# Elensil/Facet_Graph_Convolution

Hardware: AMD Instinct MI355X
Metric: facets/sec (fwd+bwd) on 100k-facet mesh (higher is better)
Workload: dtype f32; 1 GPU; c2: torus 250x200 quads = 100000 facets per GPU (N0=122224 padded nodes), full graph U-Net + MLP: rotate + forward + angular loss + backward + Adam, fp32, hipGraph replay; parallelism=single GPU

## Files before the change

facet_graph_convolution_amd/_lib.py:

```python
import ctypes as C
import os

import torch

_HERE = os.path.dirname(os.path.abspath(__file__))
LIB_PATH = os.environ.get("FGC_LIB", os.path.join(_HERE, "csrc", "libfgc.so"))

ABI_VERSION = 112
FGC_M = 9
AG_LD = 24
DL_LD = 12

c_f32p = C.c_void_p
c_i32p = C.c_void_p


class ConvDesc(C.Structure):
    _fields_ = [
        ("n", C.c_int32), ("nnz", C.c_int32),
        ("rowptr", C.c_void_p), ("col", C.c_void_p),
        ("x0", C.c_void_p), ("x1", C.c_void_p),
        ("c0", C.c_int32), ("c1", C.c_int32), ("shift", C.c_int32), ("cout", C.c_int32),
        ("W0", C.c_void_p), ("b", C.c_void_p), ("u", C.c_void_p), ("c", C.c_void_p), ("v", C.c_void_p),
        ("bias_mask", C.c_int32), ("act", C.c_int32), ("alpha", C.c_float), ("src_rows", C.c_int32), ("max_deg", C.c_int32),
        ("tile_list", C.c_void_p), ("n_tiles", C.c_int32), ("proj_row0", C.c_int32), ("proj_rows", C.c_int32),
        ("flags", C.c_int32),
        ("pair_rowptr", C.c_void_p), ("pair_col", C.c_void_p), ("pair_mul", C.c_void_p),
        ("n_pairs", C.c_int32), ("max_pair_deg", C.c_int32), ("max_pair_in_deg", C.c_int32),
        ("hc", C.c_void_p),
        ("options", C.c_void_p), ("n_options", C.c_int32), ("reserved1", C.c_int32),
        ("packed_layout", C.c_uint64),
    ]


class OptionOverride(C.Structure):
    _fields_ = [("index", C.c_int32), ("reserved", C.c_int32), ("value", C.c_int64)]


def option_overrides(**values):
    names = option_names()
    arr = (OptionOverride * len(values))()
    for k, (name, value) in enumerate(values.items()):
        arr[k].index, arr[k].reserved, arr[k].value = names.index(name[4:] if name.startswith("FGC_") else name), 0, int(value)
    return arr


class RowJob(C.Structure):
    _fields_ = [("src", C.c_void_p), ("idx", C.c_void_p), ("dst", C.c_void_p), ("rows", C.c_int32), ("width", C.c_int32)]


class ConvBwdIO(C.Structure):
    _fields_ = [
        ("trowptr", C.c_void_p), ("tcol", C.c_void_p), ("tedge", C.c_void_p), ("max_in_deg", C.c_int32), ("stages", C.c_int32),
        ("ag", C.c_void_p), ("y", C.c_void_p), ("dy", C.c_void_p),
        ("ds", C.c_void_p), ("dl", C.c_void_p), ("dag", C.c_void_p), ("r", C.c_void_p),
        ("dx0", C.c_void_p), ("dx1", C.c_void_p),
        ("accumulate0", C.c_int32), ("accumulate1", C.c_int32),
        ("dW0", C.c_void_p), ("db", C.c_void_p), ("du", C.c_void_p), ("dc", C.c_void_p), ("dv", C.c_void_p),
        ("data_tile_list", C.c_void_p), ("n_data_tiles", C.c_int32), ("flags", C.c_int32),
        ("z_saved", C.c_void_p), ("pool_y", C.c_void_p), ("pool_dy", C.c_void_p),
        ("tpair_rowptr", C.c_void_p), ("tpair_col", C.c_void_p), ("tpair_edge", C.c_void_p), ("dt", C.c_void_p),
        ("r_ld", C.c_int32), ("reserved0", C.c_int32),
    ]


class PackExtra(C.Structure):
    _fields_ = [
        ("rot_x", C.c_void_p), ("rot_y", C.c_void_p), ("rot_R", C.c_void_p), ("rot_rows", C.c_int64), ("rot_vecs", C.c_int32),
        ("rot_ag", C.c_void_p), ("rot_u", C.c_void_p), ("rot_c", C.c_void_p), ("rot_v", C.c_void_p),
        ("mlp_bf16", C.c_int32), ("mlp_W1", C.c_void_p), ("mlp_W2", C.c_void_p),
        ("mlp_n", C.c_int32), ("mlp_cin", C.c_int32), ("mlp_hidden", C.c_int32), ("mlp_cout", C.c_int32),
        ("mlp_fwd_ws", C.c_void_p), ("mlp_bwd_ws", C.c_void_p),
    ]


CONV_PACKED = 1
MLP_PACKED = 1
CONV_DEFER_REDUCE = 2
CONV_DEFER_DW = 16
CONV_SAVE_Z = 4
CONV_BF16 = 8
CONV_R_PAD = 32
SYNTH_ON = 0x80000000


def mlp_layout(layout_id):
    return int(layout_id) << 8


_SIGS = {
    "fgc_last_error": (C.c_char_p, []),
    "fgc_version": (C.c_int, []),
    "fgc_set_option": (C.c_int, [C.c_char_p, C.c_int64]),
    "fgc_get_option": (C.c_int, [C.c_char_p, C.POINTER(C.c_int64)]),
    "fgc_option_count": (C.c_int32, []),
    "fgc_option_name": (C.c_char_p, [C.c_int32]),
    "fgc_struct_size": (C.c_size_t, [C.c_int32]),
    "fgc_crc32c": (C.c_uint32, [C.c_uint32, C.c_void_p, C.c_size_t]),
    "fgc_profile_enable": (C.c_int, [C.c_int]),
    "fgc_profile_tag": (C.c_int, [C.c_char_p]),
    "fgc_profile_collect": (C.c_int, [C.c_char_p, C.c_int32]),
    "fgc_csr_from_klist": (C.c_int, [C.c_void_p, C.c_int32, C.c_int32, C.c_void_p, C.c_void_p, C.c_void_p]),
    "fgc_klist_from_csr": (C.c_int, [C.c_void_p, C.c_void_p, C.c_int32, C.c_int32, C.c_void_p]),
    "fgc_csr_transpose": (C.c_int, [C.c_void_p, C.c_void_p, C.c_int32, C.c_void_p, C.c_void_p, C.c_void_p]),
    "fgc_pair_graph": (C.c_int, [C.c_void_p, C.c_void_p, C.c_int32, C.c_void_p, C.c_void_p, C.c_void_p, C.c_void_p]),
    "fgc_face_features": (C.c_int, [C.c_void_p, C.c_int32, C.c_void_p, C.c_int32, C.c_void_p, C.c_void_p]),
    "fgc_faces_large_adj": (C.c_int, [C.c_void_p, C.c_int32, C.c_int32, C.c_int32, C.c_void_p, C.c_void_p]),
    "fgc_graph_patch": (C.c_int, [C.c_void_p, C.c_int32, C.c_int32, C.c_int32, C.c_int32, C.c_void_p, C.c_int32, C.c_void_p,
                                  C.c_void_p, C.c_void_p, C.c_void_p]),
    "fgc_mesh_patch": (C.c_int, [C.c_void_p, C.c_int32, C.c_void_p, C.c_int32, C.c_void_p, C.c_int32, C.c_int32,
                                 C.c_int32, C.c_void_p, C.c_int32, C.c_void_p, C.c_void_p, C.c_void_p, C.c_void_p,
                                 C.POINTER(C.c_int32), C.POINTER(C.c_int32)]),
    "fgc_vertices_faces": (C.c_int, [C.c_void_p, C.c_int32, C.c_int32, C.c_int32, C.c_void_p]),
    "fgc_face_centers": (C.c_int, [C.c_void_p, C.c_int32, C.c_void_p, C.c_int32, C.c_void_p, C.c_void_p]),
    "fgc_pool4_avg_iz": (C.c_int, [C.c_void_p, C.c_int32, C.c_int32, C.c_void_p, C.c_void_p]),
    "fgc_vertex_update_ms": (C.c_int, [C.c_void_p, C.c_void_p, C.c_int32, C.c_void_p, C.c_int32, C.c_void_p, C.c_int32,
                                       C.c_void_p, C.c_void_p, C.c_void_p, C.c_void_p, C.c_void_p, C.c_void_p,
                                       C.c_size_t, C.c_void_p]),
    "fgc_edge_map": (C.c_int, [C.c_void_p, C.c_int32, C.c_int32, C.c_int32, C.c_void_p, C.c_void_p, C.c_void_p]),
    "fgc_vertex_update": (C.c_int, [C.c_void_p, C.c_void_p, C.c_void_p, C.c_int32, C.c_void_p, C.c_int32, C.c_void_p,
                                    C.c_int32, C.c_void_p, C.c_int32, C.c_int32, C.c_float, C.c_void_p]),
    "fgc_metis_one_level": (C.c_int, [C.c_void_p, C.c_void_p, C.c_void_p, C.c_int64, C.c_void_p, C.c_void_p,
                                      C.c_int32, C.c_void_p, C.c_void_p]),
    "fgc_hierarchy_build": (C.c_int, [C.c_void_p, C.c_int32, C.c_int32, C.c_void_p, C.c_void_p, C.c_int32,
                                      C.c_uint64, C.c_void_p, C.c_void_p, C.c_void_p]),
    "fgc_hierarchy_free": (None, [C.c_void_p]),
    "fgc_hierarchy_size": (C.c_int32, [C.c_void_p, C.c_int32]),
    "fgc_hierarchy_real_size": (C.c_int32, [C.c_void_p, C.c_int32]),
    "fgc_hierarchy_new_to_old": (C.c_int, [C.c_void_p, C.c_int32, C.c_void_p]),
    "fgc_hierarchy_parents": (C.c_int, [C.c_void_p, C.c_int32, C.c_void_p]),
    "fgc_hierarchy_klist": (C.c_int, [C.c_void_p, C.c_int32, C.c_int32, C.c_void_p, C.c_void_p]),
    "fgc_conv_workspace_bytes": (C.c_size_t, [C.POINTER(ConvDesc)]),
    "fgc_conv_fwd": (C.c_int, [C.POINTER(ConvDesc), C.c_void_p, C.c_void_p, C.c_void_p, C.c_void_p, C.c_size_t,
                               C.c_void_p]),
    "fgc_conv_bwd_workspace_bytes": (C.c_size_t, [C.POINTER(ConvDesc)]),
# ... 195 lines not shown
```

facet_graph_convolution_amd/csrc/fgc_common.h:

```cpp
#pragma once
#include <hip/hip_runtime.h>
#include <stdint.h>
#include <stdio.h>
#include <stdarg.h>
#include <stdlib.h>

#include "../../include/fgc.h"

namespace fgc {

void set_error(const char* fmt, ...);

#define FGC_CHECK_ARG(cond, ...)          \
    do {                                  \
        if (!(cond)) {                    \
            fgc::set_error(__VA_ARGS__);  \
            return FGC_EINVAL;            \
        }                                 \
    } while (0)

#define FGC_CHECK_LAUNCH(what)                                                        \
    do {                                                                              \
        hipError_t e__ = hipGetLastError();                                           \
        if (e__ != hipSuccess) {                                                      \
// ... 11 lines not shown
    ProfScope(const char* name, hipStream_t s) : st(s), on(prof_enabled()) {
        if (on) prof_begin(name, st);
    }
    ~ProfScope() {
        if (on) prof_end(st);
    }
};
#define FGC_LAUNCH(name, st, kernel, grid, block, smem, ...)                      \
    do {                                                                          \
        fgc::ProfScope prof__(name, st);                                          \
        hipLaunchKernelGGL(kernel, grid, block, smem, st, __VA_ARGS__);           \
    } while (0)

struct LaunchCfg {
    const char* name;
    const char* what;
    hipStream_t st;
    int grid, block;
    size_t smem;
};
template <auto Kernel, typename... Args>
static inline int launch_kernel(const LaunchCfg& c, const Args&... args) {
    if (c.smem) hipFuncSetAttribute((const void*)Kernel, hipFuncAttributeMaxDynamicSharedMemorySize, (int)c.smem);
    FGC_LAUNCH(c.name, c.st, Kernel, dim3(c.grid), dim3(c.block), c.smem, args...);
    FGC_CHECK_LAUNCH(c.what);
    return FGC_OK;
}

#define FGC_OPTION_LIST(X)                                                                                                     \
    X(NO_W8, 0)                                                      \
    X(NO_W8FAST, 0)                                  \
    X(W8_NT16, 1)                           \
    X(W8_DATA16_MIN_N, 81920)                                    \
    X(W8_DATA_SMEM_PAD, 0)           \
    X(NO_PAIRS, 0)                                              \
    X(NO_NARROW, 0)                                                            \
    X(NO_NARROW_MMA, 0)                                             \
    X(NO_NARROW_FUSED_DS, 0)                              \
    X(NO_FUSED_DS, 0)                                      \
    X(NO_FUSED_DS_BF16, 0)                                                                                       \
    X(NO_FUSED_DS128, 0)                                                                   \
    X(NO_DS_VEC, 0)                                                                  \
    X(NO_K1M, 0)                                                            \
    X(NO_K1DEEP, 0)                                                              \
    X(K1_NT16, 1)                                                                       \
    X(NO_TNBF16, 0)                                                               \
    X(NO_TNSTREAM, 0)                                                                \
    X(TN_SLOTS, 64)                                           \
    X(TNB_WGS, 256)                                                             \
    X(NO_PROJ_STREAM, 0)                          \
    X(NO_MLP_SPLIT, 0)                              \
    X(NO_MLP_BWD_SPLIT, 0)                                                                         \
    X(NO_K1_SPLIT, 0)                         \
    X(NO_BFM, 0)
enum Opt {
#define FGC_OPT_ENUM(name, def) OPT_##name,
    FGC_OPTION_LIST(FGC_OPT_ENUM)
#undef FGC_OPT_ENUM
    OPT_COUNT
};
int64_t opt(Opt o);
struct OptScope {
    const void* prev_list;
    int prev_n;
    OptScope(const void* overrides , int n);
    ~OptScope();
    OptScope(const OptScope&) = delete;
    OptScope& operator=(const OptScope&) = delete;
};
#define FGC_OPT_SCOPE(d) fgc::OptScope opt_scope__((d) ? (const void*)(d)->options : nullptr, (d) ? (d)->n_options : 0)

static inline int cdiv(int a, int b) { return (a + b - 1) / b; }
static inline size_t align_up(size_t x, size_t a) { return (x + a - 1) / a * a; }

typedef float f32x4 __attribute__((ext_vector_type(4)));
typedef float f32x2c __attribute__((ext_vector_type(2)));

#ifdef __HIPCC__
typedef __bf16 bf16x2 __attribute__((ext_vector_type(2)));
typedef __bf16 bf16x4 __attribute__((ext_vector_type(4)));
typedef __bf16 bf16x8 __attribute__((ext_vector_type(8)));
typedef unsigned u32x2 __attribute__((ext_vector_type(2)));
typedef unsigned u32x4 __attribute__((ext_vector_type(4)));
__device__ __forceinline__ f32x2c bf2_to_f2(unsigned w) {
    return f32x2c{__uint_as_float(w << 16), __uint_as_float(w & 0xFFFF0000u)};
}
__device__ __forceinline__ unsigned f2_to_bf2(float a, float b) {
    return __builtin_bit_cast(unsigned, __builtin_convertvector(f32x2c{a, b}, bf16x2));
}
__device__ __forceinline__ f32x4 bf4_to_f4(u32x2 w) {
    return f32x4{__uint_as_float(w[0] << 16), __uint_as_float(w[0] & 0xFFFF0000u), __uint_as_float(w[1] << 16),
                 __uint_as_float(w[1] & 0xFFFF0000u)};
}
__device__ __forceinline__ u32x2 f4_to_bf4(f32x4 v) { return u32x2{f2_to_bf2(v[0], v[1]), f2_to_bf2(v[2], v[3])}; }
__device__ __forceinline__ float bf_to_f(unsigned short h) { return __uint_as_float((unsigned)h << 16); }
__device__ __forceinline__ unsigned short f_to_bf(float v) {
    return __builtin_bit_cast(unsigned short, (__bf16)v);
}
__device__ __forceinline__ float ld_act(const float* base, size_t idx, int bf16) {
    return bf16 ? bf_to_f(reinterpret_cast<const unsigned short*>(base)[idx]) : base[idx];
}
__device__ __forceinline__ void st_act(float* base, size_t idx, float v, int bf16) {
    if (bf16) reinterpret_cast<unsigned short*>(base)[idx] = f_to_bf(v);
    else base[idx] = v;
}

#define FGC_ROW16_SUM(v)                      \
// ... 60 lines not shown
```

facet_graph_convolution_amd/csrc/fgc_conv_bwd.hip:

```cpp
#include <stdio.h>
#include <stdlib.h>
#include <string.h>

#include <algorithm>
#include <type_traits>

#include "fgc_conv_bwd.h"
#include "fgc_conv_narrow.h"
#include "fgc_conv_pair.h"
#include "fgc_gemm_tn.h"
#include "fgc_reduce.h"
#include "fgc_split.h"

namespace fgc {

__device__ __forceinline__ float slope_from_y(float y, float alpha) { return y > 0.f ? 1.f : (y < 0.f ? alpha : 0.f); }

__device__ __forceinline__ float pool4_grad_term(const float* __restrict__ y, const float* __restrict__ pool_y,
                                                 const float* __restrict__ pool_dy, int r, int col, int cout, int bf16) {
    const size_t pi = (size_t)(r >> 2) * cout + col;
    const float m = ld_act(pool_y, pi, bf16);
    const size_t b = (size_t)(r & ~3) * cout + col;
    float ne = 0.f;
#pragma unroll
    for (int k = 0; k < 4; ++k) ne += ld_act(y, b + (size_t)k * cout, bf16) == m ? 1.f : 0.f;
    return ld_act(y, (size_t)r * cout + col, bf16) == m ? ld_act(pool_dy, pi, bf16) / ne : 0.f;
}

__global__ __launch_bounds__(256) void ds_db_kernel(const float* __restrict__ dy, const float* __restrict__ y,
                                                    const int* __restrict__ rowptr, int n, int cout, int cp2, int act,
                                                    float alpha, int bias_mask, int rows_per_block,
                                                    float* __restrict__ ds, float* __restrict__ db_part, int in_bf16,
                                                    int out_bf16, const float* __restrict__ pool_y,
                                                    const float* __restrict__ pool_dy) {
    __shared__ float part[256];
    const int col = threadIdx.x % cp2, rl = threadIdx.x / cp2, nrl = 256 / cp2;
    const int r0 = blockIdx.x * rows_per_block;
    const int r1 = min(n, r0 + rows_per_block);
    float acc = 0.f;
    if (col < cout) {
        for (int r = r0 + rl; r < r1; r += nrl) {
            const int d = rowptr[r + 1] - rowptr[r];
            float g = ld_act(dy, (size_t)r * cout + col, in_bf16);
            if (pool_dy) g += pool4_grad_term(y, pool_y, pool_dy, r, col, cout, in_bf16);
            if (act) g *= slope_from_y(ld_act(y, (size_t)r * cout + col, in_bf16), alpha);
            if (!bias_mask || d > 0) acc += g;
            st_act(ds, (size_t)r * cout + col, d > 0 ? g / (float)d : 0.f, out_bf16);
        }
    }
    part[threadIdx.x] = acc;
    __syncthreads();
    if (rl == 0 && col < cout) {
        float v = 0.f;
        for (int t = 0; t < nrl; ++t) v += part[t * cp2 + col];
        db_part[(size_t)blockIdx.x * cout + col] = v;
    }
}

template <bool BF_IN, bool BF_OUT>
__global__ __launch_bounds__(256) void ds_db_vec_kernel(const float* __restrict__ dy, const float* __restrict__ y,
                                                        const int* __restrict__ rowptr, int n, int cout, int act,
                                                        float alpha, int bias_mask, int rows_per_block,
                                                        float* __restrict__ ds, float* __restrict__ db_part,
// ... 393 lines not shown
#pragma unroll
    for (int nn = 0; nn < NPW; ++nn) {
        const int node = wave * NPW + nn;
        const int i = tile0 + node;
        const int d = __builtin_amdgcn_readfirstlane(min(s.deg[node], KMAX));
        f32x4 da = f32x4{0.f, 0.f, 0.f, 0.f};
        if (d > 0 && i < p.n) {
            const int e0 = p.rowptr[i];
            const int ntile = d > 16 ? 2 : 1;
            for (int et = 0; et < ntile; ++et) {
                const int edge = et * 16 + lr;
                const bool ok = edge < d;
                const float* qr = s.qbuf + ((size_t)node * KMAX + min(edge, d - 1)) * QLD;
                f32x4 q = f32x4{0.f, 0.f, 0.f, 0.f};
                if (lq < 2) q = *reinterpret_cast<const f32x4*>(qr + 4 * lq);
                else if (lq == 2) q[0] = qr[8];
                f32x4 g = et == 0 ? dq[nn][0] : dq[nn][1];
                if (lq == 2) { g[1] = 0.f; g[2] = 0.f; g[3] = 0.f; }
                if (lq == 3) g = f32x4{0.f, 0.f, 0.f, 0.f};
                float dot = q[0] * g[0] + q[1] * g[1] + q[2] * g[2] + q[3] * g[3];
                dot += __shfl_xor(dot, 16);
                dot += __shfl_xor(dot, 32);
                f32x4 dl;
#pragma unroll
                for (int t = 0; t < 4; ++t) dl[t] = ok ? q[t] * (g[t] - dot) : 0.f;
                if (ok && lq < 3) *reinterpret_cast<f32x4*>(lp.dl + (size_t)(e0 + edge) * FGC_DL_LD + 4 * lq) = dl;
                da += dl;
            }
#pragma unroll
            for (int t = 0; t < 4; ++t) {
                float v = da[t];
                v += __shfl_xor(v, 1);
                v += __shfl_xor(v, 2);
                v += __shfl_xor(v, 4);
                v += __shfl_xor(v, 8);
                da[t] = v;
            }
        }
        if (i < p.n && lr == 0 && lq < 3) *reinterpret_cast<f32x4*>(lp.dag + (size_t)i * FGC_AG_LD + 4 * lq) = da;
        dcacc += da;
    }
    __syncthreads();
    if (lr == 0 && lq < 3) {
#pragma unroll
        for (int t = 0; t < 4; ++t) red[wave * 12 + 4 * lq + t] = dcacc[t];
    }
    __syncthreads();
    if (tid < 12) {
        const float v = tid < FGC_M ? (red[tid] + red[12 + tid]) + (red[24 + tid] + red[36 + tid]) : 0.f;
        lp.dc_part[(size_t)blockIdx.x * 12 + tid] = v;
    }
}

template <bool LONG, int OKG, int NT_ = 32, int NPW_ = 8, bool SPLIT = false>
__global__ __launch_bounds__((NT_ / NPW_) * 64, NT_ == 32 ? 2 : 4) void conv_bwd_logits_deep_kernel(CoreParams p, LogitParams lp) {
    static_assert((NT_ == 32 && NPW_ == 8) || (NT_ == 16 && NPW_ == 4 && !LONG), "tile shapes");
    static_assert(!SPLIT || (NT_ == 16 && OKG == 2), "split dz GEMM: half tiles of the 32-wide layers");
    constexpr int TILE = NT_, NPW = NPW_, NWV = NT_ / NPW_, NTHREADS = NWV * 64, RT = NT_ / 16, LPN = NTHREADS / NT_;
    static_assert(NWV == 4, "four waves either way: the column-tile split and the dc sums below assume it");
    extern __shared__ __attribute__((aligned(16))) char smem_raw[];
    constexpr int QS = LONG ? KMAX : 16;
    const Smem s = carve(smem_raw, ZSTRIDE, QS, NT_);
    const int opad = OKG ? OKG * 16 : lp.opad;
    const int ostride = OKG ? OKG * 16 + 8 : lp.ostride;
    float* dst = s.extra;
    float* red = dst + ((LONG && lp.a_global) ? 0 : TILE * ostride);
    const int tile0 = xcd_tile(blockIdx.x, gridDim.x) * TILE;
    const int tid = threadIdx.x;
    const int wave = tid >> 6, lane = tid & 63, lr = lane & 15, lq = lane >> 4;

    const bool a_global = LONG && lp.a_global;
    if (a_global) {
    } else if constexpr (OKG > 0) {
        constexpr int V4 = TILE * OKG * 16 / 4;
        constexpr int PER = (V4 + NTHREADS - 1) / NTHREADS;
        static_assert(V4 % NTHREADS == 0 || V4 < NTHREADS, "whole float4s per thread, or fewer float4s than threads");
        const f32x4* src = reinterpret_cast<const f32x4*>(lp.ds + (size_t)tile0 * (OKG * 16));
        const int vmax = (min(p.n - tile0, TILE) * OKG * 16) / 4 - 1;
        f32x4 v[PER];
        if (lp.dy) {
            const f32x4* dy4 = reinterpret_cast<const f32x4*>(lp.dy + (size_t)tile0 * (OKG * 16));
            const f32x4* y4 = reinterpret_cast<const f32x4*>(lp.y + (size_t)tile0 * (OKG * 16));
            f32x4* out4 = reinterpret_cast<f32x4*>(lp.ds_out + (size_t)tile0 * (OKG * 16));
            f32x4 gy[PER], yy[PER];
            int dg[PER];
#pragma unroll
            for (int k = 0; k < PER; ++k) {
                const int t = min(tid + k * NTHREADS, vmax);
                const int i = tile0 + t / (OKG * 4);
                gy[k] = dy4[t];
                if (lp.act || lp.pool_dy) yy[k] = y4[t];
                dg[k] = p.rowptr[i + 1] - p.rowptr[i];
            }
            if (lp.pool_dy) {
#pragma unroll
                for (int k = 0; k < PER; ++k) {
                    const int t = min(tid + k * NTHREADS, vmax);
                    const int rl = t / (OKG * 4), c4 = t % (OKG * 4);
                    const size_t pi = (size_t)((tile0 + rl) >> 2) * (OKG * 4) + c4;
                    const f32x4 m = reinterpret_cast<const f32x4*>(lp.pool_y)[pi];
                    const f32x4 gp = reinterpret_cast<const f32x4*>(lp.pool_dy)[pi];
                    f32x4 ne = f32x4{0.f, 0.f, 0.f, 0.f};
#pragma unroll
                    for (int q = 0; q < 4; ++q) {
                        const int tq = min(((rl & ~3) + q) * (OKG * 4) + c4, vmax);
                        const f32x4 yq = y4[tq];
#pragma unroll
                        for (int c = 0; c < 4; ++c) ne[c] += yq[c] == m[c] ? 1.f : 0.f;
                    }
#pragma unroll
                    for (int c = 0; c < 4; ++c) gy[k][c] += yy[k][c] == m[c] ? gp[c] / ne[c] : 0.f;
                }
            }
#pragma unroll
            for (int k = 0; k < PER; ++k) {
                const int t = tid + k * NTHREADS;
                const bool ok = t <= vmax;
                f32x4 g = gy[k];
                if (lp.act) {
#pragma unroll
// ... 776 lines not shown
    c.ds_vec = cout % vw == 0 && 256 % (cout / vw) == 0 && cout <= 256 && al16(io->dy, io->y ? io->y : io->dy, io->ds) && pool_al &&
               opt(OPT_NO_DS_VEC) != 1;
    const bool al = al16(io->ds);
    c.okg = !al ? 0 : cout == 32 ? 2 : cout == 64 ? 4 : (cout == 128 && w.k1_half && c.fuse_ds) ? 8 : 0;
    c.a_global = w.k1 == K1_DEEP && w.k1_long && cout > 32 && cout % 16 == 0 && al;
    c.k1 = c.narrow_path ? K1_NARROW : w.k1;
    c.k1_vec4 = conv_vec4_ok(d);
    c.ds = w.pairs ? DS_PAIR : c.fuse_ds ? DS_FUSED : (c.narrow_path && narrow_fuses_ds(d, io)) ? DS_NARROW_FUSED
         : c.ds_vec ? DS_VEC : DS_SCALAR;
    return c;
}

static TnPlan layer_tn_plan(const fgc_conv_desc* d, const fgc_conv_bwd_io* io, const BwdPlan& w) {
    const int cout = d->cout, PL = FGC_M * cout + 24;
    const int rps = tn_rows_per_slab(w.nred, w.splitW), rld = io_r_ld(io, cout, w.bf16);
    if (w.pairs)
        return tn_plan_of(w.bf16, true, true, io->r, PL, d->x0, nullptr, d->c0, 0, 0, w.nred, rps, w.slab, rld);
    const bool v4 = conv_vec4_ok(d) && (cout % 4 == 0) && ((uintptr_t)io->r % 16 == 0);
    const bool stream_ok = v4 && !(opt(OPT_NO_TNSTREAM) == 1);
    return tn_plan_of(w.bf16, v4, stream_ok, io->r, PL, d->x0, d->x1, d->c0, d->c1, d->shift, w.nred, rps, w.slab, rld);
}

static void conv_param_jobs(const fgc_conv_desc* d, const fgc_conv_bwd_io* io, const BwdPlan& w, RedJob* jobs) {
    const int cin = d->c0 + d->c1, cout = d->cout;
    const int P = FGC_M * cout, PL = P + 24;
    const int ns = cdiv(w.nred, tn_rows_per_slab(w.nred, w.splitW));
    const size_t sst = (size_t)PL * cin;
    jobs[0] = RedJob{w.slab, sst, ns, P * cin, cin, cin, io->dW0, w.rtmp};
    jobs[1] = RedJob{w.slab + (size_t)P * cin, sst, ns, FGC_M * cin, cin, cin, io->du};
    jobs[2] = RedJob{w.slab + (size_t)(P + 12) * cin, sst, ns, FGC_M * cin, cin, cin, io->dv};
    jobs[3] = RedJob{w.db_part, (size_t)cout, w.nb_db, cout, cout, cout, io->db};
    jobs[4] = RedJob{w.dc_part, (size_t)12, w.n_dc, 12, 12, FGC_M, io->dc};
}

static int launch_ds_db(const BwdPlan& w, const BwdCall& c, const fgc_conv_desc* d, const fgc_conv_bwd_io* io, hipStream_t st) {
    const LaunchCfg cfg{"ds_db_kernel", "fgc_conv_bwd/ds", st, w.nb_db, 256, 0};
    const float *yy = io->y ? io->y : io->dy, *pool_y = io->pool_dy ? io->pool_y : nullptr;
    const bool out_bf16 = w.bf16 && !c.narrow_path;
    if (c.ds == DS_SCALAR) {
        int cp2 = 1;
        while (cp2 < d->cout) cp2 <<= 1;
        return launch_kernel<ds_db_kernel>(cfg, io->dy, io->y, d->rowptr, d->n, d->cout, cp2, d->act, d->alpha, d->bias_mask, w.rows_per_db,
                                           io->ds, w.db_part, w.bf16 ? 1 : 0, out_bf16 ? 1 : 0, pool_y, io->pool_dy);
    }
    auto vec = [&](auto bf_in, auto bf_out) {
        return launch_kernel<ds_db_vec_kernel<decltype(bf_in)::value, decltype(bf_out)::value>>(
            cfg, io->dy, yy, d->rowptr, d->n, d->cout, d->act, d->alpha, d->bias_mask, w.rows_per_db, io->ds, w.db_part, pool_y, io->pool_dy);
    };
    if (!w.bf16) return vec(std::false_type{}, std::false_type{});
    return out_bf16 ? vec(std::true_type{}, std::true_type{}) : vec(std::true_type{}, std::false_type{});
}

static int launch_k1(const BwdPlan& w, const BwdCall& c, const fgc_conv_desc* d, const CoreParams& p, const LogitParams& lp,
                     hipStream_t st) {
    const int nt = w.k1_nodes, cout = d->cout;
    const int qs = ((w.k1 == K1_DEEP || w.k1 == K1_BF16) && !w.k1_long) ? 16 : KMAX;
    const size_t core = smem_core_bytes(w.k1 == K1_BF16 ? ZSTRIDE_BF / 2 : w.g1.zstride, qs, nt);
    const size_t tile = w.k1 == K1_BF16 ? (size_t)nt * (cout * 2 + 32) : lp.a_global ? 0 : (size_t)nt * lp.ostride * 4;
    LaunchCfg cfg{"conv_bwd_logits_deep_kernel", "fgc_conv_bwd/logits_mfma", st, cdiv(d->n, nt), NTHREADS, core + tile + 48 * 4};
    switch (c.k1) {
        case K1_BF16:
            cfg.name = "conv_bwd_logits_bf16_kernel";
            cfg.what = "fgc_conv_bwd/logits_bf16";
            if (w.k1_long) return launch_kernel<conv_bwd_logits_bf16_kernel<true>>(cfg, p, lp);
            if (w.k1_half) return launch_kernel<conv_bwd_logits_bf16_kernel<false, 16, 4>>(cfg, p, lp);
            return launch_kernel<conv_bwd_logits_bf16_kernel<false>>(cfg, p, lp);
        case K1_DEEP:
            if (w.k1_split) {
                FGC_CHECK_ARG(c.okg == 2, "fgc_conv_bwd: ds must be 16-byte aligned (cout=%d)", cout);
                return launch_kernel<conv_bwd_logits_deep_kernel<false, 2, 16, 4, true>>(cfg, p, lp);
            }
            if (w.k1_half) switch (c.okg) {
                case 2: return launch_kernel<conv_bwd_logits_deep_kernel<false, 2, 16, 4>>(cfg, p, lp);
                case 4: return launch_kernel<conv_bwd_logits_deep_kernel<false, 4, 16, 4>>(cfg, p, lp);
                case 8: return launch_kernel<conv_bwd_logits_deep_kernel<false, 8, 16, 4>>(cfg, p, lp);
                default: return launch_kernel<conv_bwd_logits_deep_kernel<false, 0, 16, 4>>(cfg, p, lp);
            }
            if (w.k1_long) switch (c.okg) {
                case 2: return launch_kernel<conv_bwd_logits_deep_kernel<true, 2>>(cfg, p, lp);
                case 4: return launch_kernel<conv_bwd_logits_deep_kernel<true, 4>>(cfg, p, lp);
                default: return launch_kernel<conv_bwd_logits_deep_kernel<true, 0>>(cfg, p, lp);
            }
            switch (c.okg) {
                case 2: return launch_kernel<conv_bwd_logits_deep_kernel<false, 2>>(cfg, p, lp);
                case 4: return launch_kernel<conv_bwd_logits_deep_kernel<false, 4>>(cfg, p, lp);
                default: return launch_kernel<conv_bwd_logits_deep_kernel<false, 0>>(cfg, p, lp);
            }
        case K1_MFMA:
            cfg.name = "conv_bwd_logits_mfma_kernel";
            return c.k1_vec4 ? launch_kernel<conv_bwd_logits_mfma_kernel<true>>(cfg, p, lp)
                             : launch_kernel<conv_bwd_logits_mfma_kernel<false>>(cfg, p, lp);
        default:
            cfg.what = "fgc_conv_bwd/logits";
            if (c.k1_vec4) {
                cfg.name = "conv_bwd_logits_kernel<LPN, true>";
                return launch_kernel<conv_bwd_logits_kernel<8, true>>(cfg, p, lp);
            }
            cfg.name = "conv_bwd_logits_kernel<LPN, false>";
            return launch_kernel<conv_bwd_logits_kernel<8, false>>(cfg, p, lp);
    }
}

enum DataKind { DATA_NONE, DATA_W8, DATA_TILED };
struct DataForm {
    int kind;
    W8Form w8;
    bool vec4;
    int max_deg;
};
static DataForm data_form(const BwdPlan& w, const BwdCall& c, const fgc_conv_desc* d, const fgc_conv_bwd_io* io, CoreParams& p,
                          DataEpilogue& ep) {
    DataForm f{};
    const int cin = d->c0 + d->c1, cout = d->cout;
    if (c.narrow_path) return f;
    if (w.pairs) {
        fill_core_params(p, w.g2, w.nred, io->tpair_rowptr, io->tpair_col, io->tpair_edge, io->dt, nullptr, cout, 0, 0, cin, io->ag,
                         0, 12, 0, w.Wpt);
        ep = DataEpilogue{io->dl, io->dag, io->r, io_r_ld(io, cout, w.bf16), d->u, d->v, cin, d->c0, 0, 0,
                          io->dx0, nullptr, io->accumulate0, 0};
        f.max_deg = d->max_pair_in_deg;
        f.kind = DATA_W8;
    } else {
        fill_core_params(p, w.g2, d->n, io->trowptr, io->tcol, io->tedge, io->ds, nullptr, cout, 0, 0, cin, io->ag,
                         d->shift, 12, 0, w.Wpt);
        ep = DataEpilogue{io->dl, io->dag, io->r, io_r_ld(io, cout, w.bf16), d->u, d->v, cin, d->c0, d->c1, d->shift,
                          io->dx0, io->dx1, io->accumulate0, io->accumulate1};
        f.max_deg = io->max_in_deg;
        f.kind = (w.bf16 || w8_supported(p, f.max_deg)) ? DATA_W8 : DATA_TILED;
        f.vec4 = (cout % 4 == 0) && ((uintptr_t)io->ds % 16 == 0) && ((uintptr_t)io->r % 16 == 0);
    }
    p.tile_list = io->data_tile_list;
    p.n_tiles = io->n_data_tiles;
    if (f.kind == DATA_W8) f.w8 = w8_form(p, &ep, f.max_deg, w.bf16);
    return f;
}

}

using namespace fgc;

extern "C" size_t fgc_conv_bwd_workspace_bytes(const fgc_conv_desc* d) {
    FGC_OPT_SCOPE(d);
    if (!d) return 0;
    return plan_bwd(d, nullptr).bytes;
}

extern "C" uint64_t fgc_conv_layout_id(const fgc_conv_desc* d) {
    FGC_OPT_SCOPE(d);
    return d ? conv_layout_id(d) : 1;
}

extern "C" int32_t fgc_conv_r_ld(int32_t cout, int32_t padded, int32_t bf16) {
    return conv_r_ld(cout, padded ? FGC_CONV_R_PAD : 0, bf16 != 0);
}

extern "C" int fgc_conv_bwd_needs_exchange(const fgc_conv_desc* d, const fgc_conv_bwd_io* io) {
    FGC_OPT_SCOPE(d);
    if (!d || !io) return 1;
    return (io->dx0 == nullptr && narrow_supported(d)) ? 0 : 1;
}

extern "C" int fgc_conv_forms(const fgc_conv_desc* d, const fgc_conv_bwd_io* io, char* buf, int32_t buf_bytes) {
    FGC_OPT_SCOPE(d);
    int rc = validate_conv_desc(d, "fgc_conv_forms");
    if (rc) return rc;
    FGC_CHECK_ARG(buf && buf_bytes > 0, "fgc_conv_forms: no buffer");
    int len = 0;
    bool full = false;
    auto put = [&](const char* key, const char* fmt, auto value) {
        char tmp[96];
        int k = snprintf(tmp, sizeof tmp, "%s%s=", len ? " " : "", key);
        k += snprintf(tmp + k, sizeof tmp - k, fmt, value);
        if (len + k + 1 > buf_bytes) { full = true; return; }
        memcpy(buf + len, tmp, (size_t)k + 1);
        len += k;
    };
    auto put_w8 = [&](const char* pre, const W8Form& f, bool vec4) {
        char key[32];
        auto k = [&](const char* name) { snprintf(key, sizeof key, "%s_%s", pre, name); return key; };
        put(k("fast"), "%d", (int)f.fast);
        put(k("slots"), "%d", f.qs);
        put(k("nt"), "%d", f.nt);
        put(k("bfm"), "%d", (int)f.bfm);
        put(k("vec4"), "%d", (int)vec4);
    };
    static const char* const fwd_names[] = {"pair", "narrow", "w8", "tiled"};
    static const char* const proj_names[] = {"pair", "narrow", "bf16", "stream", "block", "block"};
    static const char* const ds_names[] = {"pair", "fused", "narrow-fused", "vec", "scalar"};
    static const char* const k1_names[] = {"pair", "narrow", "bf16", "deep", "mfma", "valu"};
    static const char* const k2_names[] = {"none", "w8", "tiled"};
    static const char* const tn_names[] = {"stream2", "stream4", "stream2_bf", "stream4_bf", "bf16_4", "bf16_2", "plain_v4", "plain"};
    buf[0] = 0;
    CoreParams p;
    const FwdForm ff = conv_fwd_form(d, io ? io->ag : nullptr, nullptr, &p);
    put("fwd", "%s", fwd_names[ff.kind]);
    if (ff.kind == FWD_NARROW) put("fwd_mma", "%d", (int)narrow_fwd_mma(d, nullptr));
    put_w8("fwd", ff.kind == FWD_W8 ? ff.w8 : W8Form{false, false, KMAX, TILE}, ff.vec4);
    put("proj", "%s", proj_names[ff.proj]);
    const BwdPlan w = call_plan(d, io, nullptr);
    const int rps = tn_rows_per_slab(w.nred, w.splitW);
    const BwdCall c = io ? bwd_call(w, d, io) : BwdCall{};
    if (io) {
        put("ds", "%s", ds_names[c.ds]);
        put("k1", "%s", k1_names[c.k1]);
        if (c.k1 == K1_NARROW) put("k1_mma", "%d", (int)narrow_bwd_mma(d, io));
        put("k1_okg", "%d", c.okg);
        put("k1_aglobal", "%d", (int)c.a_global);
        put("k1_vec4", "%d", (int)c.k1_vec4);
    } else {
        put("k1", "%s", k1_names[w.k1]);
    }
    put("k1_long", "%d", (int)w.k1_long);
    put("k1_half", "%d", (int)w.k1_half);
    put("k1_split", "%d", (int)w.k1_split);
    put("k1_nodes", "%d", w.k1_nodes);
    if (io) {
        DataEpilogue ep;
        const DataForm df = data_form(w, c, d, io, p, ep);
        put("k2", "%s", k2_names[df.kind]);
        put_w8("k2", df.kind == DATA_W8 ? df.w8 : W8Form{false, false, KMAX, TILE}, df.kind == DATA_W8 || df.vec4);
        put("k2_chunks", "%d", df.max_deg > 0 ? cdiv(df.max_deg, KMAX) : 0);
        if (c.k1 == K1_NARROW) put("k3", "%s", "narrow");
        else {
            const TnPlan pl = layer_tn_plan(d, io, w);
            put("k3", "%s", tn_names[pl.variant]);
            put("k3_slabs", "%d", pl.nsplits);
            put("k3_rows", "%d", pl.a.rps);
        }
    } else {
        put("k3_slabs", "%d", cdiv(w.nred, rps));
        put("k3_rows", "%d", rps);
    }
    put("nb_db", "%d", w.nb_db);
    put("n_dc", "%d", w.n_dc);
    put("layout_id", "%llu", (unsigned long long)layout_id_of(w));
    FGC_CHECK_ARG(!full, "fgc_conv_forms: buffer of %d bytes too small", buf_bytes);
    return len;
}

extern "C" int fgc_conv_bwd(const fgc_conv_desc* d, const fgc_conv_bwd_io* io, void* workspace,
                            size_t workspace_bytes, void* stream) {
    FGC_OPT_SCOPE(d);
    int rc = validate_conv_desc(d, "fgc_conv_bwd");
    if (rc) return rc;
    const int cin = d->c0 + d->c1, cout = d->cout;
    const BwdPlan w = call_plan(d, io, (char*)workspace);
    const bool bf16 = w.bf16;
    FGC_CHECK_ARG(io != nullptr, "fgc_conv_bwd: null io");
    FGC_CHECK_ARG(io->trowptr && io->tcol && io->tedge, "fgc_conv_bwd: transposed CSR missing");
    FGC_CHECK_ARG(io->ag && io->dy && io->ds && io->dl && io->dag && io->r, "fgc_conv_bwd: null buffer");
    FGC_CHECK_ARG(!d->act || io->y, "fgc_conv_bwd: y required when an activation was applied");
    FGC_CHECK_ARG(io->dW0 && io->db && io->du && io->dc && io->dv, "fgc_conv_bwd: null parameter-gradient pointer");
    FGC_CHECK_ARG(io->dx0 != nullptr || io->dx1 == nullptr, "fgc_conv_bwd: dx1 without dx0");
    FGC_CHECK_ARG(io_r_ld_ok(io, cout, bf16),
                  "fgc_conv_bwd: r_ld = %d is not a row stride of r for cout = %d (0, or >= %d and congruent to it modulo %d)",
                  io->r_ld, cout, FGC_M * cout + 24, bf16 ? 8 : 4);
    FGC_CHECK_ARG(!(io->flags & FGC_CONV_PACKED) || d->packed_layout == 0 || d->packed_layout == layout_id_of(w),
                  "fgc_conv_bwd: FGC_CONV_PACKED, but the operands were packed in layout %llu and the options now select %llu "
                  "(an option changed between fgc_conv_pack and this call)", (unsigned long long)d->packed_layout,
                  (unsigned long long)layout_id_of(w));
    FGC_CHECK_ARG(workspace && workspace_bytes >= w.bytes && (uintptr_t)workspace % 16 == 0,
                  "fgc_conv_bwd: workspace too small or misaligned (%zu < %zu)", workspace_bytes, w.bytes);
    hipStream_t st = (hipStream_t)stream;
    const BwdCall c = bwd_call(w, d, io);
    const int stages = c.stages;
    const bool pack_here = !(io->flags & FGC_CONV_PACKED);
    PackJob pjobs[2];
    size_t ptotals[2];
    if (w.pairs) {
        FGC_CHECK_ARG(io->tpair_rowptr && io->tpair_col && io->tpair_edge && io->dt && d->max_pair_in_deg > 0,
                      "fgc_conv_bwd: the pair form needs the transposed pair graph, dt and max_pair_in_deg");
        FGC_CHECK_ARG(!io->pool_dy, "fgc_conv_bwd: the pair form has no pooled output");
        FGC_CHECK_ARG(io->data_tile_list == nullptr || (io->n_data_tiles >= 0 && io->n_data_tiles <= cdiv(w.nred, TILE)),
                      "fgc_conv_bwd: pair form: n_data_tiles=%d outside [0, %d]", io->n_data_tiles, cdiv(w.nred, TILE));
        FGC_CHECK_ARG(((uintptr_t)io->dt | (uintptr_t)io->dy | (uintptr_t)io->dl | (uintptr_t)io->dag | (uintptr_t)io->r) % 16 == 0,
                      "fgc_conv_bwd: the pair form needs 16-byte aligned buffers");
        if ((stages & 4) && pack_here) {
            rc = launch_pack_jobs(pjobs, ptotals, conv_bwd_pack_jobs(d, w, pjobs, ptotals), "fgc_conv_bwd/pack", st);
            if (rc) return rc;
        }
        if (stages & 3) {
            rc = launch_pair_bwd_logits(d, io, w.db_part, w.dc_part, st);
            if (rc) return rc;
        }
        if (stages & 4) {
            CoreParams p;
            DataEpilogue ep;
            data_form(w, c, d, io, p, ep);
            const size_t smem = conv_smem_bytes(w.g2, (size_t)TILE * 24 * 4);
            FGC_CHECK_ARG(w8_erow_supported(p, d->max_pair_in_deg) && (!bf16 || w8_bf16_supported(p, d->max_pair_in_deg)),
                          "fgc_conv_bwd: pair form: unsupported shape (cin=%d cout=%d max_pair_in_deg=%d)", cin, cout,
                          d->max_pair_in_deg);
            if (!p.tile_list || p.n_tiles > 0) {
                rc = launch_data_w8_erow(p, ep, smem, d->max_pair_in_deg, st, bf16);
                if (rc) return rc;
            }
        }
    } else {
        FGC_CHECK_ARG(io->data_tile_list == nullptr || (io->n_data_tiles >= 0 && io->n_data_tiles <= cdiv(d->n, TILE)),
                      "fgc_conv_bwd: n_data_tiles=%d outside [0, %d]", io->n_data_tiles, cdiv(d->n, TILE));
        FGC_CHECK_ARG(!bf16 || c.narrow_path || (w.deep_ok && cout % 32 == 0),
                      "fgc_conv_bwd: FGC_CONV_BF16 needs widths that are multiples of 32, 16-byte aligned tensors and degrees <= %d "
                      "(cin=%d cout=%d max_deg=%d)", KMAX, cin, cout, d->max_deg);
        FGC_CHECK_ARG(!io->pool_dy || (io->pool_y && io->y && d->n % 4 == 0),
                      "fgc_conv_bwd: pool_dy needs pool_y, y and a row count that is a multiple of 4 (n=%d)", d->n);
        if ((stages & 1) && (c.ds == DS_VEC || c.ds == DS_SCALAR)) {
            rc = launch_ds_db(w, c, d, io, st);
            if (rc) return rc;
        }
        if (c.k1 == K1_NARROW) {
            if (stages & 2) {
                rc = narrow_bwd_logits(d, io, w.narrow_ws, w.db_part, st);
                if (rc) return rc;
            }
            if (stages & 8) {
                rc = narrow_bwd_params(d, io, w.narrow_ws, w.db_part, narrow_db_partials(d, io, w.nb_db),
                                       (io->flags & FGC_CONV_DEFER_REDUCE) ? 1 : 3, nullptr, st);
                if (rc) return rc;
            }
            return FGC_OK;
        }
        if ((stages & 6) && pack_here) {
            rc = launch_pack_jobs(pjobs, ptotals, conv_bwd_pack_jobs(d, w, pjobs, ptotals), "fgc_conv_bwd/pack", st);
            if (rc) return rc;
        }
        if (stages & 2) {
            CoreParams p;
            fill_core_params(p, w.g1, d->n, d->rowptr, d->col, nullptr, d->x0, d->x1, d->c0, d->c1, d->shift, cout, io->ag,
                             d->shift, 0, 12, nullptr);
            LogitParams lp{io->ds, cout, w.opad, w.opad + 8, w.Wq, io->dl, io->dag, w.dc_part};
            if (c.fuse_ds) {
                lp.dy = io->dy;
                lp.y = io->y ? io->y : io->dy;
                lp.act = d->act;
                lp.bias_mask = d->bias_mask;
                lp.alpha = d->alpha;
                lp.ds_out = io->ds;
                lp.db_part = w.db_part;
                lp.pool_y = io->pool_dy ? io->pool_y : nullptr;
                lp.pool_dy = io->pool_dy;
            }
            lp.a_global = c.a_global;
            rc = launch_k1(w, c, d, p, lp, st);
            if (rc) return rc;
        }
        if ((stages & 4) && !(io->data_tile_list && io->n_data_tiles == 0)) {
            CoreParams p;
            DataEpilogue ep;
            const DataForm f = data_form(w, c, d, io, p, ep);
            const size_t smem = conv_smem_bytes(w.g2, (size_t)TILE * 24 * 4);
            if (bf16)
                FGC_CHECK_ARG(w8_bf16_supported(p, io->max_in_deg), "fgc_conv_bwd: FGC_CONV_BF16: unsupported shape for the data "
                              "gradient (cin=%d cout=%d max_in_deg=%d)", cin, cout, io->max_in_deg);
            if (f.kind == DATA_W8) {
                rc = launch_data_w8(p, ep, smem, io->max_in_deg, st, bf16);
            } else if (f.vec4) {
                rc = launch_kernel<conv_bwd_data_kernel<8, true>>(
                    LaunchCfg{"conv_bwd_data_kernel<LPN, true>", "fgc_conv_bwd/data", st, core_grid(p), NTHREADS, smem}, p, ep);
            } else {
                rc = launch_kernel<conv_bwd_data_kernel<8, false>>(
                    LaunchCfg{"conv_bwd_data_kernel<LPN, false>", "fgc_conv_bwd/data", st, core_grid(p), NTHREADS, smem}, p, ep);
            }
            if (rc) return rc;
        }
    }
    if (stages & 8) {
        if (!(io->flags & FGC_CONV_DEFER_DW)) {
            rc = tn_launch_one(layer_tn_plan(d, io, w), "gemm_tn_kernel:dW", st);
            if (rc) return rc;
        }
        if (!(io->flags & FGC_CONV_DEFER_REDUCE)) {
            RedJob jobs[5];
            conv_param_jobs(d, io, w, jobs);
            rc = reduce_jobs("reduce:params", jobs, 5, nullptr, st);
            if (rc) return rc;
        }
    }
    return FGC_OK;
}

extern "C" int fgc_conv_bwd_reduce(const fgc_conv_desc* const* descs, const fgc_conv_bwd_io* const* ios,
                                   void* const* bwd_ws, int32_t count, void* stream) {
    FGC_CHECK_ARG(descs && ios && bwd_ws && count >= 0, "fgc_conv_bwd_reduce: bad arguments");
    hipStream_t st = (hipStream_t)stream;
    RedJob jobs[RED_MAX_JOBS];
    int nj = 0, rc = 0;
    auto flush = [&]() {
        const int r = nj ? reduce_jobs("reduce:params", jobs, nj, nullptr, st) : FGC_OK;
        nj = 0;
        return r;
    };
    {
        TnJobs G[TN_NVARIANTS];
        int nb[TN_NVARIANTS];
        for (int v = 0; v < TN_NVARIANTS; ++v) G[v].njobs = 0, nb[v] = 0;
        for (int i = 0; i < count; ++i) {
            const fgc_conv_desc* d = descs[i];
            const fgc_conv_bwd_io* io = ios[i];
            if (!io || !(io->flags & FGC_CONV_DEFER_DW)) continue;
            FGC_OPT_SCOPE(d);
            rc = validate_conv_desc(d, "fgc_conv_bwd_reduce");
            if (rc) return rc;
            FGC_CHECK_ARG(bwd_ws[i], "fgc_conv_bwd_reduce: layer %d: null workspace", i);
            const BwdPlan w = plan_bwd(d, (char*)bwd_ws[i]);
            TnPlan pl;
            if (io->dx0 == nullptr && w.narrow) {
                const float* A;
                float* slab;
                int zld, rps;
                narrow_tn_operands(d, io, w.narrow_ws, &A, &zld, &slab, &rps);
                pl = tn_plan_of(false, true, true, A, zld, io->ds, nullptr, d->cout, 0, 0, d->n, rps, slab);
            } else {
                FGC_CHECK_ARG(io->r, "fgc_conv_bwd_reduce: layer %d: FGC_CONV_DEFER_DW without r", i);
                FGC_CHECK_ARG(io_r_ld_ok(io, d->cout, (d->flags & FGC_CONV_BF16) != 0),
                              "fgc_conv_bwd_reduce: layer %d: r_ld = %d is not a row stride of r for cout = %d", i, io->r_ld, d->cout);
                pl = layer_tn_plan(d, io, w);
            }
            if (!tn_groupable(pl.variant)) {
                rc = tn_launch_one(pl, "gemm_tn_kernel:dW", st);
                if (rc) return rc;
                continue;
            }
            TnJobs& J = G[pl.variant];
            if (J.njobs == TN_MAX_JOBS) {
                rc = tn_launch_group(pl.variant, J, nb[pl.variant], "gemm_tn_kernel:dW", st);
                if (rc) return rc;
                nb[pl.variant] = 0;
            }
            pl.a.block0 = nb[pl.variant];
            J.job[J.njobs++] = pl.a;
            nb[pl.variant] += (int)tn_grid(pl.ntiles, pl.nsplits).x;
        }
        for (int v = 0; v < TN_NVARIANTS; ++v) {
            rc = tn_launch_group(v, G[v], nb[v], "gemm_tn_kernel:dW", st);
            if (rc) return rc;
        }
    }
    for (int i = 0; i < count; ++i) {
        const fgc_conv_desc* d = descs[i];
        const fgc_conv_bwd_io* io = ios[i];
        FGC_OPT_SCOPE(d);
        rc = validate_conv_desc(d, "fgc_conv_bwd_reduce");
        if (rc) return rc;
        FGC_CHECK_ARG(io && bwd_ws[i] && io->dW0 && io->db && io->du && io->dc && io->dv,
                      "fgc_conv_bwd_reduce: layer %d: null io / workspace / gradient pointer", i);
        const BwdPlan w = plan_bwd(d, (char*)bwd_ws[i]);
        if (nj + 5 > RED_MAX_JOBS && (rc = flush())) return rc;
        if (io->dx0 == nullptr && w.narrow) {
            rc = narrow_bwd_params(d, io, w.narrow_ws, w.db_part, narrow_db_partials(d, io, w.nb_db), 0, jobs + nj, st);
            if (rc) return rc;
            nj += NARROW_RED_JOBS;
        } else {
            conv_param_jobs(d, io, w, jobs + nj);
            nj += 5;
        }
    }
    if ((rc = flush())) return rc;
    return FGC_OK;
}
```

facet_graph_convolution_amd/csrc/fgc_conv_pair.h:

```cpp
#pragma once
#include "fgc_common.h"

namespace fgc {

bool pairs_ok(const fgc_conv_desc* d);
bool pairs_graph_allowed(int64_t rows, int64_t n_pairs, int max_in_deg, int cout);
int pair_blocks_per_wg(int cout);
static inline int pair_num_wgs(const fgc_conv_desc* d) {
    const int bpg = pair_blocks_per_wg(d->cout);
    return ((d->n >> 2) + bpg - 1) / bpg;
}
int launch_pair_fwd(const fgc_conv_desc* d, float* ag, float* y, void* workspace, hipStream_t st);
int launch_pair_bwd_logits(const fgc_conv_desc* d, const fgc_conv_bwd_io* io, float* db_part, float* dc_part,
                           hipStream_t st);

}
```

facet_graph_convolution_amd/csrc/fgc_conv_pair.hip:

```cpp
#include <stdlib.h>

#include "fgc_conv_core.h"
#include "fgc_conv_pair.h"

namespace fgc {

constexpr int PQ_LD = 12;
constexpr int PQ_SLOTS = 16;
constexpr int PQ_STRIDE = PQ_SLOTS * PQ_LD + 4;

bool pairs_graph_allowed(int64_t rows, int64_t n_pairs, int max_in_deg, int cout) {
    if (rows < 0 || n_pairs < 0 || cout <= 0 || max_in_deg < 0 || max_in_deg > KMAX) return false;
    if ((uint64_t)rows * FGC_M * cout * 4 >= 0xFFFFFFFFull || (uint64_t)n_pairs * cout * 4 >= 0xFFFFFFFFull) return false;
    if (rows >= (1 << 24) || n_pairs >= (1 << 24) - (1 << 20)) return false;
    return true;
}

bool pairs_ok(const fgc_conv_desc* d) {
    if (opt(OPT_NO_PAIRS) == 1) return false;
    if ((opt(OPT_NO_W8) == 1) || (opt(OPT_NO_W8FAST) == 1))
        return false;
    if (!d || !d->pair_rowptr || !d->pair_col || !d->pair_mul || !d->hc) return false;
    if (d->shift != 2 || d->c1 != 0 || d->x1 != nullptr || (d->n & 3)) return false;
    if (!(d->c0 == 32 || d->c0 == 64 || d->c0 == 128) || !(d->cout == 32 || d->cout == 64)) return false;
    if (d->n_pairs <= 0 || d->max_pair_deg <= 0 || d->max_pair_in_deg < 0 || d->max_pair_in_deg > KMAX) return false;
    if (d->tile_list && d->n_tiles != 0) return false;
    const size_t rows = d->src_rows > 0 ? (size_t)d->src_rows : (size_t)(d->n >> 2);
    if (!pairs_graph_allowed((int64_t)rows, d->n_pairs, d->max_pair_in_deg, d->cout)) return false;
    if (((uintptr_t)d->x0 | (uintptr_t)d->hc) % 16) return false;
    return true;
}

int pair_blocks_per_wg(int cout) { return 4 * (64 / (cout / 4)); }

#ifndef FGC_PT_RT
#define FGC_PT_RT 2
#endif
#ifndef FGC_PT_KO
#define FGC_PT_KO 0
#endif
#ifndef FGC_PT_CG
#define FGC_PT_CG 10
#endif
template <int CIN, int RT>
__global__ __launch_bounds__(256) void pair_transform_kernel(const float* __restrict__ x, int rows,
                                                            const float* __restrict__ W0, const float* __restrict__ u,
                                                            const float* __restrict__ c, const float* __restrict__ v,
                                                            int cout, float* __restrict__ hc, float* __restrict__ ag,
                                                            int ngroups) {
    constexpr int KG = CIN / 16;
    const int wave = threadIdx.x >> 6, lane = threadIdx.x & 63, lr = lane & 15, lq = lane >> 4;
    const int item = __builtin_amdgcn_readfirstlane(blockIdx.x * 4 + wave);
    const int rt = item / ngroups, cg = item - rt * ngroups;
    if (rt * (16 * RT) >= rows) return;
    const int th = (FGC_M * cout) >> 4;
    const int tc = th + 2;
// ... 310 lines not shown
#pragma unroll
    for (int i = 0; i < 4; ++i) yv[i] = f32x4{0.f, 0.f, 0.f, 0.f};
    for (int k0 = 0; k0 < dmax; k0 += PQ_SLOTS) {
        if (k0) pair_wave_sync();
        pair_softmax_chunk<LPB>(p, qb, kl, e0, d, k0, bc, a);
        pair_wave_sync();
        const int cnt = min(dmax - k0, PQ_SLOTS);
        HT h[FGC_M];
        pair_load_h<COUT, BF>(h_rs, qb, laneoff, h);
        FGC_PAIR_KLOOP_PRAGMA
        for (int k = 0; k < cnt; ++k) {
            const float* qk = qb + k * PQ_LD;
            const unsigned noff = pair_row_off<COUT, BF>(qb + min(k + 1, PQ_SLOTS - 1) * PQ_LD, laneoff);
            const f32x4 q0 = *reinterpret_cast<const f32x4*>(qk), q1 = *reinterpret_cast<const f32x4*>(qk + 4);
            const f32x2c q8m = *reinterpret_cast<const f32x2c*>(qk + 8), mm = *reinterpret_cast<const f32x2c*>(qk + 10);
            const float q[FGC_M] = {q0[0], q0[1], q0[2], q0[3], q1[0], q1[1], q1[2], q1[3], q8m[0]};
            const unsigned mu = __float_as_uint(mm[0]);
            f32x4 t = {0.f, 0.f, 0.f, 0.f};
#pragma unroll
            for (int m = 0; m < FGC_M; ++m) {
                t += q[m] * pair_h(h[m]);
                h[m] = pair_load_piece<COUT, BF>(h_rs, noff, m);
            }
            yv[0] += (float)(mu & 0xffu) * t;
            yv[1] += (float)((mu >> 8) & 0xffu) * t;
            yv[2] += (float)((mu >> 16) & 0xffu) * t;
            yv[3] += (float)(mu >> 24) * t;
        }
    }
    if (b >= p.nb) return;
    const f32x4 bias = *reinterpret_cast<const f32x4*>(p.bias + kl * 4);
#pragma unroll
    for (int i = 0; i < 4; ++i) {
        const float inv = deg[i] > 0 ? 1.0f / (float)deg[i] : 0.f;
        f32x4 o = yv[i] * inv;
        if (!p.bias_mask || deg[i] > 0) o += bias;
        if (p.act) {
#pragma unroll
            for (int t = 0; t < 4; ++t) o[t] = fmaxf(o[t], 0.f) - p.alpha * fmaxf(-o[t], 0.f);
        }
        pair_st4<BF>(p.y, (size_t)(4 * b + i) * COUT + kl * 4, o);
    }
}

template <int LPB>
__device__ __forceinline__ float pair_block_sum(float v) {
    v += fgc_dpp_c<0xB1>(v);
    v += fgc_dpp_c<0x4E>(v);
    v += fgc_dpp_c<0x141>(v);
    if constexpr (LPB == 16) v += fgc_dpp_c<0x140>(v);
    return v;
}

template <int COUT, bool BF>
__global__ __launch_bounds__(256, FGC_PAIR_LB_BWD) void pair_bwd_logits_kernel(PairParams p) {
    constexpr int LPB = COUT / 4, BPW = 64 / LPB, BPG = 4 * BPW;
    constexpr int RED_LD = COUT + 12;
    __shared__ __attribute__((aligned(16))) float qs[BPG * PQ_STRIDE];
    __shared__ __attribute__((aligned(16))) float red[BPG * RED_LD];
    const int wave = threadIdx.x >> 6, lane = threadIdx.x & 63, bl = lane / LPB, kl = lane % LPB;
    const int wg = xcd_tile(blockIdx.x, gridDim.x);
    const int b = (wg * 4 + wave) * BPW + bl;
    const bool valid = b < p.nb;
    const int bc = min(b, p.nb - 1);
    const int e0 = p.prow[bc];
    const int d = valid ? p.prow[bc + 1] - e0 : 0;
    float a[FGC_M];
    {
        const float* ar = p.ag + (size_t)bc * FGC_AG_LD;
        const f32x4 a0 = *reinterpret_cast<const f32x4*>(ar), a1 = *reinterpret_cast<const f32x4*>(ar + 4);
        a[0] = a0[0]; a[1] = a0[1]; a[2] = a0[2]; a[3] = a0[3]; a[4] = a1[0]; a[5] = a1[1]; a[6] = a1[2]; a[7] = a1[3];
        a[8] = ar[8];
    }
    f32x4 sv[4];
    f32x4 dbv = {0.f, 0.f, 0.f, 0.f};
#pragma unroll
    for (int i = 0; i < 4; ++i) {
        const int dg = p.rowptr[4 * bc + i + 1] - p.rowptr[4 * bc + i];
        const size_t o = (size_t)(4 * bc + i) * COUT + kl * 4;
        f32x4 g = pair_ld4<BF>(p.dy, o);
        if (p.act) {
            const f32x4 yy = pair_ld4<BF>(p.yact, o);
#pragma unroll
            for (int t = 0; t < 4; ++t) g[t] *= yy[t] > 0.f ? 1.f : (yy[t] < 0.f ? p.alpha : 0.f);
        }
        if (!valid) g = f32x4{0.f, 0.f, 0.f, 0.f};
        if (!p.bias_mask || dg > 0) dbv += g;
        sv[i] = g * (dg > 0 ? 1.0f / (float)dg : 0.f);
    }
    const int dmax = wave_max_i32(d);
    float* qb = qs + (wave * BPW + bl) * PQ_STRIDE;
    const __amdgpu_buffer_rsrc_t h_rs = __builtin_amdgcn_make_buffer_rsrc(const_cast<float*>(p.hc), 0, -1, 0x00020000);
    const unsigned laneoff = (unsigned)kl * (BF ? 8u : 16u);
    typedef typename PairH<BF>::T HT;
    float da[FGC_M];
#pragma unroll
    for (int m = 0; m < FGC_M; ++m) da[m] = 0.f;
    const __amdgpu_buffer_rsrc_t dt_rs = __builtin_amdgcn_make_buffer_rsrc(p.dt, 0, p.dt_bytes, 0x00020000);
    const __amdgpu_buffer_rsrc_t dl_rs = __builtin_amdgcn_make_buffer_rsrc(p.dl, 0, p.dl_bytes, 0x00020000);
    for (int k0 = 0; k0 < dmax; k0 += PQ_SLOTS) {
        if (k0) pair_wave_sync();
        pair_softmax_chunk<LPB>(p, qb, kl, e0, d, k0, bc, a);
        pair_wave_sync();
        const int cnt = min(dmax - k0, PQ_SLOTS);
        HT h[FGC_M];
        pair_load_h<COUT, BF>(h_rs, qb, laneoff, h);
        FGC_PAIR_KLOOP_PRAGMA
        for (int k = 0; k < cnt; ++k) {
            const float* qk = qb + k * PQ_LD;
            const int kk = k0 + k;
            const unsigned noff = pair_row_off<COUT, BF>(qb + min(k + 1, PQ_SLOTS - 1) * PQ_LD, laneoff);
            const f32x4 q0 = *reinterpret_cast<const f32x4*>(qk), q1 = *reinterpret_cast<const f32x4*>(qk + 4);
            const f32x2c q8m = *reinterpret_cast<const f32x2c*>(qk + 8), mm = *reinterpret_cast<const f32x2c*>(qk + 10);
            const float q[FGC_M] = {q0[0], q0[1], q0[2], q0[3], q1[0], q1[1], q1[2], q1[3], q8m[0]};
// ... 78 lines not shown
    const int ngroups = cdiv(tc, FGC_PT_CG);
    const int items = cdiv(rows, 16 * FGC_PT_RT) * ngroups;
    const bool bf16 = (d->flags & FGC_CONV_BF16) != 0;
    if (rows == 0) {
    } else if (bf16) {
        unsigned short* Wb = (unsigned short*)workspace;
        if (!(d->flags & FGC_CONV_PACKED)) {
            const int count = FGC_M * cout * cin;
            FGC_LAUNCH("pair_weight_bf16_kernel", st, pair_weight_bf16_kernel, dim3(cdiv(count, 1024)), dim3(256), 0, d->W0, Wb, count);
        }
#define FGC_PTB(CIN_)                                                                                                  \
    FGC_LAUNCH("pair_transform_kernel", st, (pair_transform_bf16_kernel<CIN_, FGC_PT_RT>), dim3(cdiv(items, 4)), dim3(256), 0,      \
               (const unsigned short*)x0, rows, Wb, d->u, d->c, d->v, cout, (unsigned short*)hc0, ag0, ngroups)
        if (cin == 32) FGC_PTB(32);
        else if (cin == 64) FGC_PTB(64);
        else FGC_PTB(128);
#undef FGC_PTB
    } else {
#define FGC_PT(CIN_)                                                                                                   \
    FGC_LAUNCH("pair_transform_kernel", st, (pair_transform_kernel<CIN_, FGC_PT_RT>), dim3(cdiv(items, 4)), dim3(256), 0, x0, rows,  \
               d->W0, d->u, d->c, d->v, cout, hc0, ag0, ngroups)
    if (cin == 32) FGC_PT(32);
    else if (cin == 64) FGC_PT(64);
    else FGC_PT(128);
#undef FGC_PT
    }
    FGC_CHECK_LAUNCH("fgc_conv_fwd/pair_transform");
    if (!blocks) return FGC_OK;
    PairParams p{};
    p.nb = d->n >> 2;
    p.prow = d->pair_rowptr;
    p.pcol = d->pair_col;
    p.pmul = d->pair_mul;
    p.ag = ag;
    p.hc = d->hc;
    p.rowptr = d->rowptr;
    p.bias = d->b;
    p.bias_mask = d->bias_mask;
    p.act = d->act;
    p.alpha = d->alpha;
    p.y = y;
    const int grid = pair_num_wgs(d);
    if (bf16) {
        if (cout == 32) FGC_LAUNCH("pair_fwd_kernel", st, (pair_fwd_kernel<32, true>), dim3(grid), dim3(256), 0, p);
        else FGC_LAUNCH("pair_fwd_kernel", st, (pair_fwd_kernel<64, true>), dim3(grid), dim3(256), 0, p);
    } else {
        if (cout == 32) FGC_LAUNCH("pair_fwd_kernel", st, (pair_fwd_kernel<32, false>), dim3(grid), dim3(256), 0, p);
        else FGC_LAUNCH("pair_fwd_kernel", st, (pair_fwd_kernel<64, false>), dim3(grid), dim3(256), 0, p);
    }
    FGC_CHECK_LAUNCH("fgc_conv_fwd/pair_fwd");
    return FGC_OK;
}

int launch_pair_bwd_logits(const fgc_conv_desc* d, const fgc_conv_bwd_io* io, float* db_part, float* dc_part, hipStream_t st) {
    PairParams p{};
    p.nb = d->n >> 2;
    p.prow = d->pair_rowptr;
    p.pcol = d->pair_col;
    p.pmul = d->pair_mul;
    p.ag = io->ag;
    p.hc = d->hc;
    p.rowptr = d->rowptr;
    p.bias_mask = d->bias_mask;
    p.act = d->act;
    p.alpha = d->alpha;
    p.dy = io->dy;
    p.yact = io->y;
    p.dt = io->dt;
    p.dl = io->dl;
    p.dag = io->dag;
    p.db_part = db_part;
    p.dc_part = dc_part;
    p.dt_bytes = (unsigned)((size_t)d->n_pairs * d->cout * ((d->flags & FGC_CONV_BF16) ? 2 : 4));
    p.dl_bytes = (unsigned)((size_t)d->n_pairs * FGC_DL_LD * 4);
    const int grid = pair_num_wgs(d);
    if (d->flags & FGC_CONV_BF16) {
        if (d->cout == 32) FGC_LAUNCH("pair_bwd_logits_kernel", st, (pair_bwd_logits_kernel<32, true>), dim3(grid), dim3(256), 0, p);
        else FGC_LAUNCH("pair_bwd_logits_kernel", st, (pair_bwd_logits_kernel<64, true>), dim3(grid), dim3(256), 0, p);
    } else {
        if (d->cout == 32) FGC_LAUNCH("pair_bwd_logits_kernel", st, (pair_bwd_logits_kernel<32, false>), dim3(grid), dim3(256), 0, p);
        else FGC_LAUNCH("pair_bwd_logits_kernel", st, (pair_bwd_logits_kernel<64, false>), dim3(grid), dim3(256), 0, p);
    }
    FGC_CHECK_LAUNCH("fgc_conv_bwd/pair_logits");
    return FGC_OK;
}

}

extern "C" int fgc_conv_uses_pairs(const fgc_conv_desc* d) {
    FGC_OPT_SCOPE(d);
    return fgc::pairs_ok(d) ? 1 : 0;
}
extern "C" int fgc_conv_pairs_allowed(int64_t rows, int64_t n_pairs, int32_t max_pair_in_deg, int32_t cout) {
    return fgc::pairs_graph_allowed(rows, n_pairs, max_pair_in_deg, cout) ? 1 : 0;
}
```

facet_graph_convolution_amd/csrc/fgc_gemm_tn.h:

```cpp
#pragma once
#include "fgc_common.h"

namespace fgc {

struct TnArgs {
    const void* A;
    const void* x0;
    const void* x1;
    float* slab;
    int lda, P, c0, c1, shift, rows, rps;
    int block0;
};
constexpr int TN_MAX_JOBS = 8;
struct TnJobs {
    TnArgs job[TN_MAX_JOBS];
    int njobs;
};
constexpr int TNB_PC = 320;

enum TnVariant { TN_STREAM2 = 0, TN_STREAM4, TN_STREAM2_BF, TN_STREAM4_BF, TN_BF16_4, TN_BF16_2, TN_PLAIN_V4, TN_PLAIN, TN_NVARIANTS };
struct TnPlan {
    int variant;
    TnArgs a;
    int ntiles, nsplits;
};
static inline bool tn_groupable(int v) { return v <= TN_BF16_2; }
static inline dim3 tn_grid(int ntiles, int nsplits) { return dim3((unsigned)(ntiles * 8 * cdiv(nsplits, 8))); }
TnPlan tn_plan_of(bool bf16, bool vec4, bool stream_ok, const void* A, int PL, const void* x0, const void* x1, int c0, int c1,
                  int shift, int rows, int rps, float* slab, int lda = 0);
int tn_launch_one(const TnPlan& pl, const char* tag, hipStream_t st);
int tn_launch_group(int variant, TnJobs& J, int nblocks, const char* tag, hipStream_t st);

bool tn_bf16_ok(int P, int c0, int c1);
int tn_rows_per_slab(int n, int splits);
int tn_splits(int P, int Q, int rows);
int tn_balanced_splits(int desired, int maxs, int rows);
int launch_gemm_tn_stream(const char* tag, const float* A, int lda, int P, const float* x0, int c0, int rows,
                          int rows_per_split, int nsplits, float* slab, hipStream_t st);

}
```

facet_graph_convolution_amd/csrc/fgc_gemm_tn.hip:

```cpp
#include <algorithm>

#include "fgc_gemm_tn.h"

namespace fgc {


template <bool VEC4>
__device__ __forceinline__ void tn_load(const float* __restrict__ A, int lda, int P, const float* __restrict__ x0,
                                        const float* __restrict__ x1, int c0, int c1, int shift, int row, bool valid,
                                        int pbase, int qbase, f32x4& a, f32x4& b) {
    a = f32x4{0.f, 0.f, 0.f, 0.f};
    b = f32x4{0.f, 0.f, 0.f, 0.f};
    if (!valid) return;
    const int Q = c0 + c1;
    const size_t sr = (size_t)(row >> shift);
    if (VEC4) {
        if (pbase < P) a = *reinterpret_cast<const f32x4*>(A + (size_t)row * lda + pbase);
        if (qbase < c0) b = *reinterpret_cast<const f32x4*>(x0 + sr * c0 + qbase);
        else if (qbase < Q) b = *reinterpret_cast<const f32x4*>(x1 + sr * c1 + (qbase - c0));
    } else {
#pragma unroll
        for (int t = 0; t < 4; ++t) {
            if (pbase + t < P) a[t] = A[(size_t)row * lda + pbase + t];
            const int q = qbase + t;
            if (q < c0) b[t] = x0[sr * c0 + q];
            else if (q < Q) b[t] = x1[sr * c1 + (q - c0)];
        }
    }
}

__device__ __forceinline__ bool tn_block(int ntiles, int nsplits, int& tile, int& split, int vblock = -1) {
    const int L = vblock >= 0 ? vblock : (int)blockIdx.x, xcd = L & 7, idx = L >> 3;
    tile = idx % ntiles;
    split = (idx / ntiles) * 8 + xcd;
    return split < nsplits;
}

__device__ __forceinline__ int tn_job_of(const TnJobs& J) {
    int q = 0;
#pragma unroll
    for (int t = 1; t < TN_MAX_JOBS; ++t)
        if (t < J.njobs && (int)blockIdx.x >= J.job[t].block0) q = t;
    return q;
}

template <bool VEC4>
__global__ __launch_bounds__(256) void gemm_tn_kernel(const float* __restrict__ A, int lda, int P,
                                                      const float* __restrict__ x0, const float* __restrict__ x1,
                                                      int c0, int c1, int shift, int rows, int rows_per_split,
                                                      float* __restrict__ slab) {
    __shared__ float red[4][64][65];
    const int Q = c0 + c1;
    const int npt = (P + 63) >> 6;
    int tile_id, split_id;
    if (!tn_block(npt * ((Q + 63) >> 6), (rows + rows_per_split - 1) / rows_per_split, tile_id, split_id)) return;
    const int pt = tile_id % npt, qt = tile_id / npt;
    const int p0 = pt * 64, q0 = qt * 64;
    const int tid = threadIdx.x, wave = tid >> 6, lane = tid & 63, lr = lane & 15, lq = lane >> 4;
    const int r_begin = split_id * rows_per_split;
    const int r_end = min(rows, r_begin + rows_per_split);
    const int nsteps = (r_end - r_begin + 3) >> 2;
    const int pbase = p0 + 4 * lr, qbase = q0 + 4 * lr;
    f32x4 acc[4][4];
#pragma unroll
    for (int i = 0; i < 4; ++i)
#pragma unroll
        for (int j = 0; j < 4; ++j) acc[i][j] = f32x4{0.f, 0.f, 0.f, 0.f};

    f32x4 a0, b0, a1, b1;
    auto ld = [&](int step, f32x4& a, f32x4& b) {
        const int row = r_begin + 4 * step + lq;
        tn_load<VEC4>(A, lda, P, x0, x1, c0, c1, shift, row, step < nsteps && row < r_end, pbase, qbase, a, b);
    };
    auto mm = [&](const f32x4& a, const f32x4& b) {
#pragma unroll
        for (int i = 0; i < 4; ++i)
#pragma unroll
            for (int j = 0; j < 4; ++j) acc[i][j] = __builtin_amdgcn_mfma_f32_16x16x4f32(a[i], b[j], acc[i][j], 0, 0, 0);
    };
    ld(wave, a0, b0);
    ld(wave + 4, a1, b1);
    for (int s = wave; s < nsteps; s += 8) {
        mm(a0, b0);
        ld(s + 8, a0, b0);
        if (s + 4 < nsteps) mm(a1, b1);
        ld(s + 12, a1, b1);
    }
#pragma unroll
    for (int i = 0; i < 4; ++i)
#pragma unroll
        for (int j = 0; j < 4; ++j)
#pragma unroll
            for (int t = 0; t < 4; ++t) red[wave][4 * (lq * 4 + t) + i][4 * lr + j] = acc[i][j][t];
    __syncthreads();
    float* out = slab + (size_t)split_id * P * Q;
    for (int t = tid; t < 64 * 64; t += 256) {
        const int pp = t >> 6, qq = t & 63;
        if (p0 + pp < P && q0 + qq < Q)
            out[(size_t)(p0 + pp) * Q + q0 + qq] = (red[0][pp][qq] + red[1][pp][qq]) + (red[2][pp][qq] + red[3][pp][qq]);
    }
}

template <int NJ, bool BF>
__device__ __forceinline__ void tn_stream_body(const float* __restrict__ A, int lda, int P, const float* __restrict__ x0,
                                               const float* __restrict__ x1, int c0, int c1, int shift, int rows,
                                               int rows_per_split, float* __restrict__ slab, int vblock,
                                               float (*red)[64][65]) {
    const int Q = c0 + c1;
    const int npt = (P + 63) >> 6;
    int tile_id, split_id;
    if (!tn_block(npt * ((Q + 16 * NJ - 1) / (16 * NJ)), (rows + rows_per_split - 1) / rows_per_split, tile_id, split_id, vblock))
        return;
    const int pt = tile_id % npt, qt = tile_id / npt;
    const int p0 = pt * 64, q0 = qt * (16 * NJ);
    const int tid = threadIdx.x, lane = tid & 63, lr = lane & 15, lq = lane >> 4;
    const int wave = __builtin_amdgcn_readfirstlane(tid >> 6);
    const int r_begin = split_id * rows_per_split;
    const int r_end = min(rows, r_begin + rows_per_split);
    const int nsteps = (r_end - r_begin + 3) >> 2;
    const int pc = min(p0 + 4 * lr, P - 4);
    const int qc = min(q0 + NJ * lr, Q - NJ);
    const float* bsrc = BF ? reinterpret_cast<const float*>(reinterpret_cast<const unsigned short*>(qc < c0 ? x0 : x1) +
                                                            (qc < c0 ? qc : qc - c0))
                           : (qc < c0 ? x0 + qc : x1 + (qc - c0));
    const int bld = qc < c0 ? c0 : c1;
    f32x4 acc[4][NJ];
#pragma unroll
    for (int i = 0; i < 4; ++i)
#pragma unroll
        for (int j = 0; j < NJ; ++j) acc[i][j] = f32x4{0.f, 0.f, 0.f, 0.f};

    auto ld = [&](int step, f32x4& a, f32x4& b, int& row) {
        row = r_begin + 4 * step + lq;
        const int rc = min(row, r_end - 1);
        if constexpr (BF) {
            const unsigned short* A16 = reinterpret_cast<const unsigned short*>(A);
            const unsigned short* b16 = reinterpret_cast<const unsigned short*>(bsrc);
            a = bf4_to_f4(*reinterpret_cast<const u32x2*>(A16 + (size_t)rc * lda + pc));
            if constexpr (NJ == 4) {
                b = bf4_to_f4(*reinterpret_cast<const u32x2*>(b16 + (size_t)(rc >> shift) * bld));
            } else {
                const f32x2c b2 = bf2_to_f2(*reinterpret_cast<const unsigned*>(b16 + (size_t)(rc >> shift) * bld));
                b = f32x4{b2[0], b2[1], 0.f, 0.f};
            }
            return;
        }
        a = *reinterpret_cast<const f32x4*>(A + (size_t)rc * lda + pc);
        if constexpr (NJ == 4) {
            b = *reinterpret_cast<const f32x4*>(bsrc + (size_t)(rc >> shift) * bld);
        } else {
            const f32x2c b2 = *reinterpret_cast<const f32x2c*>(bsrc + (size_t)(rc >> shift) * bld);
            b = f32x4{b2[0], b2[1], 0.f, 0.f};
        }
    };
    auto mm = [&](f32x4 a, const f32x4& b, int row) {
        if (row >= r_end) a = f32x4{0.f, 0.f, 0.f, 0.f};
#pragma unroll
        for (int i = 0; i < 4; ++i)
#pragma unroll
            for (int j = 0; j < NJ; ++j) acc[i][j] = __builtin_amdgcn_mfma_f32_16x16x4f32(a[i], b[j], acc[i][j], 0, 0, 0);
    };
    f32x4 a0, b0, a1, b1, a2, b2, a3, b3;
    int r0, r1, r2, r3;
    ld(wave, a0, b0, r0);
    ld(wave + 4, a1, b1, r1);
    ld(wave + 8, a2, b2, r2);
    ld(wave + 12, a3, b3, r3);
#define FGC_TN_STEP(A_, B_, R_, NEXT_)          \
    mm(A_, B_, R_);                             \
    __builtin_amdgcn_sched_barrier(0);          \
    ld(NEXT_, A_, B_, R_);                      \
    __builtin_amdgcn_sched_barrier(0);
    for (int s = wave; s < nsteps; s += 16) {
        FGC_TN_STEP(a0, b0, r0, s + 16)
        FGC_TN_STEP(a1, b1, r1, s + 20)
        FGC_TN_STEP(a2, b2, r2, s + 24)
        FGC_TN_STEP(a3, b3, r3, s + 28)
    }
#undef FGC_TN_STEP
    auto put = [&](int slot) {
#pragma unroll
        for (int i = 0; i < 4; ++i)
#pragma unroll
            for (int j = 0; j < NJ; ++j)
#pragma unroll
                for (int t = 0; t < 4; ++t) red[slot][4 * (lq * 4 + t) + i][NJ * lr + j] = acc[i][j][t];
    };
    auto add = [&](int slot) {
#pragma unroll
        for (int i = 0; i < 4; ++i)
#pragma unroll
            for (int j = 0; j < NJ; ++j)
#pragma unroll
                for (int t = 0; t < 4; ++t) acc[i][j][t] += red[slot][4 * (lq * 4 + t) + i][NJ * lr + j];
    };
    if (wave == 1) put(0);
    if (wave == 3) put(1);
    __syncthreads();
    if (wave == 0) add(0);
    if (wave == 2) add(1);
    __syncthreads();
    if (wave == 0) put(0);
    if (wave == 2) put(1);
    __syncthreads();
    float* out = slab + (size_t)split_id * P * Q;
    for (int t = tid; t < 64 * 16 * NJ; t += 256) {
        const int pp = t / (16 * NJ), qq = t % (16 * NJ);
        if (p0 + pp < P && q0 + qq < Q) out[(size_t)(p0 + pp) * Q + q0 + qq] = red[0][pp][qq] + red[1][pp][qq];
    }
}

__device__ __forceinline__ bool tn_direct_ok(int lda, int c0, int c1, int shift, int rows_per_split) {
    return (c1 == 0 || (c0 & 31) == 0) && shift <= 4 &&
           (long long)(rows_per_split + 160) * max(lda, max(c0, c1)) < (1ll << 29);
}

template <int NJ>
__device__ __forceinline__ void tn_direct_body(const float* __restrict__ A, int lda, int P, const float* __restrict__ x0,
                                               const float* __restrict__ x1, int c0, int c1, int shift, int rows,
                                               int rows_per_split, float* __restrict__ slab, int vblock, f32x4* red) {
    constexpr int NH = NJ / 2;
    const int Q = c0 + c1;
    const int npt = (P + 63) >> 6;
    int tile_id, split_id;
    if (!tn_block(npt * ((Q + 16 * NJ - 1) / (16 * NJ)), (rows + rows_per_split - 1) / rows_per_split, tile_id, split_id, vblock))
        return;
    const int pt = tile_id % npt, qt = tile_id / npt;
    const int p0 = pt * 64, q0 = qt * (16 * NJ);
    const int tid = threadIdx.x, lane = tid & 63, lr = lane & 15, lq = lane >> 4;
    const int wave = __builtin_amdgcn_readfirstlane(tid >> 6);
    const int r_begin = split_id * rows_per_split;
    const int r_end = min(rows, r_begin + rows_per_split);
    const int nsteps = (r_end - r_begin + 3) >> 2;
    const int row0 = 4 * wave + lq;
    const int pc = min(p0 + 4 * lr, P - 4);
    const __amdgpu_buffer_rsrc_t a_rs = __builtin_amdgcn_make_buffer_rsrc(
        const_cast<float*>(A + (size_t)r_begin * lda), 0, (r_end - r_begin) * lda * 4, 0x00020000);
    unsigned ao = (unsigned)(row0 * lda + pc) * 4u;
    const unsigned astep = 16u * (unsigned)lda * 4u;
    const int xr0 = r_begin >> shift, xrows = ((rows - 1) >> shift) + 1;
    const int xrow0 = ((r_begin + row0) >> shift) - xr0;
    __amdgpu_buffer_rsrc_t b_rs[NH];
    unsigned bo[NH], bstep[NH];
#pragma unroll
    for (int h = 0; h < NH; ++h) {
        const int hs = q0 + 32 * h;
        const bool first = hs < c0 || c1 == 0;
        const int ld = first ? c0 : c1;
        const size_t bytes = (size_t)(xrows - xr0) * ld * 4;
        b_rs[h] = __builtin_amdgcn_make_buffer_rsrc(const_cast<float*>((first ? x0 : x1) + (size_t)xr0 * ld), 0,
                                                    (int)(unsigned)std::min<size_t>(bytes, 0xffffffffu), 0x00020000);
        bo[h] = (unsigned)(xrow0 * ld + min(hs + 2 * lr, Q - 2) - (first ? 0 : c0)) * 4u;
        bstep[h] = (unsigned)((16 >> shift) * ld) * 4u;
    }
    f32x4 acc[4][NJ];
#pragma unroll
    for (int i = 0; i < 4; ++i)
#pragma unroll
        for (int j = 0; j < NJ; ++j) acc[i][j] = f32x4{0.f, 0.f, 0.f, 0.f};

    struct Set {
        f32x4 a;
        f32x2c b[NH];
    };
    auto ld = [&](Set& s) {
        s.a = __builtin_bit_cast(f32x4, __builtin_amdgcn_raw_buffer_load_b128(a_rs, ao, 0, 0));
        ao += astep;
        asm volatile("" : "+v"(ao));
#pragma unroll
        for (int h = 0; h < NH; ++h) {
            s.b[h] = __builtin_bit_cast(f32x2c, __builtin_amdgcn_raw_buffer_load_b64(b_rs[h], bo[h], 0, 0));
            bo[h] += bstep[h];
            asm volatile("" : "+v"(bo[h]));
        }
    };
    auto mm = [&](const Set& s) {
#pragma unroll
        for (int i = 0; i < 4; ++i)
#pragma unroll
            for (int j = 0; j < NJ; ++j)
                acc[i][j] = __builtin_amdgcn_mfma_f32_16x16x4f32(s.a[i], s.b[j >> 1][j & 1], acc[i][j], 0, 0, 0);
    };
    if (wave < nsteps) {
        Set s0, s1, s2, s3;
        ld(s0);
        __builtin_amdgcn_sched_barrier(0);
        ld(s1);
        __builtin_amdgcn_sched_barrier(0);
        ld(s2);
        __builtin_amdgcn_sched_barrier(0);
        ld(s3);
        __builtin_amdgcn_sched_barrier(0);
#define FGC_TN_STEP(S_)                         \
    mm(S_);                                     \
    __builtin_amdgcn_sched_barrier(0);          \
    ld(S_);                                     \
    __builtin_amdgcn_sched_barrier(0);
        int s = wave;
        do {
            FGC_TN_STEP(s0)
            FGC_TN_STEP(s1)
            FGC_TN_STEP(s2)
            FGC_TN_STEP(s3)
            s += 16;
        } while (s < nsteps);
    }
#undef FGC_TN_STEP
    auto put = [&](int slot) {
#pragma unroll
        for (int e = 0; e < 4 * NJ; ++e) red[(slot * 4 * NJ + e) * 64 + lane] = acc[e / NJ][e % NJ];
    };
    auto add = [&](int slot) {
#pragma unroll
        for (int e = 0; e < 4 * NJ; ++e) acc[e / NJ][e % NJ] += red[(slot * 4 * NJ + e) * 64 + lane];
    };
    if (wave == 1) put(0);
    if (wave == 3) put(1);
    __syncthreads();
    if (wave == 0) add(0);
    if (wave == 2) {
        add(1);
        put(1);
    }
    __syncthreads();
    if (wave != 0) return;
    add(1);
    const __amdgpu_buffer_rsrc_t c_rs =
        __builtin_amdgcn_make_buffer_rsrc(slab + (size_t)split_id * P * Q, 0, P * Q * 4, 0x00020000);
#pragma unroll
    for (int h = 0; h < NH; ++h) {
        const int q = q0 + 32 * h + 2 * lr;
        const unsigned co = q < Q ? (unsigned)((p0 + 16 * lq) * Q + q) * 4u : 0x80000000u;
#pragma unroll
        for (int t = 0; t < 4; ++t)
#pragma unroll
            for (int i = 0; i < 4; ++i)
                __builtin_amdgcn_raw_buffer_store_b64(__builtin_bit_cast(u32x2, f32x2c{acc[i][2 * h][t], acc[i][2 * h + 1][t]}), c_rs,
                                                      co + (unsigned)((4 * t + i) * Q) * 4u, 0, 0);
    }
}

template <int NJ, bool BF>
__device__ __forceinline__ void tn_stream_any(const float* __restrict__ A, int lda, int P, const float* __restrict__ x0,
                                              const float* __restrict__ x1, int c0, int c1, int shift, int rows,
                                              int rows_per_split, float* __restrict__ slab, int vblock) {
    __shared__ __attribute__((aligned(16))) float red[2][64][65];
    if constexpr (!BF) {
        if (tn_direct_ok(lda, c0, c1, shift, rows_per_split)) {
            tn_direct_body<NJ>(A, lda, P, x0, x1, c0, c1, shift, rows, rows_per_split, slab, vblock,
                               reinterpret_cast<f32x4*>(&red[0][0][0]));
            return;
        }
    }
    tn_stream_body<NJ, BF>(A, lda, P, x0, x1, c0, c1, shift, rows, rows_per_split, slab, vblock, red);
}
template <int NJ, bool BF = false>
__global__ __launch_bounds__(256, 4) void gemm_tn_stream_kernel(const float* __restrict__ A, int lda, int P,
                                                                const float* __restrict__ x0,
                                                                const float* __restrict__ x1, int c0, int c1, int shift,
                                                                int rows, int rows_per_split, float* __restrict__ slab) {
    tn_stream_any<NJ, BF>(A, lda, P, x0, x1, c0, c1, shift, rows, rows_per_split, slab, -1);
}
template <int NJ, bool BF = false>
__global__ __launch_bounds__(256, 4) void gemm_tn_stream_group_kernel(TnJobs J) {
    const TnArgs& a = J.job[tn_job_of(J)];
    tn_stream_any<NJ, BF>((const float*)a.A, a.lda, a.P, (const float*)a.x0, (const float*)a.x1, a.c0, a.c1, a.shift, a.rows,
                          a.rps, a.slab, (int)blockIdx.x - a.block0);
}

constexpr int TNB_THREADS = 256;
constexpr int TNB_AS = TNB_PC * 2 + 32;
typedef short s16x4 __attribute__((ext_vector_type(4)));

__device__ __forceinline__ u32x4 tnb_frag(const char* tile, int stride, int col0, int lq, int lr) {
    const char* a = tile + (4 * lq + (lr >> 2)) * stride + (col0 + 4 * (lr & 3)) * 2;
    const s16x4 lo = __builtin_amdgcn_ds_read_tr16_b64_v4i16((__attribute__((address_space(3))) s16x4*)a);
    const s16x4 hi = __builtin_amdgcn_ds_read_tr16_b64_v4i16((__attribute__((address_space(3))) s16x4*)(a + 16 * stride));
    const u32x2 l2 = __builtin_bit_cast(u32x2, lo), h2 = __builtin_bit_cast(u32x2, hi);
    return u32x4{l2[0], l2[1], h2[0], h2[1]};
}

template <int QT>
__device__ __forceinline__ void tn_bf16_body(const unsigned short* __restrict__ A, int lda, int P,
                                             const unsigned short* __restrict__ x0, const unsigned short* __restrict__ x1, int c0,
                                             int c1, int shift, int rows, int rows_per_split, float* __restrict__ slab,
                                             int vblock) {
    constexpr int QC = QT * 16;
    constexpr int XS = QC * 2 + 32;
    constexpr int APC = TNB_PC / 8;
    constexpr int NA = 32 * APC / TNB_THREADS;
    static_assert(32 * APC % TNB_THREADS == 0 && 32 * (QC / 8) <= TNB_THREADS, "staging shape");
    __shared__ __attribute__((aligned(16))) char As[2][32 * TNB_AS];
    __shared__ __attribute__((aligned(16))) char Xs[2][32 * XS];
    const int Q = c0 + c1;
    const int npc = (P + TNB_PC - 1) / TNB_PC;
    int tile_id, split_id;
    if (!tn_block(npc * (Q / QC), (rows + rows_per_split - 1) / rows_per_split, tile_id, split_id, vblock)) return;
    const int pc = tile_id % npc, qc = tile_id / npc;
    const int p0 = pc * TNB_PC, q0 = qc * QC;
    const int pw = min(P - p0, TNB_PC);
    const int tid = threadIdx.x, lane = tid & 63, lr = lane & 15, lq = lane >> 4;
    const int wave = __builtin_amdgcn_readfirstlane(tid >> 6);
    const int r_begin = split_id * rows_per_split;
    const int r_end = min(rows, r_begin + rows_per_split);
    const int nchunks = (r_end - r_begin + 31) >> 5;

    u32x4 ra[NA], rx;
    const int xrow = min(tid, 32 * (QC / 8) - 1) / (QC / 8), xcol = (min(tid, 32 * (QC / 8) - 1) % (QC / 8)) * 8;
    const int qcol = q0 + xcol;
    const bool x_first = qcol < c0;
    const unsigned short* xsrc = x_first ? x0 : x1;
    const int xld = x_first ? c0 : c1;
    const int xoff = min(x_first ? qcol : qcol - c0, xld - 8);
    auto fetch = [&](int ch) {
        const int rb = r_begin + ch * 32;
#pragma unroll
        for (int i = 0; i < NA; ++i) {
            const int t = tid + i * TNB_THREADS;
            const int row = min(rb + t / APC, r_end - 1);
            const int col = p0 + min((t % APC) * 8, pw - 8);
// ... 14 lines not shown
            const bool ok = rb + xrow < r_end && qcol < Q;
            *reinterpret_cast<u32x4*>(&Xs[buf][xrow * XS + xcol * 2]) = ok ? rx : u32x4{0u, 0u, 0u, 0u};
        }
    };
    f32x4 acc[5][QT];
#pragma unroll
    for (int i = 0; i < 5; ++i)
#pragma unroll
        for (int j = 0; j < QT; ++j) acc[i][j] = f32x4{0.f, 0.f, 0.f, 0.f};

    if (nchunks > 0) {
        fetch(0);
        stage(0, 0);
    }
    __syncthreads();
    for (int ch = 0; ch < nchunks; ++ch) {
        const int buf = ch & 1;
        if (ch + 1 < nchunks) fetch(ch + 1);
        u32x4 af[5], bq[QT];
#pragma unroll
        for (int i = 0; i < 5; ++i) af[i] = tnb_frag(As[buf], TNB_AS, (wave * 5 + i) * 16, lq, lr);
#pragma unroll
        for (int j = 0; j < QT; ++j) bq[j] = tnb_frag(Xs[buf], XS, j * 16, lq, lr);
#pragma unroll
        for (int i = 0; i < 5; ++i)
#pragma unroll
            for (int j = 0; j < QT; ++j)
                acc[i][j] = __builtin_amdgcn_mfma_f32_16x16x32_bf16(__builtin_bit_cast(bf16x8, af[i]), __builtin_bit_cast(bf16x8, bq[j]),
                                                                   acc[i][j], 0, 0, 0);
        if (ch + 1 < nchunks) stage(ch + 1, buf ^ 1);
        __syncthreads();
    }
    float* out = slab + (size_t)split_id * P * Q;
#pragma unroll
    for (int i = 0; i < 5; ++i)
#pragma unroll
        for (int j = 0; j < QT; ++j)
#pragma unroll
            for (int t = 0; t < 4; ++t) {
                const int pp = p0 + (wave * 5 + i) * 16 + lq * 4 + t, qq = q0 + j * 16 + lr;
                if (pp < p0 + pw && qq < Q) out[(size_t)pp * Q + qq] = acc[i][j][t];
            }
}
template <int QT>
__global__ __launch_bounds__(TNB_THREADS, 2) void gemm_tn_bf16_kernel(const unsigned short* __restrict__ A, int lda, int P,
                                                                      const unsigned short* __restrict__ x0,
                                                                      const unsigned short* __restrict__ x1, int c0, int c1,
                                                                      int shift, int rows, int rows_per_split,
                                                                      float* __restrict__ slab) {
    tn_bf16_body<QT>(A, lda, P, x0, x1, c0, c1, shift, rows, rows_per_split, slab, -1);
}
template <int QT>
__global__ __launch_bounds__(TNB_THREADS, 2) void gemm_tn_bf16_group_kernel(TnJobs J) {
    const TnArgs& a = J.job[tn_job_of(J)];
    tn_bf16_body<QT>((const unsigned short*)a.A, a.lda, a.P, (const unsigned short*)a.x0, (const unsigned short*)a.x1, a.c0, a.c1,
                     a.shift, a.rows, a.rps, a.slab, (int)blockIdx.x - a.block0);
}

bool tn_bf16_ok(int P, int c0, int c1) {
    if (opt(OPT_NO_TNBF16) == 1) return false;
    const int Q = c0 + c1;
    return P % 8 == 0 && c0 % 8 == 0 && c1 % 8 == 0 && Q % 32 == 0 && (c1 == 0 || c0 % 16 == 0) && c0 >= 8 && (c1 == 0 || c1 >= 8);
}

int launch_gemm_tn_stream(const char* tag, const float* A, int lda, int P, const float* x0, int c0, int rows,
                          int rows_per_split, int nsplits, float* slab, hipStream_t st) {
    if (c0 <= 32 && c0 % 2 == 0) {
        const dim3 grid = tn_grid(cdiv(P, 64), nsplits);
        FGC_LAUNCH(tag, st, gemm_tn_stream_kernel<2>, grid, dim3(256), 0, A, lda, P, x0, (const float*)nullptr, c0, 0, 0, rows,
                   rows_per_split, slab);
    } else {
        const dim3 grid = tn_grid(cdiv(P, 64) * cdiv(c0, 64), nsplits);
        FGC_LAUNCH(tag, st, gemm_tn_stream_kernel<4>, grid, dim3(256), 0, A, lda, P, x0, (const float*)nullptr, c0, 0, 0, rows,
                   rows_per_split, slab);
    }
    FGC_CHECK_LAUNCH("gemm_tn_stream_kernel");
    return FGC_OK;
}

int tn_rows_per_slab(int n, int splits) { return cdiv(cdiv(n, splits), 4) * 4; }

int tn_balanced_splits(int desired, int maxs, int rows) {
    desired = std::max(1, std::min(desired, maxs));
    for (int delta = 0; delta < 24; ++delta)
        for (int sgn = 1; sgn >= -1; sgn -= 2) {
            const int s = desired + sgn * delta;
            if (s >= 8 && s <= maxs && cdiv(rows, tn_rows_per_slab(rows, s)) % 8 == 0) return s;
        }
    return desired;
}

int tn_splits(int P, int Q, int rows) {
    const int tiles = cdiv(P, 64) * cdiv(Q, 64);
    const int slots = (int)opt(OPT_TN_SLOTS);
    int per = slots / tiles;
    if (per < 2) per = std::max(1, 2 * slots / tiles);
    return tn_balanced_splits(8 * per, cdiv(rows, 128), rows);
}

TnPlan tn_plan_of(bool bf16, bool vec4, bool stream_ok, const void* A, int PL, const void* x0, const void* x1, int c0, int c1,
                         int shift, int rows, int rps, float* slab, int lda) {
    TnPlan pl;
    const int cin = c0 + c1, ns = cdiv(rows, rps);
    pl.a = TnArgs{A, x0, x1, slab, lda ? lda : PL, PL, c0, c1, shift, rows, rps, 0};
    pl.nsplits = ns;
    if (bf16 && tn_bf16_ok(PL, c0, c1)) {
        pl.variant = cin % 64 == 0 ? TN_BF16_4 : TN_BF16_2;
        pl.ntiles = cdiv(PL, TNB_PC) * (cin % 64 == 0 ? cin / 64 : cin / 32);
    } else if (bf16 && cin <= 32 && c1 == 0) {
        pl.variant = TN_STREAM2_BF;
        pl.ntiles = cdiv(PL, 64);
    } else if (bf16) {
        pl.variant = TN_STREAM4_BF;
        pl.ntiles = cdiv(PL, 64) * cdiv(cin, 64);
    } else if (stream_ok && cin <= 32 && c1 == 0 && cin % 2 == 0) {
        pl.variant = TN_STREAM2;
        pl.ntiles = cdiv(PL, 64);
    } else if (stream_ok) {
        pl.variant = TN_STREAM4;
        pl.ntiles = cdiv(PL, 64) * cdiv(cin, 64);
    } else {
        pl.variant = vec4 ? TN_PLAIN_V4 : TN_PLAIN;
        pl.ntiles = cdiv(PL, 64) * cdiv(cin, 64);
    }
    return pl;
}
int tn_launch_one(const TnPlan& pl, const char* tag, hipStream_t st) {
    const TnArgs& a = pl.a;
    const dim3 grid = tn_grid(pl.ntiles, pl.nsplits);
    const float *A = (const float*)a.A, *x0 = (const float*)a.x0, *x1 = (const float*)a.x1;
    const unsigned short *A16 = (const unsigned short*)a.A, *h0 = (const unsigned short*)a.x0, *h1 = (const unsigned short*)a.x1;
    switch (pl.variant) {
        case TN_BF16_4: FGC_LAUNCH(tag, st, (gemm_tn_bf16_kernel<4>), grid, dim3(TNB_THREADS), 0, A16, a.lda, a.P, h0, h1, a.c0, a.c1, a.shift, a.rows, a.rps, a.slab); break;
        case TN_BF16_2: FGC_LAUNCH(tag, st, (gemm_tn_bf16_kernel<2>), grid, dim3(TNB_THREADS), 0, A16, a.lda, a.P, h0, h1, a.c0, a.c1, a.shift, a.rows, a.rps, a.slab); break;
        case TN_STREAM2_BF: FGC_LAUNCH(tag, st, (gemm_tn_stream_kernel<2, true>), grid, dim3(256), 0, A, a.lda, a.P, x0, x1, a.c0, a.c1, a.shift, a.rows, a.rps, a.slab); break;
        case TN_STREAM4_BF: FGC_LAUNCH(tag, st, (gemm_tn_stream_kernel<4, true>), grid, dim3(256), 0, A, a.lda, a.P, x0, x1, a.c0, a.c1, a.shift, a.rows, a.rps, a.slab); break;
        case TN_STREAM2: FGC_LAUNCH(tag, st, gemm_tn_stream_kernel<2>, grid, dim3(256), 0, A, a.lda, a.P, x0, x1, a.c0, a.c1, a.shift, a.rows, a.rps, a.slab); break;
        case TN_STREAM4: FGC_LAUNCH(tag, st, gemm_tn_stream_kernel<4>, grid, dim3(256), 0, A, a.lda, a.P, x0, x1, a.c0, a.c1, a.shift, a.rows, a.rps, a.slab); break;
        case TN_PLAIN_V4: FGC_LAUNCH(tag, st, (gemm_tn_kernel<true>), grid, dim3(256), 0, A, a.lda, a.P, x0, x1, a.c0, a.c1, a.shift, a.rows, a.rps, a.slab); break;
        default: FGC_LAUNCH(tag, st, (gemm_tn_kernel<false>), grid, dim3(256), 0, A, a.lda, a.P, x0, x1, a.c0, a.c1, a.shift, a.rows, a.rps, a.slab); break;
    }
    FGC_CHECK_LAUNCH("fgc_conv_bwd/dW");
    return FGC_OK;
}
int tn_launch_group(int variant, TnJobs& J, int nblocks, const char* tag, hipStream_t st) {
    if (J.njobs == 0) return FGC_OK;
    switch (variant) {
        case TN_BF16_4: FGC_LAUNCH(tag, st, (gemm_tn_bf16_group_kernel<4>), dim3(nblocks), dim3(TNB_THREADS), 0, J); break;
        case TN_BF16_2: FGC_LAUNCH(tag, st, (gemm_tn_bf16_group_kernel<2>), dim3(nblocks), dim3(TNB_THREADS), 0, J); break;
        case TN_STREAM2_BF: FGC_LAUNCH(tag, st, (gemm_tn_stream_group_kernel<2, true>), dim3(nblocks), dim3(256), 0, J); break;
        case TN_STREAM4_BF: FGC_LAUNCH(tag, st, (gemm_tn_stream_group_kernel<4, true>), dim3(nblocks), dim3(256), 0, J); break;
        case TN_STREAM2: FGC_LAUNCH(tag, st, (gemm_tn_stream_group_kernel<2>), dim3(nblocks), dim3(256), 0, J); break;
        default: FGC_LAUNCH(tag, st, (gemm_tn_stream_group_kernel<4>), dim3(nblocks), dim3(256), 0, J); break;
    }
    FGC_CHECK_LAUNCH("fgc_conv_bwd_reduce/dW");
    J.njobs = 0;
    return FGC_OK;
// ... 4 lines not shown
```

facet_graph_convolution_amd/net.py:

```python
import collections
import contextlib
import ctypes as C
import gc
import os
import warnings
import types

import numpy as np
import torch

from . import _lib, ops, require_graph_replay_safe
from ._lib import ConvDesc, ConvBwdIO, AG_LD, DL_LD, FGC_M
from .graph import FacetGraph, as_graph

LRELU_ALPHA = 0.1
STD_W, STD_B = 0.05, 0.01
HIDDEN = 1024
COST_SAMPLES = 4000
POINT_SAMPLES = 500
POINT_LOSS_THRESHOLD = 5000.0
VERTEX_ITERS = (80, 20, 20)


def param_spec(multi_scale=False, in_channels=6):
    M = FGC_M

    def conv(cin, cout):
        return [("weight", (M, cout, cin)), ("bias", (cout,)), ("assignment", (M, cin)), ("assignment", (M,)),
                ("assignment", (M, cin))]

    def lin(cin, cout):
        return [("weight", (cin, cout)), ("bias", (cout,))]

    spec = conv(in_channels, 32) + conv(32, 64) + conv(64, 128) + conv(128, 128)
    if multi_scale:
        spec += lin(128, HIDDEN) + lin(HIDDEN, 3)
    spec += conv(128, 64) + conv(128, 64)
    if multi_scale:
        spec += lin(64, HIDDEN) + lin(HIDDEN, 3)
    spec += conv(64, 32) + conv(64, 32) + lin(32, HIDDEN) + lin(HIDDEN, 3)
    return spec


class FlatParams:

    def __init__(self, spec, device):
        self.spec = spec
        self.offsets = []
        off = 0
        for _, shape in spec:
            self.offsets.append(off)
            off += (int(np.prod(shape)) + 3) // 4 * 4
        self.total = off
        self.device = torch.device(device)
        self.theta = torch.zeros(off, dtype=torch.float32, device=self.device)
        self.grad_ext = torch.zeros(off + 4, dtype=torch.float32, device=self.device)
        self.grad = self.grad_ext[:off]
        self.m = torch.zeros_like(self.theta)
        self.v = torch.zeros_like(self.theta)
        self.step = 0

    def _views(self, flat):
        return [flat[o:o + int(np.prod(s))].view(*s) for o, (_, s) in zip(self.offsets, self.spec)]

    @property
# ... 4 lines not shown
    def grads(self):
        return self._views(self.grad)

    def init_random(self, seed=0):
        rs = np.random.RandomState(seed)
        host = np.zeros(self.total, dtype=np.float32)
        for o, (kind, shape) in zip(self.offsets, self.spec):
            std = STD_B if kind == "bias" else STD_W
            host[o:o + int(np.prod(shape))] = rs.normal(0.0, std, size=shape).astype(np.float32).reshape(-1)
        self.theta.copy_(torch.from_numpy(host))

    def load(self, tensors):
        assert len(tensors) == len(self.spec)
        for view, t in zip(self.values, tensors):
            view.copy_(torch.as_tensor(t, dtype=torch.float32).reshape(view.shape))

    def num_parameters(self):
        return sum(int(np.prod(s)) for _, s in self.spec)


def _p(t):
    return C.c_void_p(t.data_ptr()) if t is not None else C.c_void_p(0)


_HIP = [None]


def _graph_node_count(g):
    if _HIP[0] is None:
        _HIP[0] = C.CDLL("libamdhip64.so")
    n = C.c_size_t(0)
    rc = _HIP[0].hipGraphGetNodes(C.c_void_p(g.raw_cuda_graph()), None, C.byref(n))
    if rc != 0:
        raise RuntimeError("hipGraphGetNodes failed (%d): cannot tell whether a schedule segment has launches" % rc)
    return int(n.value)


@contextlib.contextmanager
def _no_gc_while_capturing():
    if os.environ.get("FGC_NO_CAPTURE_GC_GUARD", "0") == "1":
        yield
        return
    gc.collect()
    was = gc.isenabled()
    gc.disable()
    try:
        yield
    finally:
        if was:
            gc.enable()


_ConvLayer = collections.namedtuple("_ConvLayer", "name level x0 x1 shift y pool act cout pidx", defaults=(None,))
TRUNK = (
    _ConvLayer("conv1", 0, "xr", None, 0, "h1", "p1", 1, 32),
    _ConvLayer("conv2", 1, "p1", None, 0, "h2", "p2", 1, 64),
    _ConvLayer("conv3", 2, "p2", None, 0, "h3", None, 1, 128),
    _ConvLayer("dconv3", 2, "h3", None, 0, "d3", None, 1, 128),
    _ConvLayer("upconv2", 1, "d3", None, 2, "u2", None, 0, 64),
    _ConvLayer("dconv2", 1, "u2", "h2", 0, "d2", None, 1, 64),
    _ConvLayer("upconv1", 0, "d2", None, 2, "u1", None, 0, 32),
    _ConvLayer("dconv1", 0, "u1", "h1", 0, "d1", None, 1, 32),
)


def r_ld(cout, r_pad, bf16):
    return _lib.lib().fgc_conv_r_ld(cout, 1 if r_pad else 0, 1 if bf16 else 0)


def plan_grouped_dw(ns, dtype, pairs, mode, max_r_bytes, windowed, training, r_pad=True):
    if mode == "0" or not training:
        return ()
    grouped = [TRUNK[0].name]
    for lay in ([] if windowed else TRUNK[1:]):
        cnt = ns[lay.level] * r_ld(lay.cout, r_pad, dtype == "bf16")
        used = cnt // 4 if (lay.shift == 2 and pairs) else cnt
        if mode == "1" or used * (2 if dtype == "bf16" else 4) <= max_r_bytes:
            grouped.append(lay.name)
    return tuple(grouped)


class FacetDenoiser:
    def __init__(self, device="cuda", multi_scale=False, in_channels=6, seed=0, dtype="f32", options=None):
        if not torch.cuda.is_available():
            raise RuntimeError("FacetDenoiser needs an MI355X (no CPU fallback)")
        if dtype not in ("f32", "bf16"):
            raise ValueError("dtype must be 'f32' or 'bf16' (storage of the activations; weights stay fp32)")
        self.dtype = dtype
        self.L = _lib.lib()
        self.option_overrides = _lib.option_overrides(**options) if options else None
        self.device = torch.device(device)
        self.multi_scale = multi_scale
        self.in_channels = in_channels
        self.params = FlatParams(param_spec(multi_scale, in_channels), self.device)
        self.params.init_random(seed)
        self._mesh = None
        self._mesh_cache = {}
        self.profile = False
        self.comm = None
        self.overlap = os.environ.get("FGC_NO_OVERLAP", "0") != "1"
        self.split_min_tiles = int(os.environ.get("FGC_SPLIT_MIN_TILES", "1024"))
        self.dw_in_window = os.environ.get("FGC_NO_DW_IN_WINDOW", "0") != "1"
        self.batched = os.environ.get("FGC_NO_BATCHED", "0") != "1"
        self.step_prologue = os.environ.get("FGC_NO_STEP_PROLOGUE", "0") != "1"
        self.grouped_dw_mode = os.environ.get("FGC_GROUPED_DW", "1" if dtype == "bf16" else "auto") if self.batched else "0"
        self.grouped_dw_forced = "FGC_GROUPED_DW" in os.environ
        self.grouped_dw_max_r_bytes = int(os.environ.get("FGC_GROUPED_DW_MAX_R_MB", "40")) << 20
        self.save_z = os.environ.get("FGC_NO_SAVE_Z", "0") != "1"
        self.r_pad = 0 if os.environ.get("FGC_NO_R_PAD", "0") == "1" else _lib.CONV_R_PAD
        self.fused_pool = os.environ.get("FGC_NO_FUSED_POOL", "0") != "1"
        self.fused_loss = os.environ.get("FGC_NO_FUSED_LOSS", "0") != "1"
        self.pairs = self._option("NO_PAIRS") != 1
        k = 0
        self.slot = {}
        for name in ["conv1", "conv2", "conv3", "dconv3"]:
            self.slot[name] = k
            k += 5
        if multi_scale:
            self.slot["head2"] = k
            k += 4
        for name in ["upconv2", "dconv2"]:
            self.slot[name] = k
            k += 5
        if multi_scale:
            self.slot["head1"] = k
            k += 4
        for name in ["upconv1", "dconv1"]:
            self.slot[name] = k
            k += 5
        self.slot["head0"] = k
        self.layers = [lay._replace(pidx=self.slot[lay.name]) for lay in TRUNK]

    def bind_mesh(self, x, adjs, gt=None, plan=None, comm=None):
        M = self._bind_inputs(x, adjs, plan, gt is not None)
        B = M["B"]
        B.update(self._bind_activations(M))
        scratch, M["grouped_dw_layers"] = self._bind_backward_scratch(M)
        B.update(scratch)
        B.update(self._bind_ground_truth(M, gt))
        layer_bufs, M["descs"], M["ios"], M["layer_flags"] = self._bind_layers(M)
        B.update(layer_bufs)
        self._bind_backward_wiring(M)
        mlp_bufs, M["arrays"] = self._bind_mlp_and_arrays(M)
        B.update(mlp_bufs)
        self._mesh = M
        self.comm = comm
        return self

    def _bind_inputs(self, x, adjs, plan, training):
        dev = self.device
        xt = torch.as_tensor(np.asarray(x.cpu() if isinstance(x, torch.Tensor) else x, dtype=np.float32))
        xt = xt.reshape(-1, xt.shape[-1]).contiguous()
        if xt.shape[1] != self.in_channels:
            raise ValueError("expected %d input channels" % self.in_channels)
        if plan is None:
            graphs = [as_graph(a, dev) for a in adjs]
            if len(graphs) != 3:
                raise ValueError("the network needs exactly 3 adjacency levels (model.py:858-931)")
            nh, nhp, n_total, own_lo = [0, 0, 0], [0, 0], [g.n for g in graphs], 0
        else:
            from .shard import LocalGraph
            graphs = [LocalGraph(P, dev) for P in plan.levels]
            nh = [g.n_halo for g in graphs]
            nhp = [graphs[0].pair.n_halo, graphs[1].pair.n_halo]
            n_total = list(plan.n_total)
            own_lo = plan.levels[0].lo
            xt = xt[torch.from_numpy(plan.local_rows(0))]
        n0, n1, n2 = ns = [g.n for g in graphs]
        if n0 != 4 * n1 or n1 != 4 * n2 or xt.shape[0] != n0 + nh[0]:
            raise ValueError("level sizes must be N0 = 4 N1 = 16 N2 and match x (got %d, %d, %d, x %d)" %
                             (n0, n1, n2, xt.shape[0]))
        B = {"x": xt.contiguous().to(dev)}
        B["xr"] = torch.empty_like(B["x"])
        self._alloc_step_inputs(B, COST_SAMPLES)
        mode = types.SimpleNamespace(clean=False, verts=False, gt_normals=False, synth_points=False)
        return dict(graphs=graphs, B=B, ns=ns, nh=nh, nhp=nhp, has_gt=training, plan=plan, n_total=n_total,
                    own_lo=own_lo, captured={}, mode=mode)

    def _bind_activations(self, M):
        (n0, n1, n2), nh, nhp = M["ns"], M["nh"], M["nhp"]
        f = dict(dtype=torch.float32, device=self.device)
        shapes = {"h1": (n0 + nh[0], 32), "p1": (n1 + nh[1], 32), "h2": (n1 + nh[1], 64), "p2": (n2 + nh[2], 64),
                  "h3": (n2 + nh[2], 128), "d3": (n2 + nhp[1], 128), "u2": (n1 + nh[1], 64), "d2": (n1 + nhp[0], 64),
                  "u1": (n0 + nh[0], 32), "d1": (n0, 32), "y0": (n0, 3), "nconv": (n0, 3)}
        act = dict(dtype=torch.bfloat16, device=self.device) if self.dtype == "bf16" else f
        B = {}
        for k, sh in shapes.items():
            kw = f if k in ("y0", "nconv") else act
            B[k] = torch.zeros(*sh, **kw)
            B["g_" + k] = torch.zeros(*sh, **kw)
        rows = dict({k: sh[0] for k, sh in shapes.items()}, xr=M["B"]["xr"].shape[0])
        for lay in self.layers:
            B["ag_" + lay.name] = torch.empty(rows[lay.x0], AG_LD, **f)
        if self.multi_scale:
            for k, nk in (("1", n1), ("2", n2)):
# ... 101 lines not shown
                else:
                    d.pair_rowptr = d.pair_col = d.pair_mul = d.hc = None
                    d.n_pairs = d.max_pair_deg = d.max_pair_in_deg = 0
                    pg = None
            B["wsf_" + lay.name] = torch.empty(self.L.fgc_conv_workspace_bytes(C.byref(d)) + 256, dtype=torch.uint8,
                                               device=dev)
            if training:
                B["wsb_" + lay.name] = torch.empty(self.L.fgc_conv_bwd_workspace_bytes(C.byref(d)) + 256,
                                                   dtype=torch.uint8, device=dev)
            trow, tcol, tedge = g.transposed()
            io = ConvBwdIO()
            io.trowptr, io.tcol, io.tedge = trow.data_ptr(), tcol.data_ptr(), tedge.data_ptr()
            io.max_in_deg = g.max_in_deg
            io.stages = 0
            io.ag, io.y, io.dy = A["ag_" + lay.name].data_ptr(), A[lay.y].data_ptr(), A["g_" + lay.y].data_ptr()
            io.ds, io.dl, io.dag = (A[k].data_ptr() for k in ("ds", "dl", "dag"))
            io.r = A.get("r_" + lay.name, A["r"]).data_ptr()
            io.r_ld = r_ld(lay.cout, self.r_pad, bf16)
            gW0, gb, gu, gc, gv = grads[lay.pidx:lay.pidx + 5]
            io.dW0, io.db, io.du, io.dc, io.dv = (t.data_ptr() for t in (gW0, gb, gu, gc, gv))
            if pg is not None:
                io.tpair_rowptr, io.tpair_col, io.tpair_edge = pg.trow.data_ptr(), pg.tcol.data_ptr(), pg.tedge.data_ptr()
                if training:
                    need = max(pg.n_pairs + getattr(pg, "n_cross_in", 0), 1) * d.cout
                    if "dt" not in B or B["dt"].numel() < need:
                        B["dt"] = torch.empty(need, **act)
                pair_ios.append(io)
            ios[lay.name] = io
        for io in pair_ios:
            io.dt = B["dt"].data_ptr() if "dt" in B else None
        return B, descs, ios, layer_flags

    def _bind_backward_wiring(self, M):
        B, descs, ios, layer_flags, training = M["B"], M["descs"], M["ios"], M["layer_flags"], M["has_gt"]
        for lay in self.layers[1:]:
            io = ios[lay.name]
            io.dx0 = B["g_" + lay.x0].data_ptr()
            io.dx1 = B["g_" + lay.x1].data_ptr() if lay.x1 else None
            io.accumulate0, io.accumulate1 = 0, 0
        ios["conv1"].dx0 = ios["conv1"].dx1 = None
        if self.fused_pool and training:
            ios["conv1"].pool_y, ios["conv1"].pool_dy = B["p1"].data_ptr(), B["g_p1"].data_ptr()
            ios["conv2"].pool_y, ios["conv2"].pool_dy = B["p2"].data_ptr(), B["g_p2"].data_ptr()
        if self.multi_scale and training and M["plan"] is None:
            ios["upconv2"].accumulate0 = 1
            ios["upconv1"].accumulate0 = 1
        if (layer_flags["conv1"] & _lib.CONV_SAVE_Z) and not self.L.fgc_conv_bwd_needs_exchange(
                C.byref(descs["conv1"]), C.byref(ios["conv1"])):
            ios["conv1"].z_saved = B["wsf_conv1"].data_ptr()
        else:
            layer_flags["conv1"] = descs["conv1"].flags = layer_flags["conv1"] & ~_lib.CONV_SAVE_Z
        if any(ios[n].r == B["r"].data_ptr() for n in M["grouped_dw_layers"] if n != "conv1"):
            raise RuntimeError("a layer that defers its weight-gradient GEMM shares the backward scratch r")

    def _bind_mlp_and_arrays(self, M):
        L, B, (n0, n1, n2) = self.L, M["B"], M["ns"]
        u8 = dict(dtype=torch.uint8, device=self.device)
        ws_b = L.fgc_mlp_bwd_workspace_bytes(n0, 32, HIDDEN, 3)
        if self.multi_scale:
            ws_b = max(ws_b, L.fgc_mlp_bwd_workspace_bytes(n1, 64, HIDDEN, 3), L.fgc_mlp_bwd_workspace_bytes(n2, 128, HIDDEN, 3))
        if self.dtype == "bf16":
            ws_b = max(ws_b, L.fgc_mlp_bwd_bf16_workspace_bytes(n0, 32, HIDDEN, 3))
        bufs = {"ws": torch.empty(max(L.fgc_mlp_workspace_bytes(128, HIDDEN, 3), ws_b) + 256, **u8)}
        bufs["ws_mlp_f"] = torch.empty(max(L.fgc_mlp_workspace_bytes(32, HIDDEN, 3),
                                           L.fgc_mlp_bf16_workspace_bytes(32, HIDDEN, 3)) + 256, **u8)
        names = [lay.name for lay in self.layers]
        nl = len(names)
        arrays = dict(
            descs=(C.POINTER(ConvDesc) * nl)(*[C.pointer(M["descs"][k]) for k in names]),
            ios=(C.POINTER(ConvBwdIO) * nl)(*[C.pointer(M["ios"][k]) for k in names]),
            wsf=(C.c_void_p * nl)(*[B["wsf_" + k].data_ptr() for k in names]),
            wsb=(C.c_void_p * nl)(*[B["wsb_" + k].data_ptr() for k in names]) if M["has_gt"] else None, count=nl)
        return bufs, arrays

    def _alloc_step_inputs(self, B, ns):
        B["step_in"] = B["step_in_own"] = torch.zeros(ns + 12, dtype=torch.int32, device=self.device)
        B["loss_scratch"] = torch.zeros(self.L.fgc_loss_step_scratch_floats(ns), dtype=torch.float32, device=self.device)
        B["loss_sums"] = torch.zeros(self.L.fgc_loss_shard_floats(ns), dtype=torch.float32, device=self.device)
        self._bind_step_inputs(B, B["step_in"])
        B["R"].copy_(torch.eye(3, dtype=torch.float32).reshape(9))

    @staticmethod
    def _bind_step_inputs(B, row):
        ns = row.numel() - 12
        B["step_in"] = row
        B["sample_ind"] = row[:ns]
        B["R"] = row[ns:ns + 9].view(torch.float32)
        B["noise"] = row[ns + 9:ns + 12]

    def _own_step_inputs(self):
        B = self._mesh["B"]
        own = B["step_in_own"]
        if B["step_in"] is not own:
            own.copy_(B["step_in"])
            self._bind_step_inputs(B, own)

    def _cached(self, key, bind, max_bytes=64 << 30):
        cache = self._mesh_cache
        if key in cache:
            self._mesh = cache[key]
            return self._mesh
        bind()
        used = sum(sum(t.numel() * t.element_size() for t in m["B"].values()) for m in cache.values())
        mine = sum(t.numel() * t.element_size() for t in self._mesh["B"].values())
        if used + mine <= max_bytes:
            cache[key] = self._mesh
# ... 376 lines not shown
                sk = torch.remainder(B["sample_ind"], nk)
                B["sample_ind" + k] = sk
                _lib.check(L.fgc_angular_loss_fwd(_p(nc), _p(gtk), _p(sk), sk.numel(), _p(B["loss" + k]), st), "loss")
                _lib.check(L.fgc_angular_loss_bwd(_p(nc), _p(gtk), _p(sk), sk.numel(), nk, _p(B["loss" + k]), 1.0,
                                                  _p(B["g_nconv" + k]), st), "loss bwd")
                _lib.check(L.fgc_normalize_bwd(_p(y), _p(B["g_nconv" + k]), nk, _p(B["g_y" + k]), _p(sc), st),
                           "normalize bwd")
                self._coarse_head_bwd(k)
        yield from self._params_backward_gen(fused)

    def _coarse_head_bwd(self, k):
        M, L, st = self._mesh, self.L, self._st()
        B, ws = M["B"], M["B"]["ws"]
        vals, grads = self.params.values, self.params.grads
        name, head = {"2": ("dconv3", "head2"), "1": ("dconv2", "head1")}[k]
        nk = M["ns"][int(k)]
        lay = next(l for l in self.layers if l.name == name)
        xin = B[lay.y]
        hs = self.slot[head]
        _lib.check(L.fgc_mlp_bwd(_p(xin), _p(B["g_y" + k]), nk, xin.shape[1], HIDDEN, 3, _p(vals[hs]),
                                 _p(vals[hs + 1]), _p(vals[hs + 2]), LRELU_ALPHA, _p(B["g_" + lay.y]),
                                 _p(grads[hs]), _p(grads[hs + 1]), _p(grads[hs + 2]), _p(grads[hs + 3]), 0, _p(ws),
                                 ws.numel(), st), head + " bwd")

    def _params_backward_gen(self, fused):
        M, L, st = self._mesh, self.L, self._st()
        B, ws, ns = M["B"], M["B"]["ws"], M["ns"]
        n0 = ns[0]
        vals, grads = self.params.values, self.params.grads
        s = self.slot["head0"]
        self._tag("bwd:mlp")
        _lib.check(self._mlp_bwd(_p(B["d1"]), _p(B["g_y0"]), n0, 32, HIDDEN, 3, _p(vals[s]), _p(vals[s + 1]),
                                 _p(vals[s + 2]), LRELU_ALPHA, _p(B["g_d1"]), _p(grads[s]), _p(grads[s + 1]),
                                 _p(grads[s + 2]), _p(grads[s + 3]), M.get("mlp_packed", 0), _p(ws), ws.numel(), st),
                   "head0 bwd")
        pending_dw = [None]

        def flush_dw():
            if pending_dw[0] is not None:
                pending_dw[0]()
                pending_dw[0] = None

        def defer_dw(name, d, io, lws, flags):
            def run():
                self._tag("bwd:" + name)
                io.stages, io.flags = 8, flags
                io.data_tile_list, io.n_data_tiles = None, 0
                _lib.check(L.fgc_conv_bwd(C.byref(d), C.byref(io), _p(lws), lws.numel(), st), name + " bwd/weights")
                io.flags = 0
            pending_dw[0] = run
            if not self.dw_in_window:
                flush_dw()

        for name in ["dconv1", "upconv1", "dconv2", "upconv2", "dconv3", "conv3", "conv2", "conv1"]:
            self._tag("bwd:" + name)
            if name == "conv2" and not self.fused_pool:
                _lib.check(self._pool4_bwd(_p(B["h2"]), _p(B["p2"]), _p(B["g_p2"]), _p(B["g_h2"]), ns[2], 64, 1, st),
                           "pool2 bwd")
            if name == "conv1" and not self.fused_pool:
                _lib.check(self._pool4_bwd(_p(B["h1"]), _p(B["p1"]), _p(B["g_p1"]), _p(B["g_h1"]), ns[1], 32, 1, st),
                           "pool1 bwd")
            d, io = M["descs"][name], M["ios"][name]
            lws = B["wsb_" + name]
            base = (_lib.CONV_PACKED | _lib.CONV_DEFER_REDUCE) if self.batched else 0
            if self.batched and name in M["grouped_dw_layers"]:
                base |= _lib.CONV_DEFER_DW
            if not self.sharded:
                io.stages, io.flags = 0, base
                _lib.check(L.fgc_conv_bwd(C.byref(d), C.byref(io), _p(lws), lws.numel(), st), name + " bwd")
                continue
            lay = next(l for l in self.layers if l.name == name)
            cout = d.cout
            nloc = ns[lay.level] + M["nh"][lay.level]
            g = M["graphs"][lay.level]
            call = lambda what: _lib.check(L.fgc_conv_bwd(C.byref(d), C.byref(io), _p(lws), lws.numel(), st),
                                           name + " bwd/" + what)
            io.flags = base
            if not L.fgc_conv_bwd_needs_exchange(C.byref(d), C.byref(io)):
                flush_dw()
                self._tag("bwd:" + name)
                io.stages = 1 | 2 | 8
                call("params")
                continue
            pair = L.fgc_conv_uses_pairs(C.byref(d))
            io.stages = 1 | 2
            call("pair logits" if pair else "logits")
            if pair:
                pg = g.pair
                npl = pg.n_pairs + pg.n_cross_in
                items = [("pedges", lay.level, B["dt"][:npl * cout].view(npl, cout)),
                         ("pedges", lay.level, B["dl"][:npl * DL_LD].view(npl, DL_LD))]
                tiles, min_tiles, what = pg.tiles, self.pair_split_min_tiles, "pair data"
            else:
                ds_rows = (B["ds"].view(torch.bfloat16) if self.dtype == "bf16" else B["ds"])[:nloc * cout].view(nloc, cout)
                items = [("rows", lay.level, ds_rows, False), ("edges", lay.level)]
                tiles, min_tiles, what = g.tiles, self.split_min_tiles, "data"
            if self.overlap and tiles["ttiles_int"][1] >= min_tiles:
                yield ("xchg", items, "bwd")
                flush_dw()
                self._tag("bwd:" + name)
                io.stages, io.flags = 4, base | _lib.CONV_PACKED
                io.data_tile_list, io.n_data_tiles = tiles["ttiles_int"][0].data_ptr(), tiles["ttiles_int"][1]
                call(what + "/interior")
                yield ("wait", "bwd")
                io.data_tile_list, io.n_data_tiles = tiles["ttiles_bnd"][0].data_ptr(), tiles["ttiles_bnd"][1]
                call(what + "/boundary")
                io.data_tile_list, io.n_data_tiles, io.flags = None, 0, 0
            else:
                key = "bwd" if pending_dw[0] is not None else None
                yield ("xchg", items, key)
                flush_dw()
                if key:
                    yield ("wait", key)
                self._tag("bwd:" + name)
                io.stages, io.flags = 4, base | _lib.CONV_PACKED
                call(what)
                io.flags = 0
            defer_dw(name, d, io, lws, base | _lib.CONV_PACKED)
        flush_dw()
        if self.batched:
            A = M["arrays"]
# ... 582 lines not shown
```

include/fgc.h:

```cpp
#ifndef FGC_H
#define FGC_H

#include <stddef.h>
#include <stdint.h>

#ifdef __cplusplus
extern "C" {
#endif

#define FGC_M 9
#define FGC_AG_LD 24
#define FGC_DL_LD 12

#define FGC_OK 0
#define FGC_EINVAL (-22)
#define FGC_ENOMEM (-12)
#define FGC_EHIP (-5)

#define FGC_ABI_VERSION 112

const char* fgc_last_error(void);
int fgc_version(void);
int fgc_set_option(const char* name, int64_t value);
int fgc_get_option(const char* name, int64_t* value);
int32_t fgc_option_count(void);
const char* fgc_option_name(int32_t index);
size_t fgc_struct_size(int32_t which);

int fgc_profile_enable(int on);
int fgc_profile_tag(const char* tag);
int fgc_profile_collect(char* buf, int32_t buf_bytes);


int fgc_csr_from_klist(const int32_t* adj_h, int32_t n, int32_t K, int32_t* rowptr_h, int32_t* col_h,
                       int64_t* nnz_out);
int fgc_klist_from_csr(const int32_t* rowptr_h, const int32_t* col_h, int32_t n, int32_t K, int32_t* adj_h);
int fgc_csr_transpose(const int32_t* rowptr_h, const int32_t* col_h, int32_t n, int32_t* trowptr_h,
                      int32_t* tcol_h, int32_t* tedge_h);
int fgc_pair_graph(const int32_t* rowptr_h, const int32_t* col_h, int32_t n, int32_t* prow_h, int32_t* pcol_h,
                   uint32_t* pmul_h, int64_t* n_pairs_out);


int fgc_face_features(const float* V_h, int32_t nv, const uint32_t* F_h, int32_t nf, float* normals_h,
                      double* centres_h);
int fgc_faces_large_adj(const uint32_t* F_h, int32_t nf, int32_t nv, int32_t K, int32_t* adj_h,
                        int64_t* unregistered);
int fgc_metis_one_level(const int32_t* rr_h, const int32_t* cc_h, const float* vv_h, int64_t nnz,
                        const int64_t* rid_h, const float* weights_h, int32_t N, int32_t* cluster_id_h,
                        double* total_assoc);
typedef struct fgc_hierarchy fgc_hierarchy;
int fgc_hierarchy_build(const int32_t* adj_h, int32_t n, int32_t K, const double* pos_h, const float* normals_h,
                        int32_t levels, uint64_t seed, const int32_t* const* parents_h,
                        const int32_t* parents_len_h, fgc_hierarchy** out);
void fgc_hierarchy_free(fgc_hierarchy* h);
int32_t fgc_hierarchy_size(const fgc_hierarchy* h, int32_t level);
int32_t fgc_hierarchy_real_size(const fgc_hierarchy* h, int32_t level);
int fgc_hierarchy_new_to_old(const fgc_hierarchy* h, int32_t level, int32_t* out_h);
int fgc_hierarchy_parents(const fgc_hierarchy* h, int32_t level, int32_t* out_h);
int fgc_hierarchy_klist(const fgc_hierarchy* h, int32_t level, int32_t K, int32_t* adj_h, int32_t* saturated);

int fgc_graph_patch(const int32_t* adj_h, int32_t n, int32_t K, int32_t nodes_num, int32_t seed, const int8_t* mask_h,
                    int32_t min_patch_size, int32_t* patch_adj_h, int32_t* old_index_h, int32_t* patch_n,
                    int32_t* next_seed);

int fgc_mesh_patch(const float* V_h, int32_t nv, const int32_t* F_h, int32_t nf, const int32_t* adj_h, int32_t K,
                   int32_t face_num, int32_t seed, float* v_out_h, int32_t v_cap, int32_t* f_out_h, int32_t* adj_out_h,
                   int32_t* v_old_h, int32_t* f_old_h, int32_t* n_v, int32_t* n_f);

int fgc_vertices_faces(const int32_t* faces_h, int32_t nf, int32_t nv, int32_t k_v, int32_t* v_faces_h);

int fgc_edge_map(const uint32_t* faces_h, int32_t nf, int32_t nv, int32_t max_edges, int32_t* e_map_h,
                 int32_t* n_edges, int32_t* v_e_map_h);
// ... 5 lines not shown
} fgc_option_override;

typedef struct fgc_conv_desc {
    int32_t n;
    int32_t nnz;
    const int32_t* rowptr;
    const int32_t* col;
    const float* x0;
    const float* x1;
    int32_t c0, c1;
    int32_t shift;
    int32_t cout;
    const float* W0;
    const float* b;
    const float* u;
    const float* c;
    const float* v;
    int32_t bias_mask;
    int32_t act;
    float alpha;
    int32_t src_rows;
    int32_t max_deg;
    const int32_t* tile_list;
    int32_t n_tiles;
    int32_t proj_row0;
    int32_t proj_rows;
    int32_t flags;
    const int32_t* pair_rowptr;
    const int32_t* pair_col;
    const uint32_t* pair_mul;
    int32_t n_pairs;
    int32_t max_pair_deg;
    int32_t max_pair_in_deg;
    float* hc;
    const fgc_option_override* options;
    int32_t n_options;
    int32_t reserved1;
    uint64_t packed_layout;
} fgc_conv_desc;

#define FGC_CONV_PACKED 1
#define FGC_CONV_DEFER_REDUCE 2
#define FGC_CONV_DEFER_DW 16
#define FGC_CONV_R_PAD 32
#define FGC_CONV_SAVE_Z 4

#define FGC_CONV_BF16 8

size_t fgc_conv_workspace_bytes(const fgc_conv_desc* d);

int fgc_conv_fwd(const fgc_conv_desc* d, float* ag, float* y, float* y_pool, void* workspace,
                 size_t workspace_bytes, void* stream);

typedef struct fgc_conv_bwd_io {
    const int32_t* trowptr;
    const int32_t* tcol;
    const int32_t* tedge;
    int32_t max_in_deg;
    int32_t stages;
    const float* ag;
    const float* y;
    const float* dy;
    float* ds;
    float* dl;
    float* dag;
    float* r;
    float* dx0;
    float* dx1;
    int32_t accumulate0, accumulate1;
    float* dW0;
    float* db;
    float* du;
    float* dc;
    float* dv;
    const int32_t* data_tile_list;
    int32_t n_data_tiles;
    int32_t flags;
    const float* z_saved;
    const float* pool_y;
    const float* pool_dy;
    const int32_t* tpair_rowptr;
    const int32_t* tpair_col;
    const int32_t* tpair_edge;
    float* dt;
    int32_t r_ld;
    int32_t reserved0;
} fgc_conv_bwd_io;

size_t fgc_conv_bwd_workspace_bytes(const fgc_conv_desc* d);
int32_t fgc_conv_r_ld(int32_t cout, int32_t padded, int32_t bf16);
int fgc_conv_bwd_needs_exchange(const fgc_conv_desc* d, const fgc_conv_bwd_io* io);
int fgc_conv_uses_pairs(const fgc_conv_desc* d);
int fgc_conv_pairs_allowed(int64_t rows, int64_t n_pairs, int32_t max_pair_in_deg, int32_t cout);
uint64_t fgc_conv_layout_id(const fgc_conv_desc* d);
int fgc_conv_bwd(const fgc_conv_desc* d, const fgc_conv_bwd_io* io, void* workspace, size_t workspace_bytes,
                 void* stream);
int fgc_conv_forms(const fgc_conv_desc* d, const fgc_conv_bwd_io* io, char* buf, int32_t buf_bytes);

typedef struct fgc_pack_extra {
    const float* rot_x;
    float* rot_y;
    const float* rot_R;
    int64_t rot_rows;
    int32_t rot_vecs;
    float* rot_ag;
    const float* rot_u;
    const float* rot_c;
    const float* rot_v;
    int32_t mlp_bf16;
    const float* mlp_W1;
    const float* mlp_W2;
    int32_t mlp_n, mlp_cin, mlp_hidden, mlp_cout;
    void* mlp_fwd_ws;
    void* mlp_bwd_ws;
} fgc_pack_extra;

int fgc_conv_pack(const fgc_conv_desc* const* descs, const fgc_conv_bwd_io* const* ios, void* const* fwd_ws,
                  void* const* bwd_ws, int32_t count, const fgc_pack_extra* extra, void* stream);
int fgc_conv_bwd_reduce(const fgc_conv_desc* const* descs, const fgc_conv_bwd_io* const* ios, void* const* bwd_ws,
                        int32_t count, void* stream);

#define FGC_MLP_PACKED 1
#define FGC_MLP_LAYOUT(id) ((int32_t)(id) << 8)
int32_t fgc_mlp_layout_id(int32_t cin, int32_t hidden, int32_t cout, int32_t bf16);
int32_t fgc_mlp_num_partials(int32_t n);
size_t fgc_mlp_workspace_bytes(int32_t cin, int32_t hidden, int32_t cout);
size_t fgc_mlp_bwd_workspace_bytes(int32_t n, int32_t cin, int32_t hidden, int32_t cout);
int fgc_mlp_fwd(const float* x, int32_t n, int32_t cin, int32_t hidden, int32_t cout, const float* W1,
                const float* b1, const float* W2, const float* b2, float alpha, float* y, float* abs_partial,
                int32_t flags, void* workspace, size_t workspace_bytes, void* stream);
int fgc_mlp_bwd(const float* x, const float* dy, int32_t n, int32_t cin, int32_t hidden, int32_t cout,
                const float* W1, const float* b1, const float* W2, float alpha, float* dx, float* dW1,
                float* db1, float* dW2, float* db2, int32_t flags, void* workspace, size_t workspace_bytes, void* stream);

size_t fgc_mlp_bf16_workspace_bytes(int32_t cin, int32_t hidden, int32_t cout);
size_t fgc_mlp_bwd_bf16_workspace_bytes(int32_t n, int32_t cin, int32_t hidden, int32_t cout);
int fgc_mlp_fwd_bf16(const void* x, int32_t n, int32_t cin, int32_t hidden, int32_t cout, const float* W1,
                     const float* b1, const float* W2, const float* b2, float alpha, float* y, float* abs_partial,
// ... 142 lines not shown
```

Before: 64.48 million facets/s.

## Run deferred weight-gradient GEMM blocks as riders inside later backward logits kernels

Adds a carry mechanism so that an earlier layer's deferred dW GEMM (TN stream variant) runs as extra workgroups appended to the grid of the next layer's backward logits kernel, either the deep half-tile kernel or the pair kernel. Host blocks and rider blocks share one launch, and any remaining GEMM blocks launch right after. The aim is to fill idle CUs in small, latency-bound logits launches and to remove separate GEMM launches and tail effects. In exchange it adds ABI fields, LDS sizing changes, a lower launch bound (occupancy) on the riding pair kernel, and overlap checks on the shared r buffer.

```diff
diff --git a/facet_graph_convolution_amd/_lib.py b/facet_graph_convolution_amd/_lib.py
--- a/facet_graph_convolution_amd/_lib.py
+++ b/facet_graph_convolution_amd/_lib.py
@@ -6,7 +6,7 @@
 _HERE = os.path.dirname(os.path.abspath(__file__))
 LIB_PATH = os.environ.get("FGC_LIB", os.path.join(_HERE, "csrc", "libfgc.so"))
 
-ABI_VERSION = 112
+ABI_VERSION = 113
 FGC_M = 9
 AG_LD = 24
 DL_LD = 12
@@ -60,8 +60,14 @@
         ("data_tile_list", C.c_void_p), ("n_data_tiles", C.c_int32), ("flags", C.c_int32),
         ("z_saved", C.c_void_p), ("pool_y", C.c_void_p), ("pool_dy", C.c_void_p),
         ("tpair_rowptr", C.c_void_p), ("tpair_col", C.c_void_p), ("tpair_edge", C.c_void_p), ("dt", C.c_void_p),
-        ("r_ld", C.c_int32), ("reserved0", C.c_int32),
+        ("r_ld", C.c_int32),
+        ("dw_begin", C.c_int32),
+        ("carry", C.c_void_p), ("n_carry", C.c_int32), ("reserved0", C.c_int32),
     ]
+
+
+class DwCarry(C.Structure):
+    _fields_ = [("desc", C.c_void_p), ("io", C.c_void_p), ("workspace", C.c_void_p), ("flags", C.c_int32), ("reserved", C.c_int32)]
 
 
 class PackExtra(C.Structure):
@@ -81,6 +87,7 @@
 CONV_SAVE_Z = 4
 CONV_BF16 = 8
 CONV_R_PAD = 32
+DW_CARRY_LAST = 1
 SYNTH_ON = 0x80000000
 
 
diff --git a/facet_graph_convolution_amd/csrc/fgc_common.h b/facet_graph_convolution_amd/csrc/fgc_common.h
--- a/facet_graph_convolution_amd/csrc/fgc_common.h
+++ b/facet_graph_convolution_amd/csrc/fgc_common.h
@@ -87,7 +87,11 @@
     X(NO_MLP_SPLIT, 0)                              \
     X(NO_MLP_BWD_SPLIT, 0)                                                                         \
     X(NO_K1_SPLIT, 0)                         \
-    X(NO_BFM, 0)
+    X(NO_BFM, 0)                 \
+    X(NO_DW_RIDE, 0)                                \
+    X(DW_RIDE_DEEP, 480)             \
+    X(DW_RIDE_PAIR64, 480)                                    \
+    X(DW_RIDE_PAIR32, 0)
 enum Opt {
 #define FGC_OPT_ENUM(name, def) OPT_##name,
     FGC_OPTION_LIST(FGC_OPT_ENUM)
diff --git a/facet_graph_convolution_amd/csrc/fgc_conv_bwd.hip b/facet_graph_convolution_amd/csrc/fgc_conv_bwd.hip
--- a/facet_graph_convolution_amd/csrc/fgc_conv_bwd.hip
+++ b/facet_graph_convolution_amd/csrc/fgc_conv_bwd.hip
@@ -8,7 +8,7 @@
 #include "fgc_conv_bwd.h"
 #include "fgc_conv_narrow.h"
 #include "fgc_conv_pair.h"
-#include "fgc_gemm_tn.h"
+#include "fgc_gemm_tn_dev.h"
 #include "fgc_reduce.h"
 #include "fgc_split.h"
 
@@ -508,9 +508,15 @@
     }
 }
 
-template <bool LONG, int OKG, int NT_ = 32, int NPW_ = 8, bool SPLIT = false>
-__global__ __launch_bounds__((NT_ / NPW_) * 64, NT_ == 32 ? 2 : 4) void conv_bwd_logits_deep_kernel(CoreParams p, LogitParams lp) {
+struct DwRide {
+    int nb_host, host_blocks;
+    TnJobs J;
+};
+template <bool LONG, int OKG, int NT_ = 32, int NPW_ = 8, bool SPLIT = false, typename... RIDE>
+__global__ __launch_bounds__((NT_ / NPW_) * 64, NT_ == 32 ? 2 : 4) void conv_bwd_logits_deep_kernel(CoreParams p, LogitParams lp,
+                                                                                                    RIDE... ride) {
     static_assert((NT_ == 32 && NPW_ == 8) || (NT_ == 16 && NPW_ == 4 && !LONG), "tile shapes");
+    static_assert(sizeof...(RIDE) == 0 || (NT_ == 16 && !SPLIT), "riders: 256-thread half-tile form");
     static_assert(!SPLIT || (NT_ == 16 && OKG == 2), "split dz GEMM: half tiles of the 32-wide layers");
     constexpr int TILE = NT_, NPW = NPW_, NWV = NT_ / NPW_, NTHREADS = NWV * 64, RT = NT_ / 16, LPN = NTHREADS / NT_;
     static_assert(NWV == 4, "four waves either way: the column-tile split and the dc sums below assume it");
@@ -521,7 +527,17 @@
     const int ostride = OKG ? OKG * 16 + 8 : lp.ostride;
     float* dst = s.extra;
     float* red = dst + ((LONG && lp.a_global) ? 0 : TILE * ostride);
-    const int tile0 = xcd_tile(blockIdx.x, gridDim.x) * TILE;
+    unsigned nblocks = gridDim.x;
+    if constexpr (sizeof...(RIDE) > 0) {
+        const DwRide& R = (ride, ...);
+        if ((int)blockIdx.x >= R.host_blocks) {
+            tn_group_block<4, false>(R.J, (int)blockIdx.x - R.host_blocks, reinterpret_cast<float(*)[64][65]>(smem_raw));
+            return;
+        }
+        if ((int)blockIdx.x >= R.nb_host) return;
+        nblocks = (unsigned)R.nb_host;
+    }
+    const int tile0 = xcd_tile(blockIdx.x, nblocks) * TILE;
     const int tid = threadIdx.x;
     const int wave = tid >> 6, lane = tid & 63, lr = lane & 15, lq = lane >> 4;
 
@@ -1404,12 +1420,20 @@
 }
 
 static int launch_k1(const BwdPlan& w, const BwdCall& c, const fgc_conv_desc* d, const CoreParams& p, const LogitParams& lp,
-                     hipStream_t st) {
+                     hipStream_t st, const TnJobs* riders = nullptr, int rider_blocks = 0) {
     const int nt = w.k1_nodes, cout = d->cout;
     const int qs = ((w.k1 == K1_DEEP || w.k1 == K1_BF16) && !w.k1_long) ? 16 : KMAX;
     const size_t core = smem_core_bytes(w.k1 == K1_BF16 ? ZSTRIDE_BF / 2 : w.g1.zstride, qs, nt);
     const size_t tile = w.k1 == K1_BF16 ? (size_t)nt * (cout * 2 + 32) : lp.a_global ? 0 : (size_t)nt * lp.ostride * 4;
     LaunchCfg cfg{"conv_bwd_logits_deep_kernel", "fgc_conv_bwd/logits_mfma", st, cdiv(d->n, nt), NTHREADS, core + tile + 48 * 4};
+    if (riders && rider_blocks > 0) {
+        FGC_CHECK_ARG(c.k1 == K1_DEEP && w.k1_half && !w.k1_split && c.okg == 8, "fgc_conv_bwd: no riding form of this d-logits kernel");
+        const int nb_host = cfg.grid, hb = cdiv(nb_host, 8) * 8;
+        cfg.name = "conv_bwd_logits_deep_kernel+dW";
+        cfg.grid = hb + rider_blocks;
+        cfg.smem = std::max(cfg.smem, (size_t)TN_LDS_BYTES);
+        return launch_kernel<conv_bwd_logits_deep_kernel<false, 8, 16, 4, false, DwRide>>(cfg, p, lp, DwRide{nb_host, hb, *riders});
+    }
     switch (c.k1) {
         case K1_BF16:
             cfg.name = "conv_bwd_logits_bf16_kernel";
@@ -1485,6 +1509,99 @@
     p.n_tiles = io->n_data_tiles;
     if (f.kind == DATA_W8) f.w8 = w8_form(p, &ep, f.max_deg, w.bf16);
     return f;
+}
+
+constexpr int RIDE_MAX_CARRY = TN_MAX_JOBS;
+struct RidePlan {
+    TnJobs J;
+    int blocks;
+    int n;
+    int new_begin[RIDE_MAX_CARRY];
+    TnPlan rest[RIDE_MAX_CARRY];
+    int rest_blocks[RIDE_MAX_CARRY];
+};
+static int ride_capacity(const BwdPlan& w, const BwdCall& c, const fgc_conv_desc* d) {
+    if (opt(OPT_NO_DW_RIDE) == 1 || w.bf16 || c.narrow_path) return 0;
+    int cap = 0;
+    if (w.pairs) cap = d->cout == 64 ? (int)opt(OPT_DW_RIDE_PAIR64) : d->cout == 32 ? (int)opt(OPT_DW_RIDE_PAIR32) : 0;
+    else if (c.k1 == K1_DEEP && w.k1_half && !w.k1_split && c.okg == 8) cap = (int)opt(OPT_DW_RIDE_DEEP);
+    return std::max(0, cap) / 8 * 8;
+}
+static bool ranges_overlap(const void* a, size_t abytes, const void* b, size_t bbytes) {
+    const uintptr_t a0 = (uintptr_t)a, b0 = (uintptr_t)b;
+    return a0 < b0 + bbytes && b0 < a0 + abytes;
+}
+static int plan_riders(const fgc_conv_desc* d, const fgc_conv_bwd_io* io, const BwdPlan& w, const BwdCall& c, RidePlan& rp) {
+    rp.J.njobs = 0;
+    rp.blocks = 0;
+    rp.n = 0;
+    if (!io->carry || io->n_carry <= 0 || !(c.stages & 2)) return FGC_OK;
+    FGC_CHECK_ARG(io->n_carry <= RIDE_MAX_CARRY, "fgc_conv_bwd: n_carry = %d (at most %d)", io->n_carry, RIDE_MAX_CARRY);
+    FGC_CHECK_ARG(!c.narrow_path, "fgc_conv_bwd: a first layer on the narrow path carries no weight-gradient GEMM");
+    int cap = ride_capacity(w, c, d);
+    const bool writes_r = (c.stages & 4) != 0;
+    const size_t host_r_bytes = (size_t)w.nred * io_r_ld(io, d->cout, w.bf16) * (w.bf16 ? 2 : 4);
+    for (int i = 0; i < io->n_carry; ++i) {
+        const fgc_dw_carry& e = io->carry[i];
+        FGC_CHECK_ARG(e.desc && e.io && e.workspace && e.io != io, "fgc_conv_bwd: carry %d: null descriptor / io / workspace", i);
+        FGC_OPT_SCOPE(e.desc);
+        const int rc = validate_conv_desc(e.desc, "fgc_conv_bwd/carry");
+        if (rc) return rc;
+        const BwdPlan we = plan_bwd(e.desc, (char*)e.workspace);
+        FGC_CHECK_ARG(!(e.io->dx0 == nullptr && we.narrow), "fgc_conv_bwd: carry %d: the first layer's GEMM cannot be carried", i);
+        FGC_CHECK_ARG((e.io->flags & FGC_CONV_DEFER_DW) && e.io->r && io_r_ld_ok(e.io, e.desc->cout, we.bf16),
+                      "fgc_conv_bwd: carry %d: the layer did not defer its weight-gradient GEMM (FGC_CONV_DEFER_DW), or has no r", i);
+        const TnPlan pl = layer_tn_plan(e.desc, e.io, we);
+        const int total = (int)tn_grid(pl.ntiles, pl.nsplits).x;
+        int begin = e.io->dw_begin;
+        FGC_CHECK_ARG(begin >= 0 && begin <= total && begin % 8 == 0, "fgc_conv_bwd: carry %d: dw_begin = %d outside [0, %d] or not a "
+                      "multiple of 8", i, begin, total);
+        if (pl.variant == TN_STREAM4 && cap > 0 && begin < total && rp.J.njobs < TN_MAX_JOBS) {
+            const int take = std::min(total - begin, cap);
+            TnArgs a = pl.a;
+            a.block0 = rp.blocks;
+            a.first = begin;
+            rp.J.job[rp.J.njobs++] = a;
+            rp.blocks += take;
+            cap -= take;
+            begin += take;
+        }
+        rp.rest_blocks[i] = 0;
+        if ((e.flags & FGC_DW_CARRY_LAST) && begin < total) {
+            FGC_CHECK_ARG(tn_groupable(pl.variant) || begin == 0, "fgc_conv_bwd: carry %d: a GEMM of this form runs in one piece", i);
+            rp.rest[i] = pl;
+            rp.rest[i].a.first = begin;
+            rp.rest_blocks[i] = total - begin;
+            begin = total;
+        }
+        FGC_CHECK_ARG(begin == total || !writes_r ||
+                      !ranges_overlap(e.io->r, (size_t)we.nred * io_r_ld(e.io, e.desc->cout, we.bf16) * (we.bf16 ? 2 : 4), io->r,
+                                      host_r_bytes),
+                      "fgc_conv_bwd: carry %d: %d of %d workgroups of its weight-gradient GEMM would still be pending when this "
+                      "call's data kernel overwrites the r they read (set FGC_DW_CARRY_LAST)", i, total - begin, total);
+        rp.new_begin[i] = begin;
+        rp.n = i + 1;
+    }
+    return FGC_OK;
+}
+static int finish_riders(const fgc_conv_bwd_io* io, RidePlan& rp, hipStream_t st) {
+    for (int i = 0; i < rp.n; ++i) {
+        if (rp.rest_blocks[i] > 0) {
+            int rc;
+            if (tn_groupable(rp.rest[i].variant)) {
+                TnJobs G;
+                G.njobs = 1;
+                G.job[0] = rp.rest[i].a;
+                G.job[0].block0 = 0;
+                rc = tn_launch_group(rp.rest[i].variant, G, rp.rest_blocks[i], "gemm_tn_kernel:dW", st);
+            } else {
+                rc = tn_launch_one(rp.rest[i], "gemm_tn_kernel:dW", st);
+            }
+            if (rc) return rc;
+        }
+        io->carry[i].io->dw_begin = rp.new_begin[i];
+    }
+    return FGC_OK;
 }
 
 }
@@ -1559,6 +1676,13 @@
         put("k1_okg", "%d", c.okg);
         put("k1_aglobal", "%d", (int)c.a_global);
         put("k1_vec4", "%d", (int)c.k1_vec4);
+        RidePlan rp;
+        rc = plan_riders(d, io, w, c, rp);
+        if (rc) return rc;
+        int rest = 0;
+        for (int i = 0; i < rp.n; ++i) rest += rp.rest_blocks[i];
+        put("k1_ride", "%d", rp.blocks);
+        put("k1_ride_rest", "%d", rest);
     } else {
         put("k1", "%s", k1_names[w.k1]);
     }
@@ -1616,6 +1740,9 @@
     hipStream_t st = (hipStream_t)stream;
     const BwdCall c = bwd_call(w, d, io);
     const int stages = c.stages;
+    RidePlan rp;
+    rc = plan_riders(d, io, w, c, rp);
+    if (rc) return rc;
     const bool pack_here = !(io->flags & FGC_CONV_PACKED);
     PackJob pjobs[2];
     size_t ptotals[2];
@@ -1632,7 +1759,9 @@
             if (rc) return rc;
         }
         if (stages & 3) {
-            rc = launch_pair_bwd_logits(d, io, w.db_part, w.dc_part, st);
+            rc = launch_pair_bwd_logits(d, io, w.db_part, w.dc_part, st, &rp.J, rp.blocks);
+            if (rc) return rc;
+            rc = finish_riders(io, rp, st);
             if (rc) return rc;
         }
         if (stages & 4) {
@@ -1693,7 +1822,9 @@
                 lp.pool_dy = io->pool_dy;
             }
             lp.a_global = c.a_global;
-            rc = launch_k1(w, c, d, p, lp, st);
+            rc = launch_k1(w, c, d, p, lp, st, &rp.J, rp.blocks);
+            if (rc) return rc;
+            rc = finish_riders(io, rp, st);
             if (rc) return rc;
         }
         if ((stages & 4) && !(io->data_tile_list && io->n_data_tiles == 0)) {
@@ -1768,7 +1899,12 @@
                               "fgc_conv_bwd_reduce: layer %d: r_ld = %d is not a row stride of r for cout = %d", i, io->r_ld, d->cout);
                 pl = layer_tn_plan(d, io, w);
             }
+            const int total = (int)tn_grid(pl.ntiles, pl.nsplits).x, done = io->dw_begin;
+            FGC_CHECK_ARG(done >= 0 && done <= total && done % 8 == 0, "fgc_conv_bwd_reduce: layer %d: dw_begin = %d outside [0, %d] or "
+                          "not a multiple of 8", i, done, total);
+            if (done == total) continue;
             if (!tn_groupable(pl.variant)) {
+                FGC_CHECK_ARG(done == 0, "fgc_conv_bwd_reduce: layer %d: a GEMM of this form runs in one piece", i);
                 rc = tn_launch_one(pl, "gemm_tn_kernel:dW", st);
                 if (rc) return rc;
                 continue;
@@ -1780,8 +1916,9 @@
                 nb[pl.variant] = 0;
             }
             pl.a.block0 = nb[pl.variant];
+            pl.a.first = done;
             J.job[J.njobs++] = pl.a;
-            nb[pl.variant] += (int)tn_grid(pl.ntiles, pl.nsplits).x;
+            nb[pl.variant] += total - done;
         }
         for (int v = 0; v < TN_NVARIANTS; ++v) {
             rc = tn_launch_group(v, G[v], nb[v], "gemm_tn_kernel:dW", st);
diff --git a/facet_graph_convolution_amd/csrc/fgc_conv_pair.h b/facet_graph_convolution_amd/csrc/fgc_conv_pair.h
--- a/facet_graph_convolution_amd/csrc/fgc_conv_pair.h
+++ b/facet_graph_convolution_amd/csrc/fgc_conv_pair.h
@@ -1,5 +1,6 @@
 #pragma once
 #include "fgc_common.h"
+#include "fgc_gemm_tn.h"
 
 namespace fgc {
 
@@ -12,6 +13,6 @@
 }
 int launch_pair_fwd(const fgc_conv_desc* d, float* ag, float* y, void* workspace, hipStream_t st);
 int launch_pair_bwd_logits(const fgc_conv_desc* d, const fgc_conv_bwd_io* io, float* db_part, float* dc_part,
-                           hipStream_t st);
+                           hipStream_t st, const TnJobs* riders = nullptr, int rider_blocks = 0);
 
 }
diff --git a/facet_graph_convolution_amd/csrc/fgc_conv_pair.hip b/facet_graph_convolution_amd/csrc/fgc_conv_pair.hip
--- a/facet_graph_convolution_amd/csrc/fgc_conv_pair.hip
+++ b/facet_graph_convolution_amd/csrc/fgc_conv_pair.hip
@@ -2,6 +2,7 @@
 
 #include "fgc_conv_core.h"
 #include "fgc_conv_pair.h"
+#include "fgc_gemm_tn_dev.h"
 
 namespace fgc {
 
@@ -418,14 +419,32 @@
     return v;
 }
 
-template <int COUT, bool BF>
-__global__ __launch_bounds__(256, FGC_PAIR_LB_BWD) void pair_bwd_logits_kernel(PairParams p) {
+struct PairRide {
+    int nb_host, host_blocks;
+    TnJobs J;
+};
+template <int COUT, bool BF, typename... RIDE>
+__global__ __launch_bounds__(256, sizeof...(RIDE) > 0 ? 3 : FGC_PAIR_LB_BWD) void pair_bwd_logits_kernel(PairParams p, RIDE... ride) {
     constexpr int LPB = COUT / 4, BPW = 64 / LPB, BPG = 4 * BPW;
     constexpr int RED_LD = COUT + 12;
-    __shared__ __attribute__((aligned(16))) float qs[BPG * PQ_STRIDE];
-    __shared__ __attribute__((aligned(16))) float red[BPG * RED_LD];
+    constexpr bool RIDING = sizeof...(RIDE) > 0;
+    static_assert(!RIDING || !BF, "riders: fp32 storage");
+    constexpr int HOST_FLOATS = BPG * PQ_STRIDE + BPG * RED_LD;
+    __shared__ __attribute__((aligned(16))) float qs[RIDING ? (HOST_FLOATS * 4 > TN_LDS_BYTES ? HOST_FLOATS : TN_LDS_BYTES / 4) : BPG * PQ_STRIDE];
+    __shared__ __attribute__((aligned(16))) float red_own[RIDING ? 4 : BPG * RED_LD];
+    float* const red = RIDING ? qs + BPG * PQ_STRIDE : red_own;
     const int wave = threadIdx.x >> 6, lane = threadIdx.x & 63, bl = lane / LPB, kl = lane % LPB;
-    const int wg = xcd_tile(blockIdx.x, gridDim.x);
+    unsigned nblocks = gridDim.x;
+    if constexpr (RIDING) {
+        const PairRide& R = (ride, ...);
+        if ((int)blockIdx.x >= R.host_blocks) {
+            tn_group_block<4, false>(R.J, (int)blockIdx.x - R.host_blocks, reinterpret_cast<float(*)[64][65]>(qs));
+            return;
+        }
+        if ((int)blockIdx.x >= R.nb_host) return;
+        nblocks = (unsigned)R.nb_host;
+    }
+    const int wg = xcd_tile(blockIdx.x, nblocks);
     const int b = (wg * 4 + wave) * BPW + bl;
     const bool valid = b < p.nb;
     const int bc = min(b, p.nb - 1);
@@ -610,7 +629,8 @@
     return FGC_OK;
 }
 
-int launch_pair_bwd_logits(const fgc_conv_desc* d, const fgc_conv_bwd_io* io, float* db_part, float* dc_part, hipStream_t st) {
+int launch_pair_bwd_logits(const fgc_conv_desc* d, const fgc_conv_bwd_io* io, float* db_part, float* dc_part, hipStream_t st,
+                           const TnJobs* riders, int rider_blocks) {
     PairParams p{};
     p.nb = d->n >> 2;
     p.prow = d->pair_rowptr;
@@ -632,6 +652,13 @@
     p.dt_bytes = (unsigned)((size_t)d->n_pairs * d->cout * ((d->flags & FGC_CONV_BF16) ? 2 : 4));
     p.dl_bytes = (unsigned)((size_t)d->n_pairs * FGC_DL_LD * 4);
     const int grid = pair_num_wgs(d);
+    if (riders && rider_blocks > 0) {
+        const int hb = cdiv(grid, 8) * 8;
+        if (d->cout == 32) FGC_LAUNCH("pair_bwd_logits_kernel+dW", st, (pair_bwd_logits_kernel<32, false, PairRide>), dim3(hb + rider_blocks), dim3(256), 0, p, PairRide{grid, hb, *riders});
+        else FGC_LAUNCH("pair_bwd_logits_kernel+dW", st, (pair_bwd_logits_kernel<64, false, PairRide>), dim3(hb + rider_blocks), dim3(256), 0, p, PairRide{grid, hb, *riders});
+        FGC_CHECK_LAUNCH("fgc_conv_bwd/pair_logits+dW");
+        return FGC_OK;
+    }
     if (d->flags & FGC_CONV_BF16) {
         if (d->cout == 32) FGC_LAUNCH("pair_bwd_logits_kernel", st, (pair_bwd_logits_kernel<32, true>), dim3(grid), dim3(256), 0, p);
         else FGC_LAUNCH("pair_bwd_logits_kernel", st, (pair_bwd_logits_kernel<64, true>), dim3(grid), dim3(256), 0, p);
diff --git a/facet_graph_convolution_amd/csrc/fgc_gemm_tn.h b/facet_graph_convolution_amd/csrc/fgc_gemm_tn.h
--- a/facet_graph_convolution_amd/csrc/fgc_gemm_tn.h
+++ b/facet_graph_convolution_amd/csrc/fgc_gemm_tn.h
@@ -10,6 +10,7 @@
     float* slab;
     int lda, P, c0, c1, shift, rows, rps;
     int block0;
+    int first;
 };
 constexpr int TN_MAX_JOBS = 8;
 struct TnJobs {
diff --git a/facet_graph_convolution_amd/csrc/fgc_gemm_tn.hip b/facet_graph_convolution_amd/csrc/fgc_gemm_tn.hip
--- a/facet_graph_convolution_amd/csrc/fgc_gemm_tn.hip
+++ b/facet_graph_convolution_amd/csrc/fgc_gemm_tn.hip
@@ -1,6 +1,6 @@
 #include <algorithm>
 
-#include "fgc_gemm_tn.h"
+#include "fgc_gemm_tn_dev.h"
 
 namespace fgc {
 
@@ -27,21 +27,6 @@
             else if (q < Q) b[t] = x1[sr * c1 + (q - c0)];
         }
     }
-}
-
-__device__ __forceinline__ bool tn_block(int ntiles, int nsplits, int& tile, int& split, int vblock = -1) {
-    const int L = vblock >= 0 ? vblock : (int)blockIdx.x, xcd = L & 7, idx = L >> 3;
-    tile = idx % ntiles;
-    split = (idx / ntiles) * 8 + xcd;
-    return split < nsplits;
-}
-
-__device__ __forceinline__ int tn_job_of(const TnJobs& J) {
-    int q = 0;
-#pragma unroll
-    for (int t = 1; t < TN_MAX_JOBS; ++t)
-        if (t < J.njobs && (int)blockIdx.x >= J.job[t].block0) q = t;
-    return q;
 }
 
 template <bool VEC4>
@@ -101,271 +86,18 @@
     }
 }
 
-template <int NJ, bool BF>
-__device__ __forceinline__ void tn_stream_body(const float* __restrict__ A, int lda, int P, const float* __restrict__ x0,
-                                               const float* __restrict__ x1, int c0, int c1, int shift, int rows,
-                                               int rows_per_split, float* __restrict__ slab, int vblock,
-                                               float (*red)[64][65]) {
-    const int Q = c0 + c1;
-    const int npt = (P + 63) >> 6;
-    int tile_id, split_id;
-    if (!tn_block(npt * ((Q + 16 * NJ - 1) / (16 * NJ)), (rows + rows_per_split - 1) / rows_per_split, tile_id, split_id, vblock))
-        return;
-    const int pt = tile_id % npt, qt = tile_id / npt;
-    const int p0 = pt * 64, q0 = qt * (16 * NJ);
-    const int tid = threadIdx.x, lane = tid & 63, lr = lane & 15, lq = lane >> 4;
-    const int wave = __builtin_amdgcn_readfirstlane(tid >> 6);
-    const int r_begin = split_id * rows_per_split;
-    const int r_end = min(rows, r_begin + rows_per_split);
-    const int nsteps = (r_end - r_begin + 3) >> 2;
-    const int pc = min(p0 + 4 * lr, P - 4);
-    const int qc = min(q0 + NJ * lr, Q - NJ);
-    const float* bsrc = BF ? reinterpret_cast<const float*>(reinterpret_cast<const unsigned short*>(qc < c0 ? x0 : x1) +
-                                                            (qc < c0 ? qc : qc - c0))
-                           : (qc < c0 ? x0 + qc : x1 + (qc - c0));
-    const int bld = qc < c0 ? c0 : c1;
-    f32x4 acc[4][NJ];
-#pragma unroll
-    for (int i = 0; i < 4; ++i)
-#pragma unroll
-        for (int j = 0; j < NJ; ++j) acc[i][j] = f32x4{0.f, 0.f, 0.f, 0.f};
-
-    auto ld = [&](int step, f32x4& a, f32x4& b, int& row) {
-        row = r_begin + 4 * step + lq;
-        const int rc = min(row, r_end - 1);
-        if constexpr (BF) {
-            const unsigned short* A16 = reinterpret_cast<const unsigned short*>(A);
-            const unsigned short* b16 = reinterpret_cast<const unsigned short*>(bsrc);
-            a = bf4_to_f4(*reinterpret_cast<const u32x2*>(A16 + (size_t)rc * lda + pc));
-            if constexpr (NJ == 4) {
-                b = bf4_to_f4(*reinterpret_cast<const u32x2*>(b16 + (size_t)(rc >> shift) * bld));
-            } else {
-                const f32x2c b2 = bf2_to_f2(*reinterpret_cast<const unsigned*>(b16 + (size_t)(rc >> shift) * bld));
-                b = f32x4{b2[0], b2[1], 0.f, 0.f};
-            }
-            return;
-        }
-        a = *reinterpret_cast<const f32x4*>(A + (size_t)rc * lda + pc);
-        if constexpr (NJ == 4) {
-            b = *reinterpret_cast<const f32x4*>(bsrc + (size_t)(rc >> shift) * bld);
-        } else {
-            const f32x2c b2 = *reinterpret_cast<const f32x2c*>(bsrc + (size_t)(rc >> shift) * bld);
-            b = f32x4{b2[0], b2[1], 0.f, 0.f};
-        }
-    };
-    auto mm = [&](f32x4 a, const f32x4& b, int row) {
-        if (row >= r_end) a = f32x4{0.f, 0.f, 0.f, 0.f};
-#pragma unroll
-        for (int i = 0; i < 4; ++i)
-#pragma unroll
-            for (int j = 0; j < NJ; ++j) acc[i][j] = __builtin_amdgcn_mfma_f32_16x16x4f32(a[i], b[j], acc[i][j], 0, 0, 0);
-    };
-    f32x4 a0, b0, a1, b1, a2, b2, a3, b3;
-    int r0, r1, r2, r3;
-    ld(wave, a0, b0, r0);
-    ld(wave + 4, a1, b1, r1);
-    ld(wave + 8, a2, b2, r2);
-    ld(wave + 12, a3, b3, r3);
-#define FGC_TN_STEP(A_, B_, R_, NEXT_)          \
-    mm(A_, B_, R_);                             \
-    __builtin_amdgcn_sched_barrier(0);          \
-    ld(NEXT_, A_, B_, R_);                      \
-    __builtin_amdgcn_sched_barrier(0);
-    for (int s = wave; s < nsteps; s += 16) {
-        FGC_TN_STEP(a0, b0, r0, s + 16)
-        FGC_TN_STEP(a1, b1, r1, s + 20)
-        FGC_TN_STEP(a2, b2, r2, s + 24)
-        FGC_TN_STEP(a3, b3, r3, s + 28)
-    }
-#undef FGC_TN_STEP
-    auto put = [&](int slot) {
-#pragma unroll
-        for (int i = 0; i < 4; ++i)
-#pragma unroll
-            for (int j = 0; j < NJ; ++j)
-#pragma unroll
-                for (int t = 0; t < 4; ++t) red[slot][4 * (lq * 4 + t) + i][NJ * lr + j] = acc[i][j][t];
-    };
-    auto add = [&](int slot) {
-#pragma unroll
-        for (int i = 0; i < 4; ++i)
-#pragma unroll
-            for (int j = 0; j < NJ; ++j)
-#pragma unroll
-                for (int t = 0; t < 4; ++t) acc[i][j][t] += red[slot][4 * (lq * 4 + t) + i][NJ * lr + j];
-    };
-    if (wave == 1) put(0);
-    if (wave == 3) put(1);
-    __syncthreads();
-    if (wave == 0) add(0);
-    if (wave == 2) add(1);
-    __syncthreads();
-    if (wave == 0) put(0);
-    if (wave == 2) put(1);
-    __syncthreads();
-    float* out = slab + (size_t)split_id * P * Q;
-    for (int t = tid; t < 64 * 16 * NJ; t += 256) {
-        const int pp = t / (16 * NJ), qq = t % (16 * NJ);
-        if (p0 + pp < P && q0 + qq < Q) out[(size_t)(p0 + pp) * Q + q0 + qq] = red[0][pp][qq] + red[1][pp][qq];
-    }
-}
-
-__device__ __forceinline__ bool tn_direct_ok(int lda, int c0, int c1, int shift, int rows_per_split) {
-    return (c1 == 0 || (c0 & 31) == 0) && shift <= 4 &&
-           (long long)(rows_per_split + 160) * max(lda, max(c0, c1)) < (1ll << 29);
-}
-
-template <int NJ>
-__device__ __forceinline__ void tn_direct_body(const float* __restrict__ A, int lda, int P, const float* __restrict__ x0,
-                                               const float* __restrict__ x1, int c0, int c1, int shift, int rows,
-                                               int rows_per_split, float* __restrict__ slab, int vblock, f32x4* red) {
-    constexpr int NH = NJ / 2;
-    const int Q = c0 + c1;
-    const int npt = (P + 63) >> 6;
-    int tile_id, split_id;
-    if (!tn_block(npt * ((Q + 16 * NJ - 1) / (16 * NJ)), (rows + rows_per_split - 1) / rows_per_split, tile_id, split_id, vblock))
-        return;
-    const int pt = tile_id % npt, qt = tile_id / npt;
-    const int p0 = pt * 64, q0 = qt * (16 * NJ);
-    const int tid = threadIdx.x, lane = tid & 63, lr = lane & 15, lq = lane >> 4;
-    const int wave = __builtin_amdgcn_readfirstlane(tid >> 6);
-    const int r_begin = split_id * rows_per_split;
-    const int r_end = min(rows, r_begin + rows_per_split);
-    const int nsteps = (r_end - r_begin + 3) >> 2;
-    const int row0 = 4 * wave + lq;
-    const int pc = min(p0 + 4 * lr, P - 4);
-    const __amdgpu_buffer_rsrc_t a_rs = __builtin_amdgcn_make_buffer_rsrc(
-        const_cast<float*>(A + (size_t)r_begin * lda), 0, (r_end - r_begin) * lda * 4, 0x00020000);
-    unsigned ao = (unsigned)(row0 * lda + pc) * 4u;
-    const unsigned astep = 16u * (unsigned)lda * 4u;
-    const int xr0 = r_begin >> shift, xrows = ((rows - 1) >> shift) + 1;
-    const int xrow0 = ((r_begin + row0) >> shift) - xr0;
-    __amdgpu_buffer_rsrc_t b_rs[NH];
-    unsigned bo[NH], bstep[NH];
-#pragma unroll
-    for (int h = 0; h < NH; ++h) {
-        const int hs = q0 + 32 * h;
-        const bool first = hs < c0 || c1 == 0;
-        const int ld = first ? c0 : c1;
-        const size_t bytes = (size_t)(xrows - xr0) * ld * 4;
-        b_rs[h] = __builtin_amdgcn_make_buffer_rsrc(const_cast<float*>((first ? x0 : x1) + (size_t)xr0 * ld), 0,
-                                                    (int)(unsigned)std::min<size_t>(bytes, 0xffffffffu), 0x00020000);
-        bo[h] = (unsigned)(xrow0 * ld + min(hs + 2 * lr, Q - 2) - (first ? 0 : c0)) * 4u;
-        bstep[h] = (unsigned)((16 >> shift) * ld) * 4u;
-    }
-    f32x4 acc[4][NJ];
-#pragma unroll
-    for (int i = 0; i < 4; ++i)
-#pragma unroll
-        for (int j = 0; j < NJ; ++j) acc[i][j] = f32x4{0.f, 0.f, 0.f, 0.f};
-
-    struct Set {
-        f32x4 a;
-        f32x2c b[NH];
-    };
-    auto ld = [&](Set& s) {
-        s.a = __builtin_bit_cast(f32x4, __builtin_amdgcn_raw_buffer_load_b128(a_rs, ao, 0, 0));
-        ao += astep;
-        asm volatile("" : "+v"(ao));
-#pragma unroll
-        for (int h = 0; h < NH; ++h) {
-            s.b[h] = __builtin_bit_cast(f32x2c, __builtin_amdgcn_raw_buffer_load_b64(b_rs[h], bo[h], 0, 0));
-            bo[h] += bstep[h];
-            asm volatile("" : "+v"(bo[h]));
-        }
-    };
-    auto mm = [&](const Set& s) {
-#pragma unroll
-        for (int i = 0; i < 4; ++i)
-#pragma unroll
-            for (int j = 0; j < NJ; ++j)
-                acc[i][j] = __builtin_amdgcn_mfma_f32_16x16x4f32(s.a[i], s.b[j >> 1][j & 1], acc[i][j], 0, 0, 0);
-    };
-    if (wave < nsteps) {
-        Set s0, s1, s2, s3;
-        ld(s0);
-        __builtin_amdgcn_sched_barrier(0);
-        ld(s1);
-        __builtin_amdgcn_sched_barrier(0);
-        ld(s2);
-        __builtin_amdgcn_sched_barrier(0);
-        ld(s3);
-        __builtin_amdgcn_sched_barrier(0);
-#define FGC_TN_STEP(S_)                         \
-    mm(S_);                                     \
-    __builtin_amdgcn_sched_barrier(0);          \
-    ld(S_);                                     \
-    __builtin_amdgcn_sched_barrier(0);
-        int s = wave;
-        do {
-            FGC_TN_STEP(s0)
-            FGC_TN_STEP(s1)
-            FGC_TN_STEP(s2)
-            FGC_TN_STEP(s3)
-            s += 16;
-        } while (s < nsteps);
-    }
-#undef FGC_TN_STEP
-    auto put = [&](int slot) {
-#pragma unroll
-        for (int e = 0; e < 4 * NJ; ++e) red[(slot * 4 * NJ + e) * 64 + lane] = acc[e / NJ][e % NJ];
-    };
-    auto add = [&](int slot) {
-#pragma unroll
-        for (int e = 0; e < 4 * NJ; ++e) acc[e / NJ][e % NJ] += red[(slot * 4 * NJ + e) * 64 + lane];
-    };
-    if (wave == 1) put(0);
-    if (wave == 3) put(1);
-    __syncthreads();
-    if (wave == 0) add(0);
-    if (wave == 2) {
-        add(1);
-        put(1);
-    }
-    __syncthreads();
-    if (wave != 0) return;
-    add(1);
-    const __amdgpu_buffer_rsrc_t c_rs =
-        __builtin_amdgcn_make_buffer_rsrc(slab + (size_t)split_id * P * Q, 0, P * Q * 4, 0x00020000);
-#pragma unroll
-    for (int h = 0; h < NH; ++h) {
-        const int q = q0 + 32 * h + 2 * lr;
-        const unsigned co = q < Q ? (unsigned)((p0 + 16 * lq) * Q + q) * 4u : 0x80000000u;
-#pragma unroll
-        for (int t = 0; t < 4; ++t)
-#pragma unroll
-            for (int i = 0; i < 4; ++i)
-                __builtin_amdgcn_raw_buffer_store_b64(__builtin_bit_cast(u32x2, f32x2c{acc[i][2 * h][t], acc[i][2 * h + 1][t]}), c_rs,
-                                                      co + (unsigned)((4 * t + i) * Q) * 4u, 0, 0);
-    }
-}
-
-template <int NJ, bool BF>
-__device__ __forceinline__ void tn_stream_any(const float* __restrict__ A, int lda, int P, const float* __restrict__ x0,
-                                              const float* __restrict__ x1, int c0, int c1, int shift, int rows,
-                                              int rows_per_split, float* __restrict__ slab, int vblock) {
-    __shared__ __attribute__((aligned(16))) float red[2][64][65];
-    if constexpr (!BF) {
-        if (tn_direct_ok(lda, c0, c1, shift, rows_per_split)) {
-            tn_direct_body<NJ>(A, lda, P, x0, x1, c0, c1, shift, rows, rows_per_split, slab, vblock,
-                               reinterpret_cast<f32x4*>(&red[0][0][0]));
-            return;
-        }
-    }
-    tn_stream_body<NJ, BF>(A, lda, P, x0, x1, c0, c1, shift, rows, rows_per_split, slab, vblock, red);
-}
 template <int NJ, bool BF = false>
 __global__ __launch_bounds__(256, 4) void gemm_tn_stream_kernel(const float* __restrict__ A, int lda, int P,
                                                                 const float* __restrict__ x0,
                                                                 const float* __restrict__ x1, int c0, int c1, int shift,
                                                                 int rows, int rows_per_split, float* __restrict__ slab) {
-    tn_stream_any<NJ, BF>(A, lda, P, x0, x1, c0, c1, shift, rows, rows_per_split, slab, -1);
+    __shared__ __attribute__((aligned(16))) float red[2][64][65];
+    tn_stream_any<NJ, BF>(A, lda, P, x0, x1, c0, c1, shift, rows, rows_per_split, slab, -1, red);
 }
 template <int NJ, bool BF = false>
 __global__ __launch_bounds__(256, 4) void gemm_tn_stream_group_kernel(TnJobs J) {
-    const TnArgs& a = J.job[tn_job_of(J)];
-    tn_stream_any<NJ, BF>((const float*)a.A, a.lda, a.P, (const float*)a.x0, (const float*)a.x1, a.c0, a.c1, a.shift, a.rows,
-                          a.rps, a.slab, (int)blockIdx.x - a.block0);
+    __shared__ __attribute__((aligned(16))) float red[2][64][65];
+    tn_group_block<NJ, BF>(J, (int)blockIdx.x, red);
 }
 
 constexpr int TNB_THREADS = 256;
@@ -486,9 +218,9 @@
 }
 template <int QT>
 __global__ __launch_bounds__(TNB_THREADS, 2) void gemm_tn_bf16_group_kernel(TnJobs J) {
-    const TnArgs& a = J.job[tn_job_of(J)];
+    const TnArgs& a = J.job[tn_job_of(J, (int)blockIdx.x)];
     tn_bf16_body<QT>((const unsigned short*)a.A, a.lda, a.P, (const unsigned short*)a.x0, (const unsigned short*)a.x1, a.c0, a.c1,
-                     a.shift, a.rows, a.rps, a.slab, (int)blockIdx.x - a.block0);
+                     a.shift, a.rows, a.rps, a.slab, (int)blockIdx.x - a.block0 + a.first);
 }
 
 bool tn_bf16_ok(int P, int c0, int c1) {
@@ -536,7 +268,7 @@
                          int shift, int rows, int rps, float* slab, int lda) {
     TnPlan pl;
     const int cin = c0 + c1, ns = cdiv(rows, rps);
-    pl.a = TnArgs{A, x0, x1, slab, lda ? lda : PL, PL, c0, c1, shift, rows, rps, 0};
+    pl.a = TnArgs{A, x0, x1, slab, lda ? lda : PL, PL, c0, c1, shift, rows, rps, 0, 0};
     pl.nsplits = ns;
     if (bf16 && tn_bf16_ok(PL, c0, c1)) {
         pl.variant = cin % 64 == 0 ? TN_BF16_4 : TN_BF16_2;
diff --git a/facet_graph_convolution_amd/csrc/fgc_gemm_tn_dev.h b/facet_graph_convolution_amd/csrc/fgc_gemm_tn_dev.h
--- /dev/null
+++ b/facet_graph_convolution_amd/csrc/fgc_gemm_tn_dev.h
@@ -0,0 +1,284 @@
+#pragma once
+#include <algorithm>
+
+#include "fgc_gemm_tn.h"
+
+namespace fgc {
+
+__device__ __forceinline__ bool tn_block(int ntiles, int nsplits, int& tile, int& split, int vblock = -1) {
+    const int L = vblock >= 0 ? vblock : (int)blockIdx.x, xcd = L & 7, idx = L >> 3;
+    tile = idx % ntiles;
+    split = (idx / ntiles) * 8 + xcd;
+    return split < nsplits;
+}
+
+__device__ __forceinline__ int tn_job_of(const TnJobs& J, int block) {
+    int q = 0;
+#pragma unroll
+    for (int t = 1; t < TN_MAX_JOBS; ++t)
+        if (t < J.njobs && block >= J.job[t].block0) q = t;
+    return q;
+}
+
+template <int NJ, bool BF>
+__device__ __forceinline__ void tn_stream_body(const float* __restrict__ A, int lda, int P, const float* __restrict__ x0,
+                                               const float* __restrict__ x1, int c0, int c1, int shift, int rows,
+                                               int rows_per_split, float* __restrict__ slab, int vblock,
+                                               float (*red)[64][65]) {
+    const int Q = c0 + c1;
+    const int npt = (P + 63) >> 6;
+    int tile_id, split_id;
+    if (!tn_block(npt * ((Q + 16 * NJ - 1) / (16 * NJ)), (rows + rows_per_split - 1) / rows_per_split, tile_id, split_id, vblock))
+        return;
+    const int pt = tile_id % npt, qt = tile_id / npt;
+    const int p0 = pt * 64, q0 = qt * (16 * NJ);
+    const int tid = threadIdx.x, lane = tid & 63, lr = lane & 15, lq = lane >> 4;
+    const int wave = __builtin_amdgcn_readfirstlane(tid >> 6);
+    const int r_begin = split_id * rows_per_split;
+    const int r_end = min(rows, r_begin + rows_per_split);
+    const int nsteps = (r_end - r_begin + 3) >> 2;
+    const int pc = min(p0 + 4 * lr, P - 4);
+    const int qc = min(q0 + NJ * lr, Q - NJ);
+    const float* bsrc = BF ? reinterpret_cast<const float*>(reinterpret_cast<const unsigned short*>(qc < c0 ? x0 : x1) +
+                                                            (qc < c0 ? qc : qc - c0))
+                           : (qc < c0 ? x0 + qc : x1 + (qc - c0));
+    const int bld = qc < c0 ? c0 : c1;
+    f32x4 acc[4][NJ];
+#pragma unroll
+    for (int i = 0; i < 4; ++i)
+#pragma unroll
+        for (int j = 0; j < NJ; ++j) acc[i][j] = f32x4{0.f, 0.f, 0.f, 0.f};
+
+    auto ld = [&](int step, f32x4& a, f32x4& b, int& row) {
+        row = r_begin + 4 * step + lq;
+        const int rc = min(row, r_end - 1);
+        if constexpr (BF) {
+            const unsigned short* A16 = reinterpret_cast<const unsigned short*>(A);
+            const unsigned short* b16 = reinterpret_cast<const unsigned short*>(bsrc);
+            a = bf4_to_f4(*reinterpret_cast<const u32x2*>(A16 + (size_t)rc * lda + pc));
+            if constexpr (NJ == 4) {
+                b = bf4_to_f4(*reinterpret_cast<const u32x2*>(b16 + (size_t)(rc >> shift) * bld));
+            } else {
+                const f32x2c b2 = bf2_to_f2(*reinterpret_cast<const unsigned*>(b16 + (size_t)(rc >> shift) * bld));
+                b = f32x4{b2[0], b2[1], 0.f, 0.f};
+            }
+            return;
+        }
+        a = *reinterpret_cast<const f32x4*>(A + (size_t)rc * lda + pc);
+        if constexpr (NJ == 4) {
+            b = *reinterpret_cast<const f32x4*>(bsrc + (size_t)(rc >> shift) * bld);
+        } else {
+            const f32x2c b2 = *reinterpret_cast<const f32x2c*>(bsrc + (size_t)(rc >> shift) * bld);
+            b = f32x4{b2[0], b2[1], 0.f, 0.f};
+        }
+    };
+    auto mm = [&](f32x4 a, const f32x4& b, int row) {
+        if (row >= r_end) a = f32x4{0.f, 0.f, 0.f, 0.f};
+#pragma unroll
+        for (int i = 0; i < 4; ++i)
+#pragma unroll
+            for (int j = 0; j < NJ; ++j) acc[i][j] = __builtin_amdgcn_mfma_f32_16x16x4f32(a[i], b[j], acc[i][j], 0, 0, 0);
+    };
+    f32x4 a0, b0, a1, b1, a2, b2, a3, b3;
+    int r0, r1, r2, r3;
+    ld(wave, a0, b0, r0);
+    ld(wave + 4, a1, b1, r1);
+    ld(wave + 8, a2, b2, r2);
+    ld(wave + 12, a3, b3, r3);
+#define FGC_TN_STEP(A_, B_, R_, NEXT_)          \
+    mm(A_, B_, R_);                             \
+    __builtin_amdgcn_sched_barrier(0);          \
+    ld(NEXT_, A_, B_, R_);                      \
+    __builtin_amdgcn_sched_barrier(0);
+    for (int s = wave; s < nsteps; s += 16) {
+        FGC_TN_STEP(a0, b0, r0, s + 16)
+        FGC_TN_STEP(a1, b1, r1, s + 20)
+        FGC_TN_STEP(a2, b2, r2, s + 24)
+        FGC_TN_STEP(a3, b3, r3, s + 28)
+    }
+#undef FGC_TN_STEP
+    auto put = [&](int slot) {
+#pragma unroll
+        for (int i = 0; i < 4; ++i)
+#pragma unroll
+            for (int j = 0; j < NJ; ++j)
+#pragma unroll
+                for (int t = 0; t < 4; ++t) red[slot][4 * (lq * 4 + t) + i][NJ * lr + j] = acc[i][j][t];
+    };
+    auto add = [&](int slot) {
+#pragma unroll
+        for (int i = 0; i < 4; ++i)
+#pragma unroll
+            for (int j = 0; j < NJ; ++j)
+#pragma unroll
+                for (int t = 0; t < 4; ++t) acc[i][j][t] += red[slot][4 * (lq * 4 + t) + i][NJ * lr + j];
+    };
+    if (wave == 1) put(0);
+    if (wave == 3) put(1);
+    __syncthreads();
+    if (wave == 0) add(0);
+    if (wave == 2) add(1);
+    __syncthreads();
+    if (wave == 0) put(0);
+    if (wave == 2) put(1);
+    __syncthreads();
+    float* out = slab + (size_t)split_id * P * Q;
+    for (int t = tid; t < 64 * 16 * NJ; t += 256) {
+        const int pp = t / (16 * NJ), qq = t % (16 * NJ);
+        if (p0 + pp < P && q0 + qq < Q) out[(size_t)(p0 + pp) * Q + q0 + qq] = red[0][pp][qq] + red[1][pp][qq];
+    }
+}
+
+__device__ __forceinline__ bool tn_direct_ok(int lda, int c0, int c1, int shift, int rows_per_split) {
+    return (c1 == 0 || (c0 & 31) == 0) && shift <= 4 &&
+           (long long)(rows_per_split + 160) * max(lda, max(c0, c1)) < (1ll << 29);
+}
+
+template <int NJ>
+__device__ __forceinline__ void tn_direct_body(const float* __restrict__ A, int lda, int P, const float* __restrict__ x0,
+                                               const float* __restrict__ x1, int c0, int c1, int shift, int rows,
+                                               int rows_per_split, float* __restrict__ slab, int vblock, f32x4* red) {
+    constexpr int NH = NJ / 2;
+    const int Q = c0 + c1;
+    const int npt = (P + 63) >> 6;
+    int tile_id, split_id;
+    if (!tn_block(npt * ((Q + 16 * NJ - 1) / (16 * NJ)), (rows + rows_per_split - 1) / rows_per_split, tile_id, split_id, vblock))
+        return;
+    const int pt = tile_id % npt, qt = tile_id / npt;
+    const int p0 = pt * 64, q0 = qt * (16 * NJ);
+    const int tid = threadIdx.x, lane = tid & 63, lr = lane & 15, lq = lane >> 4;
+    const int wave = __builtin_amdgcn_readfirstlane(tid >> 6);
+    const int r_begin = split_id * rows_per_split;
+    const int r_end = min(rows, r_begin + rows_per_split);
+    const int nsteps = (r_end - r_begin + 3) >> 2;
+    const int row0 = 4 * wave + lq;
+    const int pc = min(p0 + 4 * lr, P - 4);
+    const __amdgpu_buffer_rsrc_t a_rs = __builtin_amdgcn_make_buffer_rsrc(
+        const_cast<float*>(A + (size_t)r_begin * lda), 0, (r_end - r_begin) * lda * 4, 0x00020000);
+    unsigned ao = (unsigned)(row0 * lda + pc) * 4u;
+    const unsigned astep = 16u * (unsigned)lda * 4u;
+    const int xr0 = r_begin >> shift, xrows = ((rows - 1) >> shift) + 1;
+    const int xrow0 = ((r_begin + row0) >> shift) - xr0;
+    __amdgpu_buffer_rsrc_t b_rs[NH];
+    unsigned bo[NH], bstep[NH];
+#pragma unroll
+    for (int h = 0; h < NH; ++h) {
+        const int hs = q0 + 32 * h;
+        const bool first = hs < c0 || c1 == 0;
+        const int ld = first ? c0 : c1;
+        const size_t bytes = (size_t)(xrows - xr0) * ld * 4;
+        b_rs[h] = __builtin_amdgcn_make_buffer_rsrc(const_cast<float*>((first ? x0 : x1) + (size_t)xr0 * ld), 0,
+                                                    (int)(unsigned)std::min<size_t>(bytes, 0xffffffffu), 0x00020000);
+        bo[h] = (unsigned)(xrow0 * ld + min(hs + 2 * lr, Q - 2) - (first ? 0 : c0)) * 4u;
+        bstep[h] = (unsigned)((16 >> shift) * ld) * 4u;
+    }
+    f32x4 acc[4][NJ];
+#pragma unroll
+    for (int i = 0; i < 4; ++i)
+#pragma unroll
+        for (int j = 0; j < NJ; ++j) acc[i][j] = f32x4{0.f, 0.f, 0.f, 0.f};
+
+    struct Set {
+        f32x4 a;
+        f32x2c b[NH];
+    };
+    auto ld = [&](Set& s) {
+        s.a = __builtin_bit_cast(f32x4, __builtin_amdgcn_raw_buffer_load_b128(a_rs, ao, 0, 0));
+        ao += astep;
+        asm volatile("" : "+v"(ao));
+#pragma unroll
+        for (int h = 0; h < NH; ++h) {
+            s.b[h] = __builtin_bit_cast(f32x2c, __builtin_amdgcn_raw_buffer_load_b64(b_rs[h], bo[h], 0, 0));
+            bo[h] += bstep[h];
+            asm volatile("" : "+v"(bo[h]));
+        }
+    };
+    auto mm = [&](const Set& s) {
+#pragma unroll
+        for (int i = 0; i < 4; ++i)
+#pragma unroll
+            for (int j = 0; j < NJ; ++j)
+                acc[i][j] = __builtin_amdgcn_mfma_f32_16x16x4f32(s.a[i], s.b[j >> 1][j & 1], acc[i][j], 0, 0, 0);
+    };
+    if (wave < nsteps) {
+        Set s0, s1, s2, s3;
+        ld(s0);
+        __builtin_amdgcn_sched_barrier(0);
+        ld(s1);
+        __builtin_amdgcn_sched_barrier(0);
+        ld(s2);
+        __builtin_amdgcn_sched_barrier(0);
+        ld(s3);
+        __builtin_amdgcn_sched_barrier(0);
+#define FGC_TN_STEP(S_)                         \
+    mm(S_);                                     \
+    __builtin_amdgcn_sched_barrier(0);          \
+    ld(S_);                                     \
+    __builtin_amdgcn_sched_barrier(0);
+        int s = wave;
+        do {
+            FGC_TN_STEP(s0)
+            FGC_TN_STEP(s1)
+            FGC_TN_STEP(s2)
+            FGC_TN_STEP(s3)
+            s += 16;
+        } while (s < nsteps);
+    }
+#undef FGC_TN_STEP
+    auto put = [&](int slot) {
+#pragma unroll
+        for (int e = 0; e < 4 * NJ; ++e) red[(slot * 4 * NJ + e) * 64 + lane] = acc[e / NJ][e % NJ];
+    };
+    auto add = [&](int slot) {
+#pragma unroll
+        for (int e = 0; e < 4 * NJ; ++e) acc[e / NJ][e % NJ] += red[(slot * 4 * NJ + e) * 64 + lane];
+    };
+    if (wave == 1) put(0);
+    if (wave == 3) put(1);
+    __syncthreads();
+    if (wave == 0) add(0);
+    if (wave == 2) {
+        add(1);
+        put(1);
+    }
+    __syncthreads();
+    if (wave != 0) return;
+    add(1);
+    const __amdgpu_buffer_rsrc_t c_rs =
+        __builtin_amdgcn_make_buffer_rsrc(slab + (size_t)split_id * P * Q, 0, P * Q * 4, 0x00020000);
+#pragma unroll
+    for (int h = 0; h < NH; ++h) {
+        const int q = q0 + 32 * h + 2 * lr;
+        const unsigned co = q < Q ? (unsigned)((p0 + 16 * lq) * Q + q) * 4u : 0x80000000u;
+#pragma unroll
+        for (int t = 0; t < 4; ++t)
+#pragma unroll
+            for (int i = 0; i < 4; ++i)
+                __builtin_amdgcn_raw_buffer_store_b64(__builtin_bit_cast(u32x2, f32x2c{acc[i][2 * h][t], acc[i][2 * h + 1][t]}), c_rs,
+                                                      co + (unsigned)((4 * t + i) * Q) * 4u, 0, 0);
+    }
+}
+
+constexpr int TN_LDS_BYTES = 2 * 64 * 65 * 4;
+template <int NJ, bool BF>
+__device__ __forceinline__ void tn_stream_any(const float* __restrict__ A, int lda, int P, const float* __restrict__ x0,
+                                              const float* __restrict__ x1, int c0, int c1, int shift, int rows,
+                                              int rows_per_split, float* __restrict__ slab, int vblock, float (*red)[64][65]) {
+    if constexpr (!BF) {
+        if (tn_direct_ok(lda, c0, c1, shift, rows_per_split)) {
+            tn_direct_body<NJ>(A, lda, P, x0, x1, c0, c1, shift, rows, rows_per_split, slab, vblock,
+                               reinterpret_cast<f32x4*>(&red[0][0][0]));
+            return;
+        }
+    }
+    tn_stream_body<NJ, BF>(A, lda, P, x0, x1, c0, c1, shift, rows, rows_per_split, slab, vblock, red);
+}
+
+template <int NJ, bool BF>
+__device__ __forceinline__ void tn_group_block(const TnJobs& J, int block, float (*red)[64][65]) {
+    const TnArgs& a = J.job[tn_job_of(J, block)];
+    tn_stream_any<NJ, BF>((const float*)a.A, a.lda, a.P, (const float*)a.x0, (const float*)a.x1, a.c0, a.c1, a.shift, a.rows,
+                          a.rps, a.slab, block - a.block0 + a.first, red);
+}
+
+}
diff --git a/facet_graph_convolution_amd/net.py b/facet_graph_convolution_amd/net.py
--- a/facet_graph_convolution_amd/net.py
+++ b/facet_graph_convolution_amd/net.py
@@ -10,7 +10,7 @@
 import torch
 
 from . import _lib, ops, require_graph_replay_safe
-from ._lib import ConvDesc, ConvBwdIO, AG_LD, DL_LD, FGC_M
+from ._lib import ConvDesc, ConvBwdIO, DwCarry, AG_LD, DL_LD, FGC_M
 from .graph import FacetGraph, as_graph
 
 LRELU_ALPHA = 0.1
@@ -121,6 +121,7 @@
 
 
 _ConvLayer = collections.namedtuple("_ConvLayer", "name level x0 x1 shift y pool act cout pidx", defaults=(None,))
+BACKWARD_ORDER = ("dconv1", "upconv1", "dconv2", "upconv2", "dconv3", "conv3", "conv2", "conv1")
 TRUNK = (
     _ConvLayer("conv1", 0, "xr", None, 0, "h1", "p1", 1, 32),
     _ConvLayer("conv2", 1, "p1", None, 0, "h2", "p2", 1, 64),
@@ -210,6 +211,7 @@
         layer_bufs, M["descs"], M["ios"], M["layer_flags"] = self._bind_layers(M)
         B.update(layer_bufs)
         self._bind_backward_wiring(M)
+        M["dw_ride"] = self._bind_dw_ride(M)
         mlp_bufs, M["arrays"] = self._bind_mlp_and_arrays(M)
         B.update(mlp_bufs)
         self._mesh = M
@@ -417,6 +419,58 @@
             layer_flags["conv1"] = descs["conv1"].flags = layer_flags["conv1"] & ~_lib.CONV_SAVE_Z
         if any(ios[n].r == B["r"].data_ptr() for n in M["grouped_dw_layers"] if n != "conv1"):
             raise RuntimeError("a layer that defers its weight-gradient GEMM shares the backward scratch r")
+
+    def _bind_dw_ride(self, M):
+        none = {"carried": frozenset(), "hosts": {}}
+        if (not M["has_gt"] or M["plan"] is not None or self.dtype != "f32" or self.multi_scale or not self.batched
+                or self._option("NO_DW_RIDE") == 1):
+            return none
+        descs, ios, B, grouped = M["descs"], M["ios"], M["B"], M["grouped_dw_layers"]
+        order = BACKWARD_ORDER
+        deferring = _lib.CONV_PACKED | _lib.CONV_DEFER_REDUCE | _lib.CONV_DEFER_DW
+        carried, hosts = set(), {}
+
+        def attach(name, window, last):
+            io = ios[name]
+            old_flags, io.flags, io.dw_begin = io.flags, deferring, 0
+            taken = []
+            for host in window:
+                if host in hosts or not self.L.fgc_conv_bwd_needs_exchange(C.byref(descs[host]), C.byref(ios[host])):
+                    continue
+                arr = (DwCarry * 1)()
+                arr[0].desc, arr[0].io = C.addressof(descs[name]), C.addressof(io)
+                arr[0].workspace, arr[0].flags = B["wsb_" + name].data_ptr(), _lib.DW_CARRY_LAST
+                hio = ios[host]
+                hio.carry, hio.n_carry, hio.stages, hio.flags = C.addressof(arr), 1, 0, deferring
+                ride = int(_lib.conv_forms(descs[host], hio)["k1_ride"])
+                hio.carry, hio.n_carry, hio.flags = None, 0, 0
+                if ride > 0:
+                    taken.append((host, arr))
+                    io.dw_begin += ride
+            io.flags, io.dw_begin = old_flags, 0
+            taken.sort(key=lambda t: order.index(t[0]))
+            for k, (_, arr) in enumerate(taken):
+                arr[0].flags = _lib.DW_CARRY_LAST if (last and k == len(taken) - 1) else 0
+            if taken:
+                carried.add(name)
+                hosts.update(taken)
+
+        pair_form = lambda host: bool(self.L.fgc_conv_uses_pairs(C.byref(descs[host])))
+        for k, name in enumerate(order[:-1]):
+            if name in grouped:
+                continue
+            window = []
+            for host in order[k + 1:]:
+                window.append(host)
+                if host not in grouped:
+                    break
+            attach(name, sorted(window, key=pair_form), True)
+        shares_r = any(lay.name not in grouped for lay in self.layers[1:])
+        if shares_r and not self.grouped_dw_forced and os.environ.get("FGC_DW_RIDE_GROUPED", "1") != "0":
+            for k, name in enumerate(order[:-1]):
+                if name in grouped and self.L.fgc_conv_bwd_needs_exchange(C.byref(descs[name]), C.byref(ios[name])):
+                    attach(name, order[k + 1:], False)
+        return {"carried": frozenset(carried), "hosts": hosts}
 
     def _bind_mlp_and_arrays(self, M):
         L, B, (n0, n1, n2) = self.L, M["B"], M["ns"]
@@ -899,7 +953,8 @@
             if not self.dw_in_window:
                 flush_dw()
 
-        for name in ["dconv1", "upconv1", "dconv2", "upconv2", "dconv3", "conv3", "conv2", "conv1"]:
+        ride = M["dw_ride"]
+        for name in BACKWARD_ORDER:
             self._tag("bwd:" + name)
             if name == "conv2" and not self.fused_pool:
                 _lib.check(self._pool4_bwd(_p(B["h2"]), _p(B["p2"]), _p(B["g_p2"]), _p(B["g_h2"]), ns[2], 64, 1, st),
@@ -913,7 +968,10 @@
             if self.batched and name in M["grouped_dw_layers"]:
                 base |= _lib.CONV_DEFER_DW
             if not self.sharded:
-                io.stages, io.flags = 0, base
+                io.stages, io.flags = 0, base | (_lib.CONV_DEFER_DW if name in ride["carried"] else 0)
+                io.dw_begin = 0
+                carry = ride["hosts"].get(name)
+                io.carry, io.n_carry = (C.addressof(carry), len(carry)) if carry is not None else (None, 0)
                 _lib.check(L.fgc_conv_bwd(C.byref(d), C.byref(io), _p(lws), lws.numel(), st), name + " bwd")
                 continue
             lay = next(l for l in self.layers if l.name == name)
diff --git a/include/fgc.h b/include/fgc.h
--- a/include/fgc.h
+++ b/include/fgc.h
@@ -17,7 +17,7 @@
 #define FGC_ENOMEM (-12)
 #define FGC_EHIP (-5)
 
-#define FGC_ABI_VERSION 112
+#define FGC_ABI_VERSION 113
 
 const char* fgc_last_error(void);
 int fgc_version(void);
@@ -129,6 +129,17 @@
 int fgc_conv_fwd(const fgc_conv_desc* d, float* ag, float* y, float* y_pool, void* workspace,
                  size_t workspace_bytes, void* stream);
 
+struct fgc_conv_desc;
+struct fgc_conv_bwd_io;
+#define FGC_DW_CARRY_LAST 1
+typedef struct fgc_dw_carry {
+    const struct fgc_conv_desc* desc;
+    struct fgc_conv_bwd_io* io;
+    void* workspace;
+    int32_t flags;
+    int32_t reserved;
+} fgc_dw_carry;
+
 typedef struct fgc_conv_bwd_io {
     const int32_t* trowptr;
     const int32_t* tcol;
@@ -161,6 +172,9 @@
     const int32_t* tpair_edge;
     float* dt;
     int32_t r_ld;
+    int32_t dw_begin;
+    const fgc_dw_carry* carry;
+    int32_t n_carry;
     int32_t reserved0;
 } fgc_conv_bwd_io;
 
```

Result: no change. 65.07 million facets/s (median of 6 runs) (+0.9%).
